# soypat/gsdf

Hardware: AMD Instinct MI355X
Metric: sdf_evals_per_s (higher is better)
Workload: dtype f32

## Files before the change

### gsdf_amd/csrc/abi_host.h

```cpp
#pragma once
#include <hip/hip_runtime.h>

#include <atomic>
#include <cmath>
#include <cstdint>
#include <cstdlib>
#include <string>

#pragma GCC visibility push(default)
#include "../../include/gsdf_hip.h"
#pragma GCC visibility pop

int fail(int code, const std::string& msg);
#define HIP_TRY(expr)                                                                                   \
  do {                                                                                                  \
    hipError_t _e = (expr);                                                                             \
    if (_e != hipSuccess) return fail(GSDF_ERR_HIP, std::string(#expr) + ": " + hipGetErrorString(_e)); \
  } while (0)
#define HIP_TRYM(expr)                                                                                        \
  do {                                                                                                        \
    hipError_t _e = (expr);                                                                                   \
    if (_e != hipSuccess) return bail(fail(GSDF_ERR_HIP, std::string(#expr) + ": " + hipGetErrorString(_e))); \
  } while (0)

inline int env_int(const char* name, int dflt) { const char* e = getenv(name); return e ? atoi(e) : dflt; }
inline uint64_t env_u64(const char* name, uint64_t dflt) { const char* e = getenv(name); return e ? (uint64_t)strtoull(e, nullptr, 10) : dflt; }
inline bool env_flag(const char* name) { const char* e = getenv(name); return e && atoi(e) != 0; }
inline bool env_flag_on(const char* name) { const char* e = getenv(name); return !e || atoi(e) != 0; }
inline bool env_set(const char* name) { return getenv(name) != nullptr; }

inline bool finite_all(const float* v, int n) {
  for (int i = 0; i < n; i++) if (!std::isfinite(v[i])) return false;
  return true;
}

struct gsdf_mesh {
  int device = 0;
  float* d_tris = nullptr;
  uint64_t cap = 0;
  gsdf_mesh_stats st{};
  hipStream_t stream = nullptr;
  hipStream_t rstream = nullptr;
  bool host_out = false;
  void* h_tris = nullptr;
  size_t h_tris_cap = 0;
  void* h_stl = nullptr;
  size_t h_stl_cap = 0;
  int payload = 0;
  uint8_t* d_recs = nullptr;
  uint64_t recs_cap36 = 0;
  uint64_t n_recs = 0;
  bool weldable = false;
  uint8_t* d_wrecs = nullptr;
  uint64_t wrecs_cap36 = 0;
  uint64_t n_wrecs = 0;
  int num_cu = 256;
  int n_stages = 0;
  double stage_ms[8] = {0, 0, 0, 0, 0, 0, 0, 0};
  const char* stage_name[8] = {nullptr, nullptr, nullptr, nullptr, nullptr, nullptr, nullptr, nullptr};
  std::atomic<int> refs{1};
  std::atomic<int> inflight{0};
};
void mesh_inflight_done(gsdf_mesh* m);

struct gsdf_dense_part { uint64_t off, n_recs, tri0; };
constexpr int kDenseMaxParts = 64;
inline uint64_t dense_bytes(uint64_t n_recs) { return n_recs * 40ull + ((((n_recs + 255ull) / 256ull) * 4ull + 7ull) & ~7ull); }
size_t dense_parts_bytes();
void* dense_parts_at(float* d_tris, uint64_t n_tris);
int mesh_march_dense(const uint8_t* d_buf, const gsdf_dense_part* parts, int nparts, void* d_parts, float ox, float oy, float oz, float res,
                     float* d_tris, int num_cu, hipStream_t s);

int indexed_from_cube_slots(int device, int num_cu, hipStream_t s, float* d_slot_cube, uint64_t slot_cap36, uint64_t S, uint64_t cube_cap, const float* d_fv,
                            const void* d_cubes, const hipEvent_t key_ev[4], gsdf_indexed** out);
int launch_block_scan(const unsigned* d_cnt, unsigned n, unsigned* d_base, unsigned long long* d_total, hipStream_t s);

float* pool_take(int device, uint64_t need, uint64_t* cap_out);
void pool_give(int device, float* p, uint64_t cap);
void pool_exporter_opened();
void pool_exporter_closed();
void pool_note_exported(void* base);
void* hpool_take(size_t need, size_t* cap_out);
void hpool_give(void* p, size_t cap);
void big_memcpy(void* dst, const void* src, size_t n);
int host_buf(void** buf, size_t* cap, size_t need);
hipStream_t mesh_stream(gsdf_mesh* m);
void release_tris(gsdf_mesh* m);
```

### gsdf_amd/csrc/abi_mesh.hip

```cpp
#include <algorithm>
#include <cmath>
#include <cstdio>
#include <cstdlib>
#include <cstring>
#include <new>
#include <vector>

#include "kernels_common.h"
#include "kernels_octree.h"
#include "kernels_flat.h"
#include "kernels_dc.h"
#include "kernels_dc_indexed.h"
#include "kernels_stl.h"
#include "kernels_minecraft.h"
#include "abi_program.h"
#include "host_math.h"

namespace {
constexpr size_t kCtrBytes = (sizeof(MeshCounters) + 255) & ~(size_t)255;
const bool ctr_from_kernel = env_flag_on("GSDF_HIP_CTR_FROM_KERNEL");

using leaf_eval_kernel_t = decltype(&leaf_eval_kernel<4, 3>);
using leaf_dense_kernel_t = decltype(&leaf_dense_kernel<3, true, false>);
using dc_origin_kernel_t = decltype(&dc_origin_kernel<4, 3>);
using flat_grid_kernel_t = decltype(&flat_grid_kernel<4, 4>);
leaf_dense_kernel_t leaf_dense_aot(int w) {
  if (w == 3) return leaf_dense_kernel<3, true, false>;
  if (w == 2) return leaf_dense_kernel<2, true, false>;
  return nullptr;
}
leaf_eval_kernel_t leaf_eval_aot(const LeafVariant& v) {
  struct Row { int k, w; bool ucube, ntlds, dz; leaf_eval_kernel_t f; };
  static const Row rows[] = {
      {4, 2, true, true, true, leaf_eval_kernel<4, 2, true, true, false, true>},   {4, 3, true, true, true, leaf_eval_kernel<4, 3, true, true, false, true>},
      {4, 2, true, false, true, leaf_eval_kernel<4, 2, true, false, false, true>}, {4, 3, true, false, true, leaf_eval_kernel<4, 3, true, false, false, true>},
      {4, 2, false, true, false, leaf_eval_kernel<4, 2, false, true>}, {4, 2, true, true, false, leaf_eval_kernel<4, 2, true, true>}, {4, 2, true, false, false, leaf_eval_kernel<4, 2, true, false>},
      {4, 3, false, true, false, leaf_eval_kernel<4, 3, false, true>}, {4, 3, true, true, false, leaf_eval_kernel<4, 3, true, true>}, {4, 3, true, false, false, leaf_eval_kernel<4, 3, true, false>},
      {2, 3, false, true, false, leaf_eval_kernel<2, 3, false, true>}, {2, 3, true, true, false, leaf_eval_kernel<2, 3, true, true>}, {2, 3, true, false, false, leaf_eval_kernel<2, 3, true, false>},
      {1, 4, false, true, false, leaf_eval_kernel<1, 4, false, true>}, {1, 4, true, true, false, leaf_eval_kernel<1, 4, true, true>}, {1, 4, true, false, false, leaf_eval_kernel<1, 4, true, false>},
  };
  if (v.both) return nullptr;
  for (const Row& r : rows)
    if (r.k == v.k && r.w == v.w && r.ucube == v.ucube && r.ntlds == v.ntlds && r.dz == v.dz) return r.f;
  return nullptr;
}
dc_origin_kernel_t dc_origin_aot(SweepVariant v) {
  if (v.k == 4 && v.w == 3) return dc_origin_kernel<4, 3>;
  if (v.k == 2 && v.w == 3) return dc_origin_kernel<2, 3>;
  if (v.k == 1 && v.w == 4) return dc_origin_kernel<1, 4>;
  return nullptr;
}
flat_grid_kernel_t flat_grid_aot(SweepVariant v) {
  if (v.k == 4) return v.w == 4 ? flat_grid_kernel<4, 4> : flat_grid_kernel<4, 3>;
  if (v.k == 2) return v.w == 4 ? flat_grid_kernel<2, 4> : flat_grid_kernel<2, 3>;
  return flat_grid_kernel<1, 4>;
}
}

struct gsdf_mesh_job {
  gsdf_program* p = nullptr;
  gsdf_mesh* m = nullptr;
  gsdf_mesh_opts opts{};
  float res = 0, ox = 0, oy = 0, oz = 0;
  hipStream_t s = nullptr;
  int levels = 0, lq = 0, ls = 0, prune_cols = 0, pmask = 0, ptest = 0, lk = 0;
  size_t lds_prune = 0, lds_m = 0;
  bool want_recs = false;
  uint64_t qcap = 0, want = 0, want_rec_n = 0;
  int attempt = 0, slot;
  bool ctr_on_host = false, used_dz = false, used_dense = false;
  int chain_first = 0;
  uint64_t nblk = 0, nblk_q = 0, lbound = 0;
  size_t clear_bytes = 0;
  bool masks_valid = false;
  Cube* q[2] = {nullptr, nullptr};
  uint64_t capq[2] = {0, 0};
  MeshCounters* d_ctr = nullptr;
  MeshCounters* hcp = nullptr;
  hipEvent_t ev_done = nullptr;
  gsdf_program::OctreeWs& w;
  explicit gsdf_mesh_job(gsdf_program* pp, int sl) : p(pp), slot(sl), w(pp->ws[sl]) {}

  int enqueue();
  int prepare_outputs();
  int enqueue_descent();
  int enqueue_leaf();
  int enqueue_handover();
  int finish(bool* again);
  int stats();
};

int gsdf_mesh_job::enqueue() {
  ctr_on_host = false;
  used_dz = false;
  used_dense = false;
  if (int rc = prepare_outputs()) return rc;
  if (int rc = enqueue_descent()) return rc;
  if (int rc = enqueue_leaf()) return rc;
  HIP_TRY(hipEventRecord(w.ev[2], s));
  return enqueue_handover();
}

int gsdf_mesh_job::prepare_outputs() {
  HIP_TRY(w.q0.ensure(qcap * sizeof(Cube)));
  HIP_TRY(w.q1.ensure(qcap * sizeof(Cube)));
  q[0] = (Cube*)w.q0.p; q[1] = (Cube*)w.q1.p;
  capq[0] = w.q0.cap / sizeof(Cube); capq[1] = w.q1.cap / sizeof(Cube);
  if (want_recs && !m->d_recs) {
    const uint64_t nrec = want_rec_n ? want_rec_n : (p->last_recs ? p->last_recs + p->last_recs / 16 + 1024 : (uint64_t)1 << 20);
    const uint64_t units = (dense_bytes(nrec) + 35) / 36;
    m->d_recs = (uint8_t*)pool_take(p->device, units, &m->recs_cap36);
    if (!m->d_recs) { HIP_TRY(hipMalloc((void**)&m->d_recs, units * 36)); m->recs_cap36 = units; }
  }
  if (!want_recs && !m->d_tris) {
    uint64_t need = want ? want : (p->last_tris ? p->last_tris + p->last_tris / 16 + 1024 : (uint64_t)1 << 20);
    if (opts.host_output) {
      void* hb = nullptr;
      size_t hcap = 0;
      if (int rc = host_buf(&hb, &hcap, (size_t)need * 36)) return rc;
      m->d_tris = (float*)hb;
      m->cap = hcap / 36;
      m->host_out = true;
    } else {
      m->d_tris = pool_take(p->device, need, &m->cap);
      if (!m->d_tris) {
        HIP_TRY(hipMalloc((void**)&m->d_tris, need * 36));
        m->cap = need;
      }
    }
  }
  lbound = capq[lq & 1] << (3 * (lq - 1));
  {
    const uint64_t full = (levels - lq) * 3 >= 40 ? UINT64_MAX : ((uint64_t)1 << (3 * (levels - 1)));
    if (lbound > full) lbound = full;
  }
  constexpr uint64_t kRecBlocks0 = (uint64_t)384 << 10;
  nblk_q = (lbound + 63) / 64;
  nblk = p->rec_blocks ? p->rec_blocks : kRecBlocks0;
  if (nblk > nblk_q) nblk = nblk_q;
  const uint64_t ngrp = (nblk + MARCH_GROUP - 1) / MARCH_GROUP;
  const size_t hdr_bytes = nblk * sizeof(uint32_t), rec_bytes = nblk * (size_t)REC_BLOCK * sizeof(uint32_t);
  if (w.hdr.ensure(hdr_bytes) != hipSuccess || w.rec.ensure(rec_bytes) != hipSuccess) {
    (void)hipGetLastError();
    w.hdr.release(); w.rec.release();
    return fail(GSDF_ERR_CAPACITY, "no device memory for the cut-leaf record arena (" + std::to_string(nblk) + " blocks: " + std::to_string(hdr_bytes) + " + " +
                                       std::to_string(rec_bytes) + " bytes)");
  }
  if (want_recs && w.grp.ensure(ngrp * sizeof(unsigned long long)) != hipSuccess) {
    (void)hipGetLastError();
    return (fail(GSDF_ERR_CAPACITY, "no device memory for the cut-leaf record arena (payload = records needs it)"));
  }
  clear_bytes = kCtrBytes + ngrp * sizeof(unsigned long long);
  HIP_TRY(w.ctr.ensure(clear_bytes));
  d_ctr = (MeshCounters*)w.ctr.p;
  masks_valid = lq == 3 && ptest == 1 && p->prog.n_skip_ids > 0 && (pmask == 1 || (pmask > 1 && ((pmask >> lq) & 1)));
  return GSDF_OK;
}

int gsdf_mesh_job::enqueue_descent() {
  static const bool use_spec = env_flag_on("GSDF_HIP_PRUNE_SPEC");
  if (!use_spec) HIP_TRY(hipMemsetAsync(d_ctr, 0, clear_bytes, s));
  HIP_TRY(hipEventRecord(w.ev[0], s));
  static const int prune_bpc = env_int("GSDF_HIP_PRUNE_BPC", 2);
  int first_level = levels;
  chain_first = levels;
  unsigned* spec_part = nullptr;
  unsigned spec_rows = 0, spec_mask = 0;
  int spec_top_S = 0;
  const unsigned test_mask = pmask == 1 ? 0xffffffffu : (unsigned)pmask;
  if (use_spec) {
    const int S = levels - lq + 1 < 7 ? levels - lq + 1 : 7;
    const int last_spec = levels - (S - 1);
    unsigned n_spec = 0;
    for (int j = 0; j < S; j++) n_spec += 1u << (3 * j);
    const unsigned rrows = (n_spec + SPEC_STAGE - 1) / SPEC_STAGE;
    const size_t part_off = ((size_t)n_spec + 63) & ~(size_t)63;
    const unsigned n_last = 1u << (3 * (S - 1));
    const size_t mask_off_b = (part_off + (size_t)rrows * 16 * sizeof(unsigned) + 63) & ~(size_t)63;
    const bool spec_masks = masks_valid && last_spec == lq;
    HIP_TRY(w.spec_pass.ensure(mask_off_b + (spec_masks ? (size_t)n_last * sizeof(uint16_t) : 0)));
    uint16_t* d_mask16 = spec_masks ? (uint16_t*)((char*)w.spec_pass.p + mask_off_b) : nullptr;
    const bool chain_follows = last_spec - 1 >= lq;
    spec_part = chain_follows ? (unsigned*)((char*)w.spec_pass.p + part_off) : nullptr;
    spec_rows = rrows;
    spec_top_S = levels | (S << 8);
    spec_mask = test_mask;
    const int shard_level = opts.shard_count > 1 ? ls : -1;
    HIP_TRY(launch_kernel(prune_spec_kernel, p->spec.f_prune_spec, grid_for(n_spec, p->num_cu, 8), BLOCK, lds_prune, s, p->d_code.p, levels, n_spec, prune_cols, p->prog.nslots, ox, oy,
                          oz, res, test_mask, ptest, shard_level, opts.shard_rank, opts.shard_count, w.spec_pass.p, (unsigned*)d_ctr, clear_bytes / 4, d_mask16, n_spec - n_last));
    hipLaunchKernelGGL(prune_resolve_kernel, dim3((n_spec + SPEC_STAGE - 1) / SPEC_STAGE), dim3(BLOCK), 0, s, (const uint8_t*)w.spec_pass.p, levels, S,
                       n_spec, test_mask, q[last_spec & 1], (unsigned long long)capq[last_spec & 1], d_ctr, spec_part,
                       (const uint16_t*)d_mask16);
    HIP_TRY(hipGetLastError());
    first_level = last_spec - 1;
    chain_first = first_level;
  }
  for (int level = first_level; level >= lq; level--) {
    const int expand = level != levels;
    const int do_test = (level >= 3 && (pmask == 1 || (pmask > 1 && ((pmask >> level) & 1)))) ? ptest : 0;
    uint64_t bound = (levels - level) * 3 >= 40 ? UINT64_MAX : ((uint64_t)1 << (3 * (levels - level)));
    if (bound > capq[(level + 1) & 1] * 8) bound = capq[(level + 1) & 1] * 8;
    HIP_TRY(launch_kernel(prune_kernel, p->spec.f_prune, grid_for(bound, p->num_cu, prune_bpc), BLOCK, lds_prune, s, p->d_code.p, q[(level + 1) & 1], capq[(level + 1) & 1], expand, level,
                          prune_cols, p->prog.nslots, ox, oy, oz, res, do_test, q[level & 1], capq[level & 1], (opts.shard_count > 1 && level == ls) ? 1 : 0, opts.shard_rank,
                          opts.shard_count, d_ctr, level == first_level ? spec_part : nullptr, spec_rows, spec_top_S, spec_mask));
  }
  HIP_TRY(hipEventRecord(w.ev[1], s));
  return GSDF_OK;
}

int gsdf_mesh_job::enqueue_leaf() {
  const uint64_t bound = lbound;
  const unsigned long long tcap = opts.max_tris ? opts.max_tris : m->cap;
  static const int leaf_bpc = env_int("GSDF_HIP_LEAF_BPC", 32);
  const unsigned grid = grid_for(bound, p->num_cu, leaf_bpc);
  const Cube* cubes = q[lq & 1];
  const uint64_t ncubes = capq[lq & 1];
  uint32_t* d_hdr = (uint32_t*)w.hdr.p;
  uint32_t* d_rec = (uint32_t*)w.rec.p;
  unsigned long long* d_psum = (unsigned long long*)((char*)w.ctr.p + kCtrBytes);
  const unsigned use_masks = masks_valid ? 1u : 0u;
  used_dense = opts.share_corners == 1 && lq == 3 && lk == 4;
  const bool want_dz = opts.share_corners == 2 && lq == 3 && lk == 4;
  if (used_dense) {
    spec_ensure(p, SPEC_DENSE);
    const size_t lds_d = p->lds_dense();
    HIP_TRY(launch_kernel(leaf_dense_aot(3 * lds_d <= gsdf_program::kLdsPerCu ? 3 : 2), p->spec.f_leaf_dense, grid, BLOCK, lds_d, s, p->d_code.p, cubes, ncubes, p->prog.nslots, ox, oy, oz, res,
                          d_hdr, d_rec, d_psum, nblk, d_ctr, use_masks));
  } else {
    if (want_dz) spec_ensure(p, SPEC_ROWS);
    const LeafPick pick = p->leaf_pick(lq, want_dz);
    used_dz = pick.v.dz;
    HIP_TRY(launch_kernel(leaf_eval_aot(pick.v), pick.f, grid, BLOCK, lq != 3 ? lds_m + 256 : lds_m, s, p->d_code.p, cubes, ncubes, lq, p->prog.nslots, ox, oy, oz, res, d_hdr, d_rec,
                          d_psum, nblk, d_ctr, use_masks));
  }
  HIP_TRY(hipEventRecord(w.ev[3], s));
  if (want_recs) {
    uint64_t rec_cap = m->recs_cap36 * 36 / 41;
    if (rec_cap > 2) rec_cap -= 2;
    hipLaunchKernelGGL(scan_groups_kernel, dim3(1), dim3(1024), 0, s, (const unsigned long long*)d_psum, (unsigned long long)nblk, lq, d_ctr,
                       (unsigned long long*)w.grp.p, m->d_recs, (unsigned long long)rec_cap,
                       ctr_from_kernel ? hcp : (MeshCounters*)nullptr);
    HIP_TRY(hipGetLastError());
    const uint64_t ngrp_q = (nblk_q + MARCH_GROUP - 1) / MARCH_GROUP;
    const uint64_t gmax = (uint64_t)p->num_cu * 8;
    hipLaunchKernelGGL(pack_records_kernel, dim3((unsigned)(ngrp_q < gmax ? (ngrp_q ? ngrp_q : 1) : gmax)), dim3(BLOCK), 0, s, (const uint32_t*)d_hdr,
                       (const uint32_t*)d_rec, (const unsigned long long*)w.grp.p, (unsigned long long)nblk, lq, (const MeshCounters*)d_ctr,
                       m->d_recs, (unsigned long long)rec_cap);
  } else {
    static const int march_bpc = env_int("GSDF_HIP_MARCH_BPC", 4);
    const size_t lds_march = MARCH_LDS_BYTES;
    hipLaunchKernelGGL(march_records_kernel, dim3(grid_for(nblk_q, p->num_cu, march_bpc)), dim3(BLOCK), lds_march, s, d_hdr, d_rec,
                       d_psum, (unsigned long long)nblk, lq, ox, oy, oz, res, m->d_tris, (uint64_t)tcap, d_ctr,
                       ctr_from_kernel ? hcp : (MeshCounters*)nullptr);
  }
  ctr_on_host = ctr_from_kernel;
  HIP_TRY(hipGetLastError());
  return GSDF_OK;
}

int gsdf_mesh_job::enqueue_handover() {
  if (!ctr_on_host) {
    HIP_TRY(hipMemcpyAsync(hcp, d_ctr, sizeof(MeshCounters), hipMemcpyDeviceToHost, s));
    HIP_TRY(hipEventRecord(w.ev[4], s));
  }
  ev_done = ctr_on_host ? w.ev[2] : w.ev[4];
  return GSDF_OK;
}

int gsdf_mesh_job::finish(bool* again) {
    MeshCounters& hc = *hcp;
    HIP_TRY(hipEventSynchronize(ev_done));
    if (hc.q_overflow) {
      if (attempt >= 8) return (fail(GSDF_ERR_CAPACITY, "octree queue capacity exceeded"));
      qcap *= 4;
      *again = true;
      return GSDF_OK;
    }
    const uint64_t need = ((hc.n_level[lq] << (3 * (lq - 1))) + 63) / 64;
    if (need > nblk) {
      if (attempt >= 8) return (fail(GSDF_ERR_CAPACITY, "cut-leaf record arena capacity exceeded"));
      p->rec_blocks = need + need / 8 + 1024;
      *again = true;
      return GSDF_OK;
    }
    if (hc.overflow && want_recs) {
      if (attempt >= 8) return (fail(GSDF_ERR_CAPACITY, "device record buffer capacity exceeded"));
      pool_give(p->device, (float*)m->d_recs, m->recs_cap36);
      m->d_recs = nullptr; m->recs_cap36 = 0;
      want_rec_n = hc.n_cut + hc.n_cut / 16 + 1024;
      *again = true;
      return GSDF_OK;
    }
    if (hc.overflow) {
      if (opts.max_tris) return (fail(GSDF_ERR_CAPACITY, "device triangle buffer capacity exceeded"));
      if (attempt >= 8) return (fail(GSDF_ERR_CAPACITY, "device triangle buffer capacity exceeded"));
      release_tris(m);
      want = hc.n_tris + hc.n_tris / 16 + 1024;
      *again = true;
      return GSDF_OK;
    }
    *again = false;
    return GSDF_OK;
}

int gsdf_mesh_job::stats() {
  MeshCounters& hc = *hcp;
  float ms01 = 0, ms12 = 0, ms13 = 0;
  HIP_TRY(hipEventElapsedTime(&ms01, w.ev[0], w.ev[1]));
  HIP_TRY(hipEventElapsedTime(&ms12, w.ev[1], w.ev[2]));
  HIP_TRY(hipEventElapsedTime(&ms13, w.ev[1], w.ev[3]));
  uint64_t evals_prune = 0, pruned = 0;
  for (int level = levels; level >= lq; level--) {
    evals_prune += hc.n_items[level];
    const bool dealt_here = opts.shard_count > 1 && level == ls;
    const uint64_t passed = (level <= chain_first && !dealt_here) ? hc.n_level[level] : hc.n_pass[level];
    if (hc.n_items[level]) pruned += (hc.n_items[level] - passed) << (3 * (level - 1));
  }
  const uint64_t n_leaves = hc.n_level[lq] << (3 * (lq - 1));
  const uint64_t evals_leaf = used_dz || used_dense ? hc.n_points
                                                    : n_leaves * (uint64_t)lk + (uint64_t)(8 - lk) * (lq == 3 ? n_leaves : hc.n_cont);
  m->st.n_tris = hc.n_tris;
  m->st.evals = evals_prune + evals_leaf;
  m->st.evals_prune = evals_prune;
  m->st.evals_leaf = evals_leaf;
  m->st.pruned_leaves = pruned;
  m->st.leaf_cubes = n_leaves;
  m->st.active_leaves = hc.n_active;
  m->st.ms_prune = ms01;
  m->st.ms_leaf = ms12;
  m->st.ms_march = ms13;
  m->st.ms_emit = ms12 - ms13;
  m->st.cut_leaves = hc.n_cut;
  m->st.ms_total = (double)ms01 + (double)ms12;
  p->evals += m->st.evals;
  p->last_tris = hc.n_tris;
  if (want_recs) { m->payload = GSDF_PAYLOAD_RECORDS; m->n_recs = hc.n_cut; p->last_recs = hc.n_cut; m->weldable = opts.shard_count == 1; }
  return GSDF_OK;
}

static void job_release(gsdf_mesh_job* j, bool failed = true) {
  if (!j) return;
  if (failed && j->s) { (void)hipStreamSynchronize(j->s); (void)hipGetLastError(); }
  if (j->p) j->w.job_busy = false;
  if (j->m) gsdf_hip_mesh_destroy(j->m);
  delete j;
}

static constexpr size_t lds_prune_of(int cols) { return (size_t)(cols > 0 ? cols : 1) * 2 * BLOCK * sizeof(float) + PRUNE_STAGE * sizeof(Cube) + 64; }
static constexpr size_t kPruneSpecStatic = SPEC_STAGE * sizeof(Cube) + 256;
static_assert(lds_prune_of(GSDF_HIP_MAX_COLS_OCTREE) + kPruneSpecStatic <= gsdf_program::kLdsPerCu && lds_prune_of(GSDF_HIP_MAX_COLS_OCTREE + 1) + kPruneSpecStatic > gsdf_program::kLdsPerCu,
              "gsdf_hip.h: GSDF_HIP_MAX_COLS_OCTREE is the largest slots + interval stack the centre tests fit into a CU's LDS");
static constexpr size_t lds_dc_edges_of(int slots) { return (size_t)(slots > 0 ? slots : 1) * 3 * BLOCK * sizeof(float) + DC_EDGE_PASSES * BLOCK * sizeof(uint16_t) + 64; }
static_assert(lds_dc_edges_of(GSDF_HIP_MAX_SLOTS_DC) <= gsdf_program::kLdsPerCu && lds_dc_edges_of(GSDF_HIP_MAX_SLOTS_DC + 1) > gsdf_program::kLdsPerCu,
              "gsdf_hip.h: GSDF_HIP_MAX_SLOTS_DC is the largest slot count the edge pass fits into a CU's LDS");
static_assert(GSDF_HIP_MAX_SLOTS_ALL + 16 == GSDF_HIP_MAX_COLS_OCTREE && GSDF_HIP_MAX_SLOTS_ALL <= GSDF_HIP_MAX_SLOTS_DC, "gsdf_hip.h: GSDF_HIP_MAX_SLOTS_ALL");

extern "C" int gsdf_hip_mesh_octree_start(gsdf_program* p, float res, const gsdf_mesh_opts* opts_in, gsdf_mesh_job** out) {
  if (!p || !out) return fail(GSDF_ERR_BAD_ARGUMENT, "null argument");
  *out = nullptr;
  spec_adopt(p);
  if (p->prog.is2d) return fail(GSDF_ERR_DIMENSION, "program is 2D");
  if (!(res > 0) || std::isnan(res) || std::isinf(res)) return fail(GSDF_ERR_RESOLUTION, "invalid renderer cube resolution");
  gsdf_mesh_opts opts{};
  opts.prune = 1; opts.shard_rank = 0; opts.shard_count = 1; opts.share_corners = 0;
  if (opts_in) opts = *opts_in;
  if (opts.shard_count < 1 || opts.shard_rank < 0 || opts.shard_rank >= opts.shard_count) return fail(GSDF_ERR_BAD_ARGUMENT, "bad shard rank/count");
  if (opts.payload != GSDF_PAYLOAD_TRIANGLES && opts.payload != GSDF_PAYLOAD_RECORDS) return fail(GSDF_ERR_BAD_ARGUMENT, "bad payload kind");
  const bool want_recs = opts.payload == GSDF_PAYLOAD_RECORDS;
  if (opts.share_corners < 0 || opts.share_corners > 3) return fail(GSDF_ERR_BAD_ARGUMENT, "share_corners is 0 (every corner of every leaf, as the reference), 1 (distinct lattice points of a brick), 2 (distinct z rows of a brick) or 3 (1 or 2, whichever suits the tree)");
  if (opts.share_corners == 3) opts.share_corners = gsdf_dev::spec_xy_shared_weight(p->prog) < 3 ? 1 : 2;
  if (want_recs && (opts.host_output || opts.max_tris))
    return fail(GSDF_ERR_BAD_ARGUMENT, "payload = records goes with the two-kernel leaf phase only (no host_output, max_tris)");
  {
    const size_t need_prune = lds_prune_of(p->prog.nslots + p->prog.lip_depth) + kPruneSpecStatic, need_leaf = p->leaf_config().lds + 256 + 1024;
    if (int rc = p->lds_refused("gsdf_hip_mesh_octree", need_prune > need_leaf ? need_prune : need_leaf, "slots + interval stack <= " + std::to_string(GSDF_HIP_MAX_COLS_OCTREE))) return rc;
  }
  HIP_TRY(hipSetDevice(p->device));

  float mn[3], mx[3];
  scale_centered(p->prog.bb, 1.01f, mn, mx);
  const float longAxis = fmaxf(mx[0] - mn[0], fmaxf(mx[1] - mn[1], mx[2] - mn[2]));
  const float l2 = gsdf::log2f32(longAxis / res);
  const int levels = (int)std::ceil(l2) + 1;
  if (levels <= 1) return fail(GSDF_ERR_RESOLUTION, "resolution not fine enough for marching cubes");
  if (levels > 17) return fail(GSDF_ERR_RESOLUTION, "resolution too fine: more than 17 octree levels");
// ... 61 lines not shown
    j->attempt++;
    if (int rc = j->enqueue()) { job_release(j); return rc; }
  }
  if (int rc = j->stats()) { job_release(j); return rc; }
  *out = j->m;
  j->m = nullptr;
  job_release(j, false);
  return GSDF_OK;
}

extern "C" int gsdf_hip_mesh_octree(gsdf_program* p, float res, const gsdf_mesh_opts* opts_in, gsdf_mesh** out) {
  if (!out) return fail(GSDF_ERR_BAD_ARGUMENT, "null argument");
  *out = nullptr;
  gsdf_mesh_job* j = nullptr;
  if (int rc = gsdf_hip_mesh_octree_start(p, res, opts_in, &j)) return rc;
  return gsdf_hip_mesh_octree_wait(j, out);
}

static_assert(sizeof(gsdf_dense_part) == sizeof(DensePart) && kDenseMaxParts == DENSE_MAX_PARTS, "abi_host.h mirrors kernels_octree.h");
size_t dense_parts_bytes() { return sizeof(DenseParts) + 8; }
void* dense_parts_at(float* d_tris, uint64_t n_tris) {
  return (void*)(((uintptr_t)(d_tris + n_tris * 9) + 7) & ~(uintptr_t)7);
}
int mesh_march_dense(const uint8_t* d_buf, const gsdf_dense_part* parts, int nparts, void* d_parts, float ox, float oy, float oz, float res,
                     float* d_tris, int num_cu, hipStream_t s) {
  if (nparts < 1 || nparts > DENSE_MAX_PARTS) return fail(GSDF_ERR_BAD_ARGUMENT, "march over packed records: 1 to 64 parts");
  DenseParts h{};
  h.n = nparts;
  uint64_t chunks = 0;
  for (int i = 0; i < nparts; i++) {
    h.p[i].off = parts[i].off; h.p[i].n_recs = parts[i].n_recs; h.p[i].tri0 = parts[i].tri0;
    chunks += (parts[i].n_recs + DENSE_CHUNK - 1) / DENSE_CHUNK;
    if (dense_bytes(parts[i].n_recs) != dense_payload_bytes(parts[i].n_recs)) return fail(GSDF_ERR_BAD_ARGUMENT, "internal: payload layouts differ");
  }
  if (chunks == 0) return GSDF_OK;
  HIP_TRY(hipMemcpyAsync(d_parts, &h, sizeof h, hipMemcpyHostToDevice, s));
  static const int march_bpc = env_int("GSDF_HIP_MARCH_BPC", 4);
  const uint64_t gmax = (uint64_t)num_cu * (uint64_t)(march_bpc > 0 ? march_bpc : 4);
  const size_t lds = MARCH_DENSE_LDS_BYTES;
  hipLaunchKernelGGL(march_dense_kernel, dim3((unsigned)(chunks < gmax ? chunks : gmax)), dim3(BLOCK), lds, s, d_buf, (const DenseParts*)d_parts, ox, oy, oz, res, d_tris);
  HIP_TRY(hipGetLastError());
  return GSDF_OK;
}

extern "C" int gsdf_hip_mesh_stage_ms(const gsdf_mesh* m, double* ms, const char** names, int cap, int* n) {
  if (!m || !n) return fail(GSDF_ERR_BAD_ARGUMENT, "null argument");
  *n = m->n_stages;
  for (int k = 0; k < m->n_stages && k < cap; k++) {
    if (ms) ms[k] = m->stage_ms[k];
    if (names) names[k] = m->stage_name[k];
  }
  return GSDF_OK;
}

extern "C" int gsdf_hip_mesh_payload(const gsdf_mesh* m, uint64_t* n_records, uint64_t* payload_bytes) {
  if (!m) return fail(GSDF_ERR_BAD_ARGUMENT, "null argument");
  const bool r = m->payload == GSDF_PAYLOAD_RECORDS;
  if (n_records) *n_records = r ? m->n_recs : 0;
  if (payload_bytes) *payload_bytes = r ? dense_bytes(m->n_recs) : 0;
  return m->payload;
}

extern "C" int gsdf_hip_mesh_read_records(const gsdf_mesh* m, uint32_t* dst, uint64_t dst_records, uint64_t* n_records) {
  if (!m) return fail(GSDF_ERR_BAD_ARGUMENT, "null argument");
  const bool r = m->payload == GSDF_PAYLOAD_RECORDS;
  const uint8_t* d = r ? m->d_recs : m->d_wrecs;
  const uint64_t n = r ? m->n_recs : m->n_wrecs;
  if (!r && !m->weldable) return fail(GSDF_ERR_BAD_ARGUMENT, "the mesh holds no cut-leaf records (payload = GSDF_PAYLOAD_RECORDS keeps them)");
  if (n_records) *n_records = n;
  if (!dst) return GSDF_OK;
  if (dst_records < n) return fail(GSDF_ERR_SHORT_BUFFER, "short buffer");
  if (n == 0) return GSDF_OK;
  HIP_TRY(hipSetDevice(m->device));
  HIP_TRY(hipMemcpy(dst, d, n * 40ull, hipMemcpyDeviceToHost));
  return GSDF_OK;
}

extern "C" int gsdf_hip_mesh_march(gsdf_mesh* m) {
  if (!m) return fail(GSDF_ERR_BAD_ARGUMENT, "null argument");
  if (m->payload != GSDF_PAYLOAD_RECORDS) return GSDF_OK;
  if (m->inflight.load() > 0) return fail(GSDF_ERR_BAD_ARGUMENT, "the mesh is being gathered: wait for the gather first");
  HIP_TRY(hipSetDevice(m->device));
  const uint64_t n = m->st.n_tris;
  if (n) {
    const uint64_t units = n + (dense_parts_bytes() + 35) / 36;
    m->d_tris = pool_take(m->device, units, &m->cap);
    if (!m->d_tris) {
      if (hipMalloc((void**)&m->d_tris, units * 36) != hipSuccess) { (void)hipGetLastError(); return fail(GSDF_ERR_HIP, "hipMalloc of the triangle buffer failed"); }
      m->cap = units;
    }
    const gsdf_dense_part part{0, m->n_recs, 0};
    hipStream_t rs = mesh_stream(m);
    const int rc = mesh_march_dense(m->d_recs, &part, 1, dense_parts_at(m->d_tris, n), m->st.origin[0], m->st.origin[1], m->st.origin[2], m->st.res, m->d_tris,
                                    m->num_cu, rs);
    if (rc) { release_tris(m); return rc; }
    hipError_t e = hipStreamSynchronize(rs);
    if (e != hipSuccess) { release_tris(m); return fail(GSDF_ERR_HIP, std::string("march over the records: ") + hipGetErrorString(e)); }
  }
  if (m->weldable) { m->d_wrecs = m->d_recs; m->wrecs_cap36 = m->recs_cap36; m->n_wrecs = m->n_recs; }
  else pool_give(m->device, (float*)m->d_recs, m->recs_cap36);
  m->d_recs = nullptr; m->recs_cap36 = 0; m->n_recs = 0;
  m->payload = GSDF_PAYLOAD_TRIANGLES;
  return GSDF_OK;
}

namespace {
// ... 610 lines not shown
```

### gsdf_amd/csrc/abi_program.h

```cpp
#pragma once
#include <condition_variable>
#include <mutex>
#include <thread>
#include <vector>

#include "abi_host.h"
#include "compile.h"
#include "launch_args.h"
#include "specialize.h"

struct NoCopy {
  NoCopy() = default;
  NoCopy(const NoCopy&) = delete;
  NoCopy& operator=(const NoCopy&) = delete;
};
struct Arena : NoCopy {
  void* p = nullptr;
  size_t cap = 0;
  ~Arena() { release(); }
  hipError_t ensure(size_t bytes) {
    if (bytes <= cap) return hipSuccess;
    release();
    size_t want = bytes + bytes / 4 + 4096;
    hipError_t e = hipMalloc(&p, want);
// ... 31 lines not shown
  int k, w;
  std::string spec_name(const char* base, int dim = 0) const { return std::string(base) + "<" + (dim ? std::to_string(dim) + ", " : "") + std::to_string(k) + ", " + std::to_string(w) + ">"; }
  std::string short_name(const char* base, int dim = 0) const { return std::string(base) + "<" + (dim ? std::to_string(dim) + "," : "") + std::to_string(k) + "," + std::to_string(w) + ">"; }
};
struct LeafVariant {
  int k, w;
  bool ucube, ntlds, both, dz;
  std::string spec_name() const {
    auto b = [](bool x) { return x ? ", true" : ", false"; };
    return "leaf_eval_kernel<" + std::to_string(k) + ", " + std::to_string(w) + b(ucube) + b(ntlds) + b(both) + b(dz) + ">";
  }
  std::string short_name() const {
    return "leaf_eval_kernel<" + std::to_string(k) + "," + std::to_string(w) + (both ? ",both" : "") + (dz ? ",rows" : "") + ">";
  }
};
struct LeafPick { LeafVariant v; hipFunction_t f; };

enum SpecGroup { SPEC_AUX, SPEC_ROWS, SPEC_EVAL_K1, SPEC_DENSE, SPEC_VIEW, SPEC_PROJECT, SPEC_PICTURE, SPEC_RAY, SPEC_GROUPS };
struct SpecBuilt {
  std::vector<hipModule_t> mods;
  int eval_k = 0, eval_w = 0, leaf_k = 0, leaf_w = 0, rows_w = 0, dense_w = 0;
  bool leaf_both = false, rows_both = false;
  std::string compiler, key;
  double compile_s = 0;
};
struct SpecFns {
  hipFunction_t f_eval = nullptr, f_eval_k1 = nullptr, f_prune = nullptr, f_prune_spec = nullptr, f_leaf = nullptr, f_leaf_dz = nullptr, f_leaf_dense = nullptr;
  hipFunction_t f_dc_block_test = nullptr, f_dc_origin = nullptr, f_dc_edges = nullptr, f_dc_normals = nullptr, f_normals = nullptr, f_image = nullptr, f_flat_grid = nullptr;
  hipFunction_t f_view = nullptr, f_view_plain = nullptr, f_project = nullptr, f_imgc[4] = {nullptr, nullptr, nullptr, nullptr};
  hipFunction_t f_ray = nullptr, f_ray_thick = nullptr;
};
struct SpecKernels : SpecBuilt, SpecFns, NoCopy {
  std::atomic<unsigned> todo{0};
  ~SpecKernels() { for (hipModule_t m : mods) (void)hipModuleUnload(m); }
  bool specialised() const { return !mods.empty(); }
  void take(SpecKernels& from) {
    std::swap(static_cast<SpecBuilt&>(*this), static_cast<SpecBuilt&>(from));
    compile_s += from.compile_s;
    std::atomic_thread_fence(std::memory_order_release);
    static_cast<SpecFns&>(*this) = from;
    todo.store(from.todo.load(), std::memory_order_release);
  }
};

struct gsdf_program {
  gsdf_dev::Program prog;
  int device = 0;
  Stream stream;
  struct OctreeWs {
    Stream own;
    Arena q0, q1;
    Arena ctr;
    Arena spec_pass;
    Arena rec, hdr;
    Arena grp;
    EventSet<5> ev;
    bool job_busy = false;
    hipStream_t job_stream = nullptr;
  };
  static constexpr int kJobs = 3;
  OctreeWs ws[kJobs];
  bool mesh_in_flight() const { for (const OctreeWs& w : ws) if (w.job_busy) return true; return false; }
  DevPtr<uint32_t> d_code;
  std::atomic<uint64_t> evals{0};
  DevPtr<void> d_pos;
  DevPtr<float> d_dist;
  size_t cap_pos_bytes = 0, cap_dist = 0;
  struct Slot : NoCopy {
    Stream s;
    PinnedPtr<void> h_pos;
    PinnedPtr<float> h_dist;
    bool busy = false, waiting = false;
    unsigned gen = 0;
    float* user_dist = nullptr;
    size_t n = 0;
    bool zero_copy = false;
    PinnedPtr<unsigned> h_flag;
    unsigned* d_flag = nullptr;
    unsigned flag_val = 0;
    bool flagged = false;
  };
  static constexpr int kSlots = 4;
  Slot slot[kSlots];
  std::mutex slot_mu;
  std::condition_variable slot_cv;
  std::atomic<uint64_t> evals_host{0};
  int num_cu = 256;
  Arena dc_tile, dc_grid, dc_dist, dc_fv, dc_nrm, dc_edge, dc_erun, dc_flag;
  Arena dc_ix, dc_ix_sort;
  EventSet<4> dc_ev;
  Arena flat_grid;
  Arena flat_bits;
  Arena flat_list;
  PinnedPtr<void> h_ctr;
  uint64_t last_tris = 0;
  uint64_t last_recs = 0;
  uint64_t rec_blocks = 0;
  uint64_t last_dc_cubes = 0;
  SpecKernels spec;
  size_t lds_dense() const { return (size_t)(prog.nslots * 4 > 8 ? prog.nslots * 4 : 8) * BLOCK * sizeof(float) + 256 + 4 * 512 * sizeof(float) + 4 * 24 * sizeof(float) + 16; }
  struct CountedLaunch { DevPtr<void> ctr; EventSet<2> ev; };
  CountedLaunch proj, ray;
  std::atomic<int> spec_async{0};
  std::thread spec_thread;
  gsdf_program* spec_shadow = nullptr;
  std::mutex spec_async_mu;
// ... 108 lines not shown
```

### gsdf_amd/csrc/compile.cpp

```cpp
#include "compile.h"

#include <algorithm>
#include <cmath>
#include <cstdlib>
#include <cstring>
#include <stdexcept>
#include <string>
#include <utility>

#include "host_math.h"
#include "dev_ops.h"
#include "gsdf_seams.h"

namespace gsdf_dev {

float recip_for(float d) {
  const float a = std::fabs(d);
  if (!(a >= 9.313225746154785e-10f && a <= 1073741824.0f)) return 0.f;
  float best = (float)(1.0 / (double)d);
  long double berr = fabsl(1.0L - (long double)d * (long double)best);
  const float cand[2] = {std::nextafterf(best, INFINITY), std::nextafterf(best, -INFINITY)};
  for (float c : cand) {
    long double err = fabsl(1.0L - (long double)d * (long double)c);
    if (err < berr) { berr = err; best = c; }
  }
  return best;
}

namespace {

constexpr float SQRT3 = 1.7320508075688772935274463415058723669428052538103806280558069794f;

struct Ctx {
  const gsdf_tree* t;
  std::vector<uint32_t> code;
  int slots = 0;
  int max_slots = 0;
  int lip_depth = 0, max_lip_depth = 0;
  int n_recip = 0, n_recip_declined = 0, n_poly_recip = 0, n_poly_plain = 0;
  float node_recip(float d) { const float r = recip_for(d); (r != 0.f ? n_recip : n_recip_declined)++; return r; }
  int lip_push() { const int d = lip_depth++; if (lip_depth > max_lip_depth) max_lip_depth = lip_depth; op(D_LIP_PUSH, d); return d; }
  void lip_pop(int d) { op(D_LIP_POP, d); lip_depth--; }
  int discont = 0;
  bool numbering = false;
  std::vector<double> cand_cost;
  std::vector<int> cand_id;
  std::vector<uint64_t> cand_key;
  size_t cand_next = 0;
  bool cand_mismatch = false;
  int candidate(double cost, uint32_t node, uint32_t child_slot) {
    const size_t i = cand_next++;
    const uint64_t key = ((uint64_t)node << 32) | child_slot;
    if (!numbering) { cand_cost.push_back(cost); cand_key.push_back(key); return -1; }
    if (i >= cand_id.size() || cand_key[i] != key) { cand_mismatch = true; return -1; }
    return cand_id[i];
  }
  size_t max_code;
  std::vector<int8_t> clob;
  struct Table { size_t patch; float angle; int n; };
  std::vector<Table> tables;
  uint32_t xyver = 1, next_ver = 2, hxyver = 0;
  std::vector<uint32_t> slotver = std::vector<uint32_t>(1 << 16, 0);
  void bump() { xyver = next_ver++; }
  uint32_t pver = 1;
  std::vector<uint32_t> slotpver = std::vector<uint32_t>(1 << 16, 0);
  uint8_t dep[3] = {1, 2, 4};
  std::vector<uint32_t> slotdep = std::vector<uint32_t>(1 << 16, 0x070707u);
  uint32_t shxy_flag() const { return ((dep[0] | dep[1]) & 4) ? 0u : D_FLAG_SHXY; }
  uint32_t shz_flag() const { return (dep[2] & 3) ? 0u : D_FLAG_SHZ; }
  void dep_after(uint32_t base) {
    switch (base) {
      case D_TRANSLATE: case D_SCALE_PRE: case D_SYMMETRY: case D_ELONGATE_PRE: case D_ELONGATE2D_PRE: case D_EXTRUDE_PRE:
        break;
      case D_ROT2D: case D_CIRC_PRE: dep[0] = dep[1] = (uint8_t)(dep[0] | dep[1]); break;
      case D_TWIST: dep[0] = dep[1] = (uint8_t)(dep[0] | dep[1] | dep[2]); break;
      default: dep[0] = dep[1] = dep[2] = 7; break;
    }
  }
  struct Outer { bool valid = false; int slot = 0; float ok = 0.f; } outer;
  struct Saved { int slot; bool is2d; };
  std::vector<Saved> live;
  int find_saved(bool is2d) const {
    for (size_t k = live.size(); k-- > 0;) {
      const Saved& s = live[k];
      if (is2d ? (slotver[(size_t)s.slot] == xyver) : (!s.is2d && slotpver[(size_t)s.slot] == pver)) return s.slot;
    }
    return -1;
  }
  void mark_saved(int slot, bool is2d) {
    slotver[(size_t)slot] = xyver;
    slotpver[(size_t)slot] = pver;
    slotdep[(size_t)slot] = dep[0] | (dep[1] << 8) | (dep[2] << 16);
    live.push_back({slot, is2d});
  }
  void load_saved(int slot, bool is2d) {
    op(is2d ? D_LOADP2 : D_LOADP3, slot);
// ... 618 lines not shown

void gen(Ctx& c, uint32_t i, int depth) {
  if (depth > 256) throw std::runtime_error("tree too deep (cycle?)");
  const gsdf_node& n = c.node(i);
  if (n.op != GSDF_DIFF && n.op != GSDF_SMOOTH_DIFF && n.op != GSDF_DIFF2D) c.outer.valid = false;
  const float* P = n.p;
  auto need_children = [&](uint32_t k) { if (n.nchild != k) throw std::runtime_error("bad child count for op " + std::to_string(n.op)); };
  auto child_dim = [&](bool want2d) {
    for (uint32_t k = 0; k < n.nchild; k++)
      if ((bool)gsdf_op_is2d(c.node(c.child(n, k)).op) != want2d) throw std::runtime_error("child dimension mismatch for op " + std::to_string(n.op));
  };
  switch (n.op) {
    case GSDF_SPHERE: c.op(D_SPHERE); c.f(P[0]); break;
    case GSDF_BOX: c.op(D_BOX); c.f(0.5f * P[0]); c.f(0.5f * P[1]); c.f(0.5f * P[2]); c.f(P[3]); break;
    case GSDF_BOXFRAME: {
      float e = P[3];
      c.op(D_BOXFRAME); c.f(e);
      c.f(0.5f * P[0] + (-2 * e)); c.f(0.5f * P[1] + (-2 * e)); c.f(0.5f * P[2] + (-2 * e));
      break;
    }
    case GSDF_TORUS: c.op(D_TORUS | c.hxy_flag() | c.shxy_flag()); c.f(P[0]); c.f(P[1]); break;
    case GSDF_CYLINDER: {
      float r = P[0], h = (P[1] - 2 * P[2]) / 2, round = P[2];
      if (round == 0) { c.op(D_CYL0 | c.hxy_flag() | c.shxy_flag()); c.f(r); c.f(h); }
      else { c.op(D_CYLR | c.hxy_flag() | c.shxy_flag()); c.f(r); c.f(h); c.f(round); }
      break;
    }
    case GSDF_HEX: c.op(D_HEX); c.f(P[0]); c.f(P[1]); c.f(0.57735f * P[0]); break;
    case GSDF_UNION: if (n.nchild < 2) throw std::runtime_error("OpUnion must have at least 2 elements"); child_dim(false); gen_combine(c, n, D_COMBINE_MIN, false, depth); break;
    case GSDF_INTERSECT: need_children(2); child_dim(false); gen_combine(c, n, D_COMBINE_MAX, false, depth); break;
    case GSDF_DIFF: need_children(2); child_dim(false); gen_combine(c, n, D_COMBINE_DIFF, false, depth); break;
    case GSDF_XOR: need_children(2); child_dim(false); gen_combine(c, n, D_COMBINE_XOR, false, depth); break;
    case GSDF_SMOOTH_UNION: need_children(2); child_dim(false); gen_combine(c, n, D_COMBINE_SUNION, true, depth); break;
    case GSDF_SMOOTH_DIFF: need_children(2); child_dim(false); gen_combine(c, n, D_COMBINE_SDIFF, true, depth); break;
    case GSDF_SMOOTH_INTERSECT: need_children(2); child_dim(false); gen_combine(c, n, D_COMBINE_SINTER, true, depth); break;
    case GSDF_SCALE: need_children(1); child_dim(false);
      { const int ld = c.lip_push(); c.op(D_SCALE_PRE); c.f(1.f / P[0]); c.bump(); gen(c, c.child(n, 0), depth + 1); c.op(D_MULR); c.f(P[0]); c.lip_pop(ld); } break;
    case GSDF_SYMMETRY: need_children(1); child_dim(false);
      c.op(D_SYMMETRY); c.u((uint32_t)(int)P[0]); if ((int)P[0] & 3) c.bump(); gen(c, c.child(n, 0), depth + 1); break;
    case GSDF_ARRAY: {
      need_children(1); child_dim(false);
      int slotP = c.alloc(3), slotD = c.alloc(1);
      const unsigned seams = array_seams(c, i);
      const int lipd = seams ? c.lip_push() : -1;
      c.op(D_SAVEP3, slotP);
      c.op(D_SETSLOT, slotD); c.f(1e20f);
      for (int k = 0; k < 2; k++) for (int j = 0; j < 2; j++) for (int ii = 0; ii < 2; ii++) {
        c.op(D_ARRAY_PRE, slotP);
        c.bump();
        c.f((float)ii); c.f((float)j); c.f((float)k);
        c.f(P[0]); c.f(P[1]); c.f(P[2]);
        c.f(P[3] + -1); c.f(P[4] + -1); c.f(P[5] + -1);
        if (seams && k == 0 && j == 0 && ii == 0) { c.op(D_LIP_SEAM); c.u(seams); }
        c.discont++; gen(c, c.child(n, 0), depth + 1); c.discont--;
        c.op(D_COMBINE_MIN, slotD);
        if (!(k == 1 && j == 1 && ii == 1)) c.op(D_SAVER, slotD);
      }
      if (lipd >= 0) c.lip_pop(lipd);
      c.release(4);
      break;
    }
    case GSDF_ELONGATE: {
      need_children(1); child_dim(false);
      int s = c.alloc(1);
      c.op(D_ELONGATE_PRE, s); c.f(0.5f * P[0]); c.f(0.5f * P[1]); c.f(0.5f * P[2]);
      c.bump();
      gen(c, c.child(n, 0), depth + 1);
      c.op(D_ADDR_SLOT, s);
      c.release(1);
      break;
    }
    case GSDF_SHELL: need_children(1); child_dim(false);
      { const int ld = c.lip_push(); c.op(D_SCALE_PRE); c.f(1 / P[0]); c.bump(); gen(c, c.child(n, 0), depth + 1); c.op(D_SHELL_POST); c.f(P[0]); c.lip_pop(ld); } break;
    case GSDF_OFFSET: need_children(1); child_dim(false);
      gen(c, c.child(n, 0), depth + 1); c.op(D_ADDR); c.f(P[0]); break;
    case GSDF_TRANSLATE: need_children(1); child_dim(false);
      c.op(D_TRANSLATE); c.f(P[0]); c.f(P[1]); c.f(P[2]);
      if (!(P[0] == 0.f && P[1] == 0.f)) c.bump();
      gen(c, c.child(n, 0), depth + 1); break;
    case GSDF_TRANSFORM: {
      need_children(1); child_dim(false);
      if (n.aux_len < 16) throw std::runtime_error("transform needs 16 aux floats");
      int lipd = -1;
      {
        float f = lip_norm3(&c.t->aux[n.aux_off]);
        if (f > kLipRigidTol) { lipd = c.lip_push(); c.op(D_LIP_MUL); c.f(f * kLipRoundUp); }
      }
      c.op(D_TRANSFORM);
      for (int k = 0; k < 12; k++) c.f(c.t->aux[n.aux_off + k]);
      c.bump();
      gen(c, c.child(n, 0), depth + 1);
      if (lipd >= 0) c.lip_pop(lipd);
      break;
    }
    case GSDF_CIRCARRAY: case GSDF_CIRCARRAY2D: {
      need_children(1);
      bool is2d = n.op == GSDF_CIRCARRAY2D;
      child_dim(is2d);
      int slotP = c.alloc(is2d ? 2 : 3), slotD = c.alloc(1);
      const bool seams = circ_seams(c, i);
      const int lipd = seams ? c.lip_push() : -1;
      if (!is2d) c.op(D_SAVEP3, slotP);
      c.op(D_CIRC_PRE | c.shxy_flag(), slotP);
      c.bump();
      c.slotver[(size_t)slotP] = c.xyver;
      c.slotpver[(size_t)slotP] = c.next_ver++;
      c.slotdep[(size_t)slotP] = c.dep[0] | (c.dep[1] << 8) | (c.dep[2] << 16);
      c.live.push_back({slotP, is2d});
      c.bump();
      c.f((float)(2 * gsdf::kPi) / P[1]); c.f(P[1]); c.f((float)((int)P[0] - 1));
      c.tables.push_back({c.code.size(), (float)(2 * gsdf::kPi) / P[1], (int)P[1]});
      c.u(0);
      Region cg;
      const bool sector_off = [] { const char* e = getenv("GSDF_HIP_NO_SECTOR_GATE"); return e && atoi(e) != 0; }();
      constexpr double kSectorGateMinCost = 150.0;
      const bool sector_gate = !sector_off && !is2d && subtree_cost(c, c.child(n, 0)) >= kSectorGateMinCost && lower_region(c, c.child(n, 0), cg) &&
                               (cg.kind == Region::BOX || cg.kind == Region::OBOX);
      if (sector_gate && cg.kind == Region::BOX) {
        Region o;
        o.kind = Region::OBOX;
        o.b[0] = 0.5f * (cg.b[0] + cg.b[3]); o.b[1] = 0.5f * (cg.b[1] + cg.b[4]); o.b[2] = 1.f; o.b[3] = 0.f;
        o.b[4] = 0.5f * (cg.b[3] - cg.b[0]) * 1.000001f; o.b[5] = 0.5f * (cg.b[4] - cg.b[1]) * 1.000001f; o.b[6] = cg.b[2]; o.b[7] = cg.b[5];
        cg = o;
      }
      if (sector_gate) { c.op(D_CIRC_ORDER, slotP); for (int j = 0; j < 6; j++) c.f(cg.b[j]); }
      if (seams) { c.op(D_LIP_SEAM, slotP); c.u(8u); }
      c.discont++;
      gen(c, c.child(n, 0), depth + 1);
      c.op(D_SAVER, slotD);
      c.load_saved(slotP, is2d);
      if (is2d) c.slotpver[(size_t)slotP] = c.pver;
      long skip_at = -1, gate_pc = -1;
      const uint32_t hxy_before = c.hxyver;
      if (sector_gate) {
        gate_pc = (long)c.code.size();
        c.op(D_GATEOB, slotD);
        for (int j = 0; j < 8; j++) c.f(cg.b[j]);
        c.f(1.0f); c.f(0.0f); c.u(0xffffu); c.f(0.0f); c.f(0.0f);
        skip_at = (long)c.code.size();
        c.u(0);
      }
      gen(c, c.child(n, 0), depth + 1);
      c.discont--;
      if (skip_at >= 0) {
        if (c.hxyver != hxy_before) c.hxyver = 0;
        c.code[(size_t)skip_at] = (uint32_t)((long)c.code.size() - gate_pc);
      }
      c.op(D_COMBINE_MIN, slotD);
      if (lipd >= 0) c.lip_pop(lipd);
      c.live.pop_back();
      c.release(is2d ? 3 : 4);
      break;
    }
    case GSDF_TWIST: {
      need_children(1); child_dim(false);
      const int lipd = c.lip_push();
      c.op(D_TWIST | c.shz_flag()); c.f(P[0]); c.bump(); gen(c, c.child(n, 0), depth + 1);
      c.lip_pop(lipd);
      break;
    }
    case GSDF_EXTRUSION: {
      need_children(1); child_dim(true);
      int s = c.alloc(1);
      c.op(D_EXTRUDE_PRE, s); c.f(P[0] / 2);
      gen(c, c.child(n, 0), depth + 1);
      c.op(D_EXTRUDE_POST, s);
      c.release(1);
      break;
    }
    case GSDF_REVOLUTION: need_children(1); child_dim(true);
      c.op(D_REVOLVE_PRE); c.f(P[0]); c.bump(); gen(c, c.child(n, 0), depth + 1); break;
    case GSDF_SCREW: {
      need_children(1); child_dim(true);
      int s = c.alloc(1);
      const int lipd = c.lip_push();
      c.op(D_SCREW_PRE | c.hxy_flag() | c.shxy_flag(), s);
      c.bump();
      c.f(P[0]); c.f(P[1]); c.f(P[2]); c.f(gsdf::tanf32(P[3])); c.f(P[0] / 2); c.f(c.node_recip(P[0]));
      c.op(D_LIP_WRAP); c.f(P[0] / 2); c.f(lip_screw_seam(*c.t, c.child(n, 0), P[0]));
      c.discont++; gen(c, c.child(n, 0), depth + 1); c.discont--;
      c.lip_pop(lipd);
      c.op(D_MAXR_SLOT, s);
      c.release(1);
      break;
    }
    case GSDF_LINE2D: {
      float bax = P[2] - P[0], bay = P[3] - P[1];
      c.op(D_LINE2D); c.f(P[0]); c.f(P[1]); c.f(bax); c.f(bay); c.f(bax * bax + bay * bay); c.f(P[4] / 2);
      break;
    }
    case GSDF_ARC2D: {
      float s, cs;
      gsdf::sincosf32(P[1] / 2, s, cs);
      c.op(D_ARC2D); c.f(P[0]); c.f(P[2] / 2); c.f(s); c.f(cs); c.f(P[0] * s); c.f(P[0] * cs);
      break;
    }
    case GSDF_QUADBEZIER2D: {
      float Ax = P[0], Ay = P[1], Bx = P[2], By = P[3], Cx = P[4], Cy = P[5];
      float ax = Bx - Ax, ay = By - Ay;
      float a2 = ax * ax + ay * ay;
      float bx = Ax + (Cx - 2 * Bx), by = Ay + (Cy - 2 * By);
      float cx = 2 * ax, cy = 2 * ay;
      float kk = 1.f / (bx * bx + by * by);
      float kx = kk * (ax * bx + ay * by);
      float kx2 = kx * kx;
      c.op(D_QUADBEZIER2D);
      c.f(Ax); c.f(Ay); c.f(ax); c.f(ay); c.f(a2); c.f(bx); c.f(by); c.f(cx); c.f(cy); c.f(kk); c.f(kx); c.f(kx2); c.f(P[6] / 2);
      break;
    }
    case GSDF_CIRCLE2D: c.op(D_CIRCLE2D | c.hxy_flag() | c.shxy_flag()); c.f(P[0]); break;
    case GSDF_EQTRI2D: { float r = P[0] / SQRT3; c.op(D_EQTRI2D); c.f(r); c.f(r / SQRT3); break; }
    case GSDF_RECT2D: c.op(D_RECT2D); c.f(0.5f * P[0]); c.f(0.5f * P[1]); break;
    case GSDF_DIAMOND2D: {
      float bx = 0.5f * P[0], by = 0.5f * P[1];
      c.op(D_DIAMOND2D); c.f(bx); c.f(by); c.f(bx * bx + by * by); c.f(0.5f * bx); c.f(0.5f * by); c.f(bx * by);
      break;
    }
    case GSDF_X2D: c.op(D_X2D); c.f(P[0]); c.f(P[1]); break;
    case GSDF_HEX2D: c.op(D_HEX2D); c.f(P[0]); c.f(0.577350269f * P[0]); break;
    case GSDF_OCT2D: c.op(D_OCT2D); c.f(P[0]); c.f(0.4142135623f * P[0]); break;
    case GSDF_ELLIPSE2D: c.op(D_ELLIPSE2D); c.f(P[0]); c.f(P[1]); break;
    case GSDF_POLY2D: {
      uint32_t nv = n.aux_len / 2;
      if (nv < 3) throw std::runtime_error("polygon needs at least 3 vertices");
      const float* v = &c.t->aux[n.aux_off];
      bool all_recip = true;
      {
        uint32_t jv0 = nv - 1;
        for (uint32_t iv = 0; iv < nv; iv++) {
          float ex = v[2 * jv0] - v[2 * iv], ey = v[2 * jv0 + 1] - v[2 * iv + 1];
          if (recip_for(ex * ex + ey * ey) == 0.f) all_recip = false;
          jv0 = iv;
        }
      }
      (all_recip ? c.n_poly_recip : c.n_poly_plain)++;
      c.op(D_POLY2D); c.u(nv | (all_recip ? 0x80000000u : 0u)); c.f(v[0]); c.f(v[1]);
      while (c.code.size() % 8 != 0) c.u(0);
      uint32_t jv = nv - 1;
      for (uint32_t iv = 0; iv < nv; iv++) {
        float v1x = v[2 * iv], v1y = v[2 * iv + 1], v2x = v[2 * jv], v2y = v[2 * jv + 1];
        float ex = v2x - v1x, ey = v2y - v1y;
        const float n2e = ex * ex + ey * ey;
        c.f(v1x); c.f(v1y); c.f(ex); c.f(ey); c.f(n2e); c.f(v2y); c.f(recip_for(n2e)); c.u(0);
        jv = iv;
      }
      break;
    }
    case GSDF_LINES2D: {
      uint32_t ns = n.aux_len / 4;
      const float* sg = &c.t->aux[n.aux_off];
      c.op(D_LINES2D); c.u(ns); c.f(P[0] / 2);
      for (uint32_t k = 0; k < ns; k++) {
        float ax = sg[4 * k], ay = sg[4 * k + 1], bax = sg[4 * k + 2] - ax, bay = sg[4 * k + 3] - ay;
        c.f(ax); c.f(ay); c.f(bax); c.f(bay); c.f(bax * bax + bay * bay);
      }
      break;
    }
    case GSDF_UNION2D: if (n.nchild < 2) throw std::runtime_error("OpUnion2D must have at least 2 elements"); child_dim(true); gen_combine(c, n, D_COMBINE_MIN, false, depth); break;
    case GSDF_INTERSECT2D: need_children(2); child_dim(true); gen_combine(c, n, D_COMBINE_MAX, false, depth); break;
    case GSDF_DIFF2D: need_children(2); child_dim(true); gen_combine(c, n, D_COMBINE_DIFF, false, depth); break;
    case GSDF_XOR2D: need_children(2); child_dim(true); gen_combine(c, n, D_COMBINE_XOR, false, depth); break;
    case GSDF_ARRAY2D: {
      need_children(1); child_dim(true);
      int slotP = c.alloc(2), slotD = c.alloc(1);
      const unsigned seams = array_seams(c, i);
      const int lipd = seams ? c.lip_push() : -1;
      c.op(D_SAVEP2, slotP);
      c.op(D_SETSLOT, slotD); c.f(1e20f);
      for (int j = 0; j < 2; j++) for (int ii = 0; ii < 2; ii++) {
        c.op(D_ARRAY2D_PRE, slotP);
        c.bump();
        c.f((float)ii); c.f((float)j); c.f(P[0]); c.f(P[1]); c.f(P[2] + -1); c.f(P[3] + -1);
        if (seams && j == 0 && ii == 0) { c.op(D_LIP_SEAM); c.u(seams); }
        c.discont++; gen(c, c.child(n, 0), depth + 1); c.discont--;
        c.op(D_COMBINE_MIN, slotD);
        if (!(j == 1 && ii == 1)) c.op(D_SAVER, slotD);
      }
      if (lipd >= 0) c.lip_pop(lipd);
      c.release(3);
      break;
    }
    case GSDF_OFFSET2D: need_children(1); child_dim(true); gen(c, c.child(n, 0), depth + 1); c.op(D_ADDR); c.f(P[0]); break;
    case GSDF_TRANSLATE2D: need_children(1); child_dim(true);
      c.op(D_TRANSLATE); c.f(P[0]); c.f(P[1]); c.f(0.f); if (!(P[0] == 0.f && P[1] == 0.f)) c.bump(); gen(c, c.child(n, 0), depth + 1); break;
    case GSDF_SYMMETRY2D: need_children(1); child_dim(true);
      c.op(D_SYMMETRY); c.u((uint32_t)(int)P[0] & 3u); if ((int)P[0] & 3) c.bump(); gen(c, c.child(n, 0), depth + 1); break;
    case GSDF_ANNULUS2D: need_children(1); child_dim(true); gen(c, c.child(n, 0), depth + 1); c.op(D_ANNULUS); c.f(P[0]); break;
    case GSDF_TRANSLATEMULTI2D: {
      need_children(1); child_dim(true);
      uint32_t nd = n.aux_len / 2;
      const float* d = &c.t->aux[n.aux_off];
      int slotP = c.alloc(2), slotD = c.alloc(1);
      c.op(D_SAVEP2, slotP);
      c.op(D_SETSLOT, slotD); c.f(3.40282346638528859811704183484516925440e+38f);
      if (nd == 0) { c.op(D_SETR); c.f(3.40282346638528859811704183484516925440e+38f); }
      for (uint32_t k = 0; k < nd; k++) {
        c.op(D_LOADP2_SUB, slotP); c.f(d[2 * k]); c.f(d[2 * k + 1]);
        c.bump();
        gen(c, c.child(n, 0), depth + 1);
        c.op(D_COMBINE_MIN, slotD);
        if (k + 1 < nd) c.op(D_SAVER, slotD);
      }
      c.release(3);
      break;
    }
    case GSDF_ROTATION2D: {
      need_children(1); child_dim(true);
      int lipd = -1;
      {
        float f = lip_norm2(P[0], P[1], P[2], P[3]);
        if (f > kLipRigidTol) { lipd = c.lip_push(); c.op(D_LIP_MUL); c.f(f * kLipRoundUp); }
      }
      c.op(D_ROT2D); c.f(P[0]); c.f(P[1]); c.f(P[2]); c.f(P[3]); c.bump(); gen(c, c.child(n, 0), depth + 1);
      if (lipd >= 0) c.lip_pop(lipd);
      break;
    }
    case GSDF_SCALE2D: need_children(1); child_dim(true);
      { const int ld = c.lip_push(); c.op(D_SCALE_PRE); c.f(1.f / P[0]); c.bump(); gen(c, c.child(n, 0), depth + 1); c.op(D_MULR); c.f(P[0]); c.lip_pop(ld); } break;
    case GSDF_ELONGATE2D: {
      need_children(1); child_dim(true);
      int s = c.alloc(1);
      c.op(D_ELONGATE2D_PRE, s); c.f(0.5f * P[0]); c.f(0.5f * P[1]);
      c.bump();
      gen(c, c.child(n, 0), depth + 1);
      c.op(D_ADDR_SLOT, s);
      c.release(1);
      break;
// ... 63 lines not shown
    const bool masks_off = [] { const char* e = getenv("GSDF_HIP_NO_BRICK_MASKS"); return e && atoi(e) != 0; }();
    cand_id.assign(c0.cand_cost.size(), -1);
    cand_key = c0.cand_key;
    if (!masks_off) {
      std::vector<size_t> idx(c0.cand_cost.size());
      for (size_t i = 0; i < idx.size(); i++) idx[i] = i;
      std::stable_sort(idx.begin(), idx.end(), [&](size_t x, size_t y) { return c0.cand_cost[x] > c0.cand_cost[y]; });
      std::vector<char> take(idx.size(), 0);
      for (size_t i = 0; i < idx.size() && i < 16; i++) take[idx[i]] = 1;
      int next = 0;
      for (size_t i = 0; i < take.size(); i++) if (take[i]) cand_id[i] = next++;
    }
  }
  Ctx c;
  c.t = &t;
  c.max_code = max_code_words;
  c.clob.assign(t.n_nodes, -1);
  c.numbering = true;
  c.cand_id = cand_id;
  c.cand_key = cand_key;
  gen(c, t.root, 0);
  if (c.cand_mismatch || c.cand_next != cand_id.size()) {
    bool any = false;
    for (int v : cand_id) any = any || v >= 0;
    if (any) {
      Ctx c2;
      c2.t = &t;
      c2.max_code = max_code_words;
      c2.clob.assign(t.n_nodes, -1);
      c2.numbering = true;
      c2.cand_id.assign(cand_id.size(), -1);
      c2.cand_key = cand_key;
      gen(c2, t.root, 0);
      if (c2.cand_mismatch || c2.cand_next != cand_id.size()) throw std::runtime_error("lowering is not repeatable: candidate subtrees differ between runs");
      c = std::move(c2);
      std::fill(cand_id.begin(), cand_id.end(), -1);
    }
  }
  c.op(D_END);
  for (const Ctx::Table& tb : c.tables) {
    if (tb.n < 1 || tb.n > 4096) continue;
    c.code[tb.patch] = (uint32_t)c.code.size();
    for (int i = 0; i < tb.n; i++) {
      float sn, cs;
      gsdf::sincosf32(tb.angle * (float)i, sn, cs);
      c.f(sn); c.f(cs);
    }
  }
  Program p;
  p.code = std::move(c.code);
  p.nslots = c.max_slots;
  p.lip_depth = c.max_lip_depth;
  p.n_recip = c.n_recip; p.n_recip_declined = c.n_recip_declined; p.n_poly_recip = c.n_poly_recip; p.n_poly_plain = c.n_poly_plain;
  p.n_skip_ids = 0;
  for (int v : cand_id) if (v >= 0) p.n_skip_ids++;
  p.is2d = gsdf_op_is2d(t.nodes[t.root].op);
  p.has_exact_bb = exact_box(c, t.root, p.exact_bb);
  std::memcpy(p.bb, t.bb, sizeof(p.bb));
  return p;
}

}
```

### gsdf_amd/csrc/compile.h

```cpp
#pragma once
#include <cstddef>
#include <cstdint>
#include <vector>

#include "../../include/gsdf_program.h"

namespace gsdf_dev {

struct Program {
  std::vector<uint32_t> code;
  int nslots = 0;
  int lip_depth = 0;
  int n_skip_ids = 0;
  bool is2d = false;
  float bb[6] = {0};
  bool has_exact_bb = false;
  float exact_bb[6] = {0};
  int n_recip = 0, n_recip_declined = 0, n_poly_recip = 0, n_poly_plain = 0;
};

float recip_for(float d);

int region_of(const gsdf_tree& t, uint32_t node, float params[8]);

Program compile(const gsdf_tree& t, size_t max_code_words = (1u << 22));

}
```

### gsdf_amd/csrc/dev_ops.h

```cpp
#pragma once
#ifndef __HIPCC_RTC__
#include <stdint.h>
#endif

#define D_OP_MASK 0x0fffu
#define D_FLAG_SHZ 0x1000u
#define D_FLAG_SHXY 0x2000u
#define D_FLAG_HXY 0x4000u
#define D_FLAG_SWAP 0x8000u

enum DevOp : uint32_t {
  D_END = 0,
  D_SPHERE,
  D_BOX,
  D_BOXFRAME,
  D_TORUS,
  D_CYL0,
  D_CYLR,
  D_HEX,
  D_LINE2D,
  D_ARC2D,
  D_QUADBEZIER2D,
  D_CIRCLE2D,
  D_EQTRI2D,
// ... 18 lines not shown
  D_ELONGATE2D_PRE,
  D_ARRAY_PRE,
  D_ARRAY2D_PRE,
  D_CIRC_PRE,
  D_LOADP2_SUB,
  D_MULR,
  D_SHELL_POST,
  D_ADDR,
  D_ANNULUS,
  D_EXTRUDE_POST,
  D_MAXR_SLOT,
  D_ADDR_SLOT,
  D_SAVEP3, D_LOADP3, D_SAVEP2, D_LOADP2, D_SAVER,
  D_SETSLOT,
  D_SETR,
  D_COMBINE_MIN, D_COMBINE_MAX, D_COMBINE_DIFF, D_COMBINE_XOR,
  D_COMBINE_SUNION, D_COMBINE_SDIFF, D_COMBINE_SINTER,
  D_GATE2D,
  D_GATE3D,
  D_GATEZC,
  D_UBOUND2D,
  D_UBOUND3D,
  D_GATEOB,
  D_CIRC_ORDER,
  D_LIP_PUSH,
  D_LIP_POP,
  D_LIP_MUL,
  D_LIP_WRAP,
  D_SKIP,
  D_LIP_DOM,
  D_LIP_SEAM,
  D_OP_COUNT
};

static const uint8_t kDevOpParams[D_OP_COUNT] = {
     0,
     1,  4,  4,  2,  2,  3,  3,
     6,  6,  13,  1,  2,  2,  6,  2,
     2,  2,  2,  3,  2,
     3,  1,  1,  12,  1,  4,
     1,  1,  6,  3,  2,
     9,  6,  4,  2,
     1,  1,  1,  1,  0,  0,  0,
     0,  0,  0,  0,  0,  1,  1,
     0,  0,  0,  0,  2,  2,  2,
     10,  12,  13,  1,  1,  14,  6,
     0,  0,  1,  2,
     3,  5,  1,
};
#define GSDF_GATE_SKIP(w) ((w) & 0x00ffffffu)
#define GSDF_GATE_ID1(w) ((w) >> 24)
#define GSDF_BRICK_MASK_VALID 0x80000000u
#define GSDF_SKIP_BIG 1.0e30f
```

### gsdf_amd/csrc/interp.h

```cpp
#pragma once
#ifndef __HIPCC_RTC__
#include <hip/hip_runtime.h>
#endif

#include "dev_math.h"
#include "dev_ops.h"

namespace gsdf_dev {

typedef const uint32_t __attribute__((address_space(4))) * code_ptr;
typedef float v4f __attribute__((ext_vector_type(4)));
typedef const v4f __attribute__((address_space(4))) * f4ptr;

struct P3 { float x, y, z; };

__device__ __forceinline__ uint32_t lane_id() { return __builtin_amdgcn_mbcnt_hi(~0u, __builtin_amdgcn_mbcnt_lo(~0u, 0u)); }

#define LDSF(slot) lds[((slot) * K + kp) * nthreads]
#define KLOOP _Pragma("unroll") for (int kp = 0; kp < K; ++kp)

template <bool ON>
__device__ __forceinline__ float in_vgpr(float s) {
  if (!ON) return s;
  float v;
// ... 80 lines not shown
__device__ __forceinline__ float wave_minmax(float v) {
  if (MAX) {
#define GSDF_DPP_CHAIN(op)                                                                                                   \
  asm volatile("s_nop 1\n\t" op "_dpp %0, %0, %0 row_shr:1 row_mask:0xf bank_mask:0xf\n\t"                                  \
               "s_nop 1\n\t" op "_dpp %0, %0, %0 row_shr:2 row_mask:0xf bank_mask:0xf\n\t"                                  \
               "s_nop 1\n\t" op "_dpp %0, %0, %0 row_shr:4 row_mask:0xf bank_mask:0xf\n\t"                                  \
               "s_nop 1\n\t" op "_dpp %0, %0, %0 row_shr:8 row_mask:0xf bank_mask:0xf\n\t"                                  \
               "s_nop 1\n\t" op "_dpp %0, %0, %0 row_bcast:15 row_mask:0xa bank_mask:0xf\n\t"                               \
               "s_nop 1\n\t" op "_dpp %0, %0, %0 row_bcast:31 row_mask:0xc bank_mask:0xf\n\t"                               \
               "s_nop 1"                                                                                                     \
               : "+v"(v))
    GSDF_DPP_CHAIN("v_max_f32");
  } else {
    GSDF_DPP_CHAIN("v_min_f32");
  }
#undef GSDF_DPP_CHAIN
  return __uint_as_float((uint32_t)__builtin_amdgcn_readlane((int)__float_as_uint(v), 63));
}

template <int K>
__device__ __forceinline__ void poly_cull(code_ptr code, uint32_t q0, uint32_t nv, const P3 (&pv)[K], uint64_t& keepd,
                                          uint64_t& keeps, const bool recip = false) {
  using namespace dm;
  float x0 = pv[0].x, x1 = pv[0].x, y0 = pv[0].y, y1 = pv[0].y;
  KLOOP {
    x0 = minf(x0, pv[kp].x); x1 = maxf(x1, pv[kp].x);
    y0 = minf(y0, pv[kp].y); y1 = maxf(y1, pv[kp].y);
  }
  wave_box(x0, x1, y0, y1);
  const uint32_t lane = lane_id();
  const bool valid = lane < nv;
  const v4f* rec = (const v4f*)((const float*)(uintptr_t)code + q0 + 8u * (valid ? lane : 0u));
  const v4f r0 = rec[0], r1 = rec[1];
  const float v1x = r0.x, v1y = r0.y, ex = r0.z, ey = r0.w, n2e = r1.x, v2y = r1.y;
  const float cx = 0.5f * (x0 + x1), cy = 0.5f * (y0 + y1), hx = 0.5f * (x1 - x0), hy = 0.5f * (y1 - y0);
#ifdef GSDF_NO_CULL_APPROX
  const bool approx = false;
#else
  const bool approx = recip;
#endif
  const float rb2 = hx * hx + hy * hy;
  const float rb = approx ? __builtin_amdgcn_sqrtf(rb2) : sqrtf_(rb2);
  const float wx = cx - v1x, wy = cy - v1y;
  const float num = wx * ex + wy * ey;
  const float t = __builtin_amdgcn_fmed3f(approx ? num * r1.z : num / n2e, 0.f, 1.f);
  const float bx = wx - t * ex, by = wy - t * ey;
  const float dc2 = bx * bx + by * by;
  const float dc = approx ? __builtin_amdgcn_sqrtf(dc2) : sqrtf_(dc2);
  const float m = 1.0e-5f * (absf(wx) + absf(wy) + absf(ex) + absf(ey) + rb + absf(cx) + absf(cy));
  const float U = wave_minmax<false>(valid ? (dc + rb) + m : __builtin_inff());
  const uint64_t vm = nv >= 64u ? ~0ull : (1ull << nv) - 1ull;
  keepd = vm & ~wave_mask((dc - rb) - m > U);
  keeps = vm & ~((wave_mask(y0 >= v1y) & wave_mask(y0 >= v2y)) | (wave_mask(y1 < v1y) & wave_mask(y1 < v2y)));
}

template <int K, typename F>
__device__ __forceinline__ void xy_shared(const P3 (&pv)[K], float (&out)[K], bool shared, bool brick, F f, bool column = false) {
  if (shared && column) {
    const float v = f(pv[0].x, pv[0].y);
    KLOOP out[kp] = v;
    return;
  }
  if (K == 4 && shared && brick) {
    const uint32_t lane = lane_id();
    const bool odd = ((lane >> 4) & 1u) != 0u;
    const float sx = odd ? pv[K > 2 ? 2 : 0].x : pv[0].x, sy = odd ? pv[K > 2 ? 2 : 0].y : pv[0].y;
    const float v = f(sx, sy);
    const float v0 = __shfl(v, (int)(lane & 15u), 64), v1 = __shfl(v, (int)((lane & 15u) + 16u), 64);
    out[0] = v0; out[K > 1 ? 1 : 0] = v0;
    out[K > 2 ? 2 : 0] = v1; out[K > 3 ? 3 : 0] = v1;
    return;
  }
  KLOOP if (!(kp & 1)) out[kp] = f(pv[kp].x, pv[kp].y);
  if (shared) { KLOOP if (kp & 1) out[kp] = out[kp ? kp - 1 : 0]; }
  else { KLOOP if (kp & 1) out[kp] = f(pv[kp].x, pv[kp].y); }
}
struct XYCache {
  float th = 0.0f;
  uint32_t pc = 0xffffffffu;
};

template <int K>
__device__ __forceinline__ void atan2_shared(const P3 (&pv)[K], float (&out)[K], bool shared, bool brick, bool column) {
#if defined(GSDF_SPECIALIZED) && !defined(GSDF_NO_ATAN2_FAST)
  if (!(shared && column)) {
    dm::wave_ok ok;
    xy_shared<K>(pv, out, shared, brick, [&ok](float x, float y) { return dm::atan2_fast(y, x, ok); }, column);
    if (ok.all()) return;
  }
#endif
  xy_shared<K>(pv, out, shared, brick, [](float x, float y) { return dm::atan2_ref(y, x); }, column);
}

__device__ __forceinline__ void cossin_voted(float x, float& c, float& s) {
#if defined(GSDF_SPECIALIZED) && !defined(GSDF_NO_COSSIN_FAST)
  dm::wave_ok ok;
  dm::cossin_fast(x, c, s, ok);
  if (ok.all()) return;
#endif
  dm::cossinf_(x, c, s);
}

#define ENSURE_HXY() \
  if (!use_hxy) xy_shared<K>(pv, hxy, sh_xy, brick, [](float x, float y) { return dm::hypotf_(x, y); }, sh_col)

template <int K, int DIM>
// ... 161 lines not shown
            switch (kind) {                                                                                                            \
              case 0u: sb = blo > ahi + GSDF_DOM_M(blo, ahi); sa = alo > bhi + GSDF_DOM_M(alo, bhi); break;                            \
              case 1u: sb = bhi < alo - GSDF_DOM_M(bhi, alo); sa = ahi < blo - GSDF_DOM_M(ahi, blo); break;                            \
              case 2u: sb = blo > -alo + GSDF_DOM_M(blo, alo); sa = ahi < -bhi - GSDF_DOM_M(ahi, bhi); break;                          \
              case 3u: sb = blo - ahi > GSDF_DOM_M(blo, ahi); sa = alo - bhi > GSDF_DOM_M(alo, bhi); break;                            \
              case 4u: sb = blo + alo > GSDF_DOM_M(blo, alo); sa = bhi + ahi < -GSDF_DOM_M(bhi, ahi); break;                           \
              case 5u: sb = alo - bhi > GSDF_DOM_M(alo, bhi); sa = blo - ahi > GSDF_DOM_M(blo, ahi); break;                            \
              default: break;                                                                                                          \
            }                                                                                                                          \
            if (sa && ida < 32u) *lip_fired |= 1u << ida;                                                                              \
            if (sb && idb < 32u) *lip_fired |= 1u << idb;                                                                              \
          }                                                                                                                            \
        }                                                                                                                              \

#define GSDF_LIP_SEAM_BODY \
        if (LIP) {                                                                                                                     \
          const uint32_t seams = PU(0);                                                                                                \
          bool reach = false;                                                                                                          \
          if ((seams & 1u) != 0u) reach = reach || !(absf(pv[0].x) > lipR);                                                            \
          if ((seams & 2u) != 0u) reach = reach || !(absf(pv[0].y) > lipR);                                                            \
          if ((seams & 4u) != 0u) reach = reach || !(absf(pv[0].z) > lipR);                                                            \
          if ((seams & 8u) != 0u) {                  \
            const float x0 = lds[((slot) * K + LIP_LO) * nthreads], y0 = lds[((slot + 1u) * K + LIP_LO) * nthreads];                   \
            reach = !(lip_ray_dist(pv[0].x, pv[0].y) > lipR) || !(lip_ray_dist(x0, y0) > lipR);                                        \
          }                                                                                                                            \
          if (reach) lipR = GSDF_LIP_BIG;                                                                                              \
        }                                                                                                                              \

static_assert(GSDF_BRICK_MASK_VALID == 1u << 31, "GSDF_GATE_TEST reads the brick mask's valid flag as bit 31");
#define GSDF_GATE_TEST(REGION, DIM, I0)                                                                                      \
  float L[K];                                                                                                               \
  bool far_ = false;                                                                                                        \
  {                                                                                                                         \
    const uint32_t gid1 = GSDF_GATE_ID1(PU((I0) + 5));                                                                      \
     \
    const bool untested = !LIP && gid1 != 0u && ((bmask >> 31u) & 1u) != 0u;  \
    if (!untested) {                                                                                                        \
      float a[K], cc[K];                                                                                                    \
      const uint32_t oslot = PU((I0) + 2);                                                                                  \
      const bool has_outer = oslot != 0xffffu;                                                            \
      KLOOP { a[kp] = LDSF(slot); cc[kp] = has_outer ? LDSF(oslot) : 0.0f; }                                                \
      REGION;                                                                                                               \
      if (LIP) KLOOP L[kp] = L[kp] - lipR;  \
      bool lane_good = false;                                                                                               \
      far_ = gate_far<K, DIM, LIP>(pv, a, L, PF(I0), PF((I0) + 1), cc, has_outer, PF((I0) + 3), PF((I0) + 4), &lane_good);  \
      if (LIP && gid1 != 0u && lip_fired != nullptr && lane_good) *lip_fired |= 1u << (gid1 - 1u);                          \
    }                                                                                                                       \
  }
#define GSDF_GATE_TAKEN                                                       \
  {                                                                           \
    if (LIP) { Rv[LIP_LO] = L[LIP_LO]; Rv[LIP_HI] = GSDF_SKIP_BIG; }          \
    else { KLOOP Rv[kp] = L[kp]; }                                            \
  }
#ifndef GSDF_SPECIALIZED
template <int K, int SHARE = 0, bool LIP = false>
__device__ __forceinline__ void sdf_eval(code_ptr code, P3 (&pv)[K], float (&Rv)[K],
                                         float* __restrict__ lds , const uint32_t nthreads,
                                         const bool brick = false ,
                                         const float lip_h = 0.0f, const uint32_t lip_base = 0u,
                                         const uint32_t bmask_w = 0u ,
                                         uint32_t* lip_fired = nullptr ,
                                         XYCache* xyc = nullptr ) {
  using namespace dm;
  static_assert(!LIP || (K == 2 && SHARE == 0), "interval mode: two points per lane, lower and upper bound");
  [[maybe_unused]] float lipR = lip_h;
  const dm::uniform_word bmask{bmask_w};
  KLOOP Rv[kp] = 0.0f;
  float hxy[K];
  KLOOP hxy[kp] = 0.0f;
  uint32_t pc = 0;
#define PF(k) __uint_as_float(code[pc + 1 + (k)])
#define PU(k) (code[pc + 1 + (k)])
  for (;;) {
    pc = __builtin_amdgcn_readfirstlane(pc);
    const uint32_t w = code[pc];
    const uint32_t op = w & D_OP_MASK;
    const uint32_t slot = w >> 16;
    const bool use_hxy = (w & D_FLAG_HXY) != 0u;
    const bool swap_ab = (w & D_FLAG_SWAP) != 0u;
    const bool sh_xy = SHARE != 0 && K >= 2 && (w & D_FLAG_SHXY) != 0u;
    const bool sh_z = SHARE == 1 && K >= 4 && (w & D_FLAG_SHZ) != 0u;
    const bool sh_col = SHARE == 2;
    const bool sh_zu = SHARE == 2 && brick && (w & D_FLAG_SHZ) != 0u;
    switch (op) {
      case D_END:
        return;
      case D_SPHERE: {
        KLOOP {
          [[maybe_unused]] P3& p = pv[kp];
          [[maybe_unused]] float& R = Rv[kp];
          R = norm3(p.x, p.y, p.z) - PF(0);
        }
        pc += 2;
        break;
      }
      case D_BOX: {
        {
          const float r = PF(3);
          float u[K], v[K], w[K];
          KLOOP {
            const P3& p = pv[kp];
            u[kp] = (absf(p.x) - PF(0)) + r; v[kp] = (absf(p.y) - PF(1)) + r; w[kp] = (absf(p.z) - PF(2)) + r;
          }
          if (face3_op<K>(u, v, w)) {
            KLOOP Rv[kp] = face_val(maxf(u[kp], maxf(v[kp], w[kp]))) - r;
          } else {
            float mx[K], my[K], mz[K], in[K], hyz[K], n3[K];
            KLOOP {
              const float qx = u[kp], qy = v[kp], qz = w[kp];
              mx[kp] = maxf(qx, 0.f); my[kp] = maxf(qy, 0.f); mz[kp] = maxf(qz, 0.f);
              in[kp] = minf(maxf(qx, maxf(qy, qz)), 0.0f);
            }
            hypot_k<K>(my, mz, hyz);
            hypot_k<K>(mx, hyz, n3);
            KLOOP Rv[kp] = n3[kp] + in[kp] - r;
          }
// ... 297 lines not shown
          [[maybe_unused]] P3& p = pv[kp];
          [[maybe_unused]] float& R = Rv[kp];
          float a = PF(0), b = PF(1);
          float px = absf(p.x), py = absf(p.y);
          if (px > py) { float t = px; px = py; py = t; t = a; a = b; b = t; }
          float l = b * b - a * a;
          float m = a * px / l;
          float m2 = m * m;
          float nn = b * py / l;
          float n2 = nn * nn;
          float c = (m2 + n2 - 1.f) / 3.f;
          float c3 = c * c * c;
          float q = c3 + 2.f * m2 * n2;
          float d = c3 + m2 * n2;
          float g = m + m * n2;
          float co;
          if (d < 0.f) {
            float h = acosf_(q / c3) / 3.f;
            float sh, ch;
            sincosf_(h, sh, ch);
            float t = 1.7320508075688772f * sh;
            float rx = sqrtf_(-c * (ch + t + 2.f) + m2);
            float ry = sqrtf_(-c * (ch - t + 2.f) + m2);
            co = (ry + signf(l) * rx + absf(g) / (rx * ry) - m) / 2.f;
          } else {
            float h = 2.f * m * nn * sqrtf_(d);
            float sv = signf(q + h) * cbrtf_(absf(q + h));
            float u = signf(q - h) * cbrtf_(absf(q - h));
            float rx = -sv - u - 4.f * c + 2.f * m2;
            float ry = 1.7320508075688772f * (sv - u);
            float rm = hypotf_(rx, ry);
            co = (ry / sqrtf_(rm - rx) + 2.f * g / rm - m) / 2.f;
          }
          float rx2 = a * co, ry2 = b * sqrtf_(1.f - co * co);
          R = norm2(rx2 - px, ry2 - py) * signf(py - ry2);
        }
        pc += 3;
        break;
      }
      case D_POLY2D: {
        const uint32_t hdr = PU(0);
        const uint32_t nv = hdr & 0x7fffffffu;
        const float v0x = PF(1), v0y = PF(2);
        const uint32_t q0 = (pc + 4u + 7u) & ~7u;
        if (LIP) {
          const P3 p1[1] = {pv[0]};
          float d1[1];
          bool neg1[1];
          bool done1 = false;
          if (hdr >> 31) done1 = poly_edges<1, true>(code, q0, nv, v0x, v0y, p1, d1, neg1);
          if (!done1) poly_edges<1, false>(code, q0, nv, v0x, v0y, p1, d1, neg1);
          const float sd = sqrtf_(d1[0]);
          KLOOP Rv[kp] = neg1[0] ? -sd : sd;
        } else {
          float d[K];
          bool neg[K];
          bool done = false;
          uint64_t keepd = ~0ull, keeps = ~0ull;
          if (brick && nv >= 6u && nv <= 64u) poly_cull<K>(code, q0, nv, pv, keepd, keeps, (hdr >> 31) != 0u);
          if (hdr >> 31) done = poly_edges<K, true>(code, q0, nv, v0x, v0y, pv, d, neg, keepd, keeps);
          if (!done) poly_edges<K, false>(code, q0, nv, v0x, v0y, pv, d, neg, keepd, keeps);
          float sd[K];
          sqrt_k<K>(d, sd);
          KLOOP Rv[kp] = neg[kp] ? -sd[kp] : sd[kp];
        }
        pc = q0 + 8u * nv;
        break;
      }
      case D_LINES2D: {
        const uint32_t ns = PU(0);
        const float w2 = PF(1);
        float d[K];
        KLOOP d[kp] = 1e23f;
        uint32_t q = pc + 3;
        for (uint32_t sg = 0; sg < ns; sg++, q += 5) {
          const float ax = __uint_as_float(code[q]), ay = __uint_as_float(code[q + 1]), bax = __uint_as_float(code[q + 2]),
                      bay = __uint_as_float(code[q + 3]), dotba = __uint_as_float(code[q + 4]);
          KLOOP {
            float pax = pv[kp].x - ax, pay = pv[kp].y - ay;
            float h = clampf((pax * bax + pay * bay) / dotba, 0.f, 1.f);
            float rx = pax - h * bax, ry = pay - h * bay;
            d[kp] = minf(d[kp], rx * rx + ry * ry);
          }
        }
        float sd[K];
        sqrt_k<K>(d, sd);
        KLOOP Rv[kp] = sd[kp] - w2;
        pc = q;
        break;
      }
      case D_TRANSLATE: {
        KLOOP {
          [[maybe_unused]] P3& p = pv[kp];
          [[maybe_unused]] float& R = Rv[kp];
          p.x = p.x - PF(0); p.y = p.y - PF(1); p.z = p.z - PF(2);
        }
        pc += 4;
        break;
      }
      case D_SCALE_PRE: {
        KLOOP {
          [[maybe_unused]] P3& p = pv[kp];
          [[maybe_unused]] float& R = Rv[kp];
          const float f = PF(0);
          p.x = f * p.x; p.y = f * p.y; p.z = f * p.z;
        }
        if (LIP) lipR = lipR * absf(PF(0));
        pc += 2;
        break;
      }
      case D_SYMMETRY: {
        KLOOP {
// ... 61 lines not shown
        break;
      }
      case D_EXTRUDE_PRE: {
        KLOOP {
          [[maybe_unused]] P3& p = pv[kp];
          [[maybe_unused]] float& R = Rv[kp];
          LDSF(slot) = absf(p.z) - PF(0);
        }
        if (LIP) LIP_WIDEN(lds[((slot) * K + LIP_LO) * nthreads], lds[((slot) * K + LIP_HI) * nthreads]);
        pc += 2;
        break;
      }
      case D_REVOLVE_PRE: {
        KLOOP {
          [[maybe_unused]] P3& p = pv[kp];
          [[maybe_unused]] float& R = Rv[kp];
          float x = hypotf_(p.x, p.z) - PF(0);
          p.x = x;
        }
        pc += 2;
        break;
      }
      case D_SCREW_PRE: {
        float th[K];
#ifdef GSDF_NO_XYCACHE
        xyc = nullptr;
#endif
        if (!LIP && xyc != nullptr && sh_xy && sh_col && xyc->pc == pc) {
          KLOOP th[kp] = xyc->th;
        } else {
          atan2_shared<K>(pv, th, sh_xy, brick, sh_col);
          if (!LIP && xyc != nullptr && sh_xy && sh_col) { xyc->th = th[0]; xyc->pc = pc; }
        }
        ENSURE_HXY();
        {
          const float pitch = PF(0), lead = PF(1), L = PF(2), tanTaper = PF(3), halfp = PF(4), rpitch = PF(5);
          const float twopi = 6.2831853071795862f, rtwopi = 0.15915493667125702f;
          float n1[K], q1[K], xs[K], t[K];
          KLOOP n1[kp] = lead * th[kp];
          div_uniform_k<K>(n1, twopi, rtwopi, q1);
          KLOOP xs[kp] = (pv[kp].z + q1[kp]) + halfp;
          div_uniform_k<K>(xs, pitch, rpitch, t);
          KLOOP {
            [[maybe_unused]] P3& p = pv[kp];
            float y0 = hxy[kp];
            y0 += p.z * tanTaper;
            float x0 = pitch * (t[kp] - floorf_(t[kp])) - halfp;
            LDSF(slot) = absf(p.z) - L;
            p.x = x0; p.y = y0;
          }
          if (LIP) {
            LIP_WIDEN(lds[((slot) * K + LIP_LO) * nthreads], lds[((slot) * K + LIP_HI) * nthreads]);
            lipR = minf(lipR * lip_screw(hxy[0], lipR, absf(lead), tanTaper), GSDF_LIP_BIG);
          }
        }
        pc += 7;
        break;
      }
      case D_ELONGATE_PRE: {
        KLOOP {
          [[maybe_unused]] P3& p = pv[kp];
          [[maybe_unused]] float& R = Rv[kp];
          float qx = absf(p.x) - PF(0), qy = absf(p.y) - PF(1), qz = absf(p.z) - PF(2);
          LDSF(slot) = minf(maxf(qx, maxf(qy, qz)), 0.f);
          p.x = maxf(qx, 0.f); p.y = maxf(qy, 0.f); p.z = maxf(qz, 0.f);
        }
        if (LIP) LIP_WIDEN(lds[((slot) * K + LIP_LO) * nthreads], lds[((slot) * K + LIP_HI) * nthreads]);
        pc += 4;
        break;
      }
      case D_ELONGATE2D_PRE: {
        KLOOP {
          [[maybe_unused]] P3& p = pv[kp];
          [[maybe_unused]] float& R = Rv[kp];
          float qx = absf(p.x) - PF(0), qy = absf(p.y) - PF(1);
          LDSF(slot) = minf(maxf(qx, qy), 0.f);
          p.x = maxf(qx, 0.f); p.y = maxf(qy, 0.f);
        }
        if (LIP) LIP_WIDEN(lds[((slot) * K + LIP_LO) * nthreads], lds[((slot) * K + LIP_HI) * nthreads]);
        pc += 3;
        break;
      }
      case D_ARRAY_PRE: {
        KLOOP {
          [[maybe_unused]] P3& p = pv[kp];
          [[maybe_unused]] float& R = Rv[kp];
          float ox = LDSF(slot), oy = LDSF(slot + 1), oz = LDSF(slot + 2);
          const float sx = PF(3), sy = PF(4), sz = PF(5);
          float idx = roundf_(ox / sx), idy = roundf_(oy / sy), idz = roundf_(oz / sz);
          float o_x = signf(ox - sx * idx), o_y = signf(oy - sy * idy), o_z = signf(oz - sz * idz);
          float rx = clampf(idx + PF(0) * o_x, 0.f, PF(6));
          float ry = clampf(idy + PF(1) * o_y, 0.f, PF(7));
          float rz = clampf(idz + PF(2) * o_z, 0.f, PF(8));
          p.x = ox - sx * rx; p.y = oy - sy * ry; p.z = oz - sz * rz;
        }
        pc += 10;
        break;
      }
      case D_ARRAY2D_PRE: {
        KLOOP {
          [[maybe_unused]] P3& p = pv[kp];
          [[maybe_unused]] float& R = Rv[kp];
          float ox = LDSF(slot), oy = LDSF(slot + 1);
          const float sx = PF(2), sy = PF(3);
          float idx = roundf_(ox / sx), idy = roundf_(oy / sy);
          float o_x = signf(ox - sx * idx), o_y = signf(oy - sy * idy);
// ... 239 lines not shown
                        dz = maxf(absf(pv[kp].z - z0), absf(pv[kp].z - z1));
            m2[kp] = minf(m2[kp], dx * dx + dy * dy + dz * dz);
          }
        }
        if (LIP) {
          const float u = 1.002f * (sqrtf_(m2[0]) + lipR) + 2e-6f * (absf(pv[0].x) + absf(pv[0].y) + absf(pv[0].z)) + 1e-30f;
          KLOOP LDSF(slot) = u;
        } else {
          KLOOP LDSF(slot) = 1.001f * sqrtf_(m2[kp]) + 1e-30f;
        }
        pc = q;
        break;
      }
      case D_GATE2D: {
        GSDF_GATE_TEST((region_lb_box<K, 2>(pv, PF(0), PF(1), 0.f, PF(2), PF(3), 0.f, L)), 2, 4)
        if (far_) { GSDF_GATE_TAKEN pc += GSDF_GATE_SKIP(PU(9)); } else { pc += 11; }
        break;
      }
      case D_GATE3D: {
        GSDF_GATE_TEST((region_lb_box<K, 3>(pv, PF(0), PF(1), PF(2), PF(3), PF(4), PF(5), L)), 3, 6)
        if (far_) { GSDF_GATE_TAKEN pc += GSDF_GATE_SKIP(PU(11)); } else { pc += 13; }
        break;
      }
      case D_GATEZC: {
        GSDF_GATE_TEST((region_lb_zcyl<K>(pv, hxy, use_hxy, PF(0), PF(1), PF(2), PF(3), PF(4), PF(5), PF(6), L)), 3, 7)
        if (far_) { GSDF_GATE_TAKEN pc += GSDF_GATE_SKIP(PU(12)); } else { pc += 14; }
        break;
      }
      case D_GATEOB: {
        GSDF_GATE_TEST((region_lb_obox<K, 3>(pv, PF(0), PF(1), PF(2), PF(3), PF(4), PF(5), PF(6), PF(7), L)), 3, 8)
        if (far_) { GSDF_GATE_TAKEN pc += GSDF_GATE_SKIP(PU(13)); } else { pc += 15; }
        break;
      }
      case D_CIRC_ORDER: {
        if (!LIP) {
          const float d1 = pv[0].x * PF(0) + pv[0].y * PF(1);
          const float d0 = lds[((slot) * K) * nthreads] * PF(0) + lds[((slot + 1) * K) * nthreads] * PF(1);
          const uint64_t v0 = __builtin_amdgcn_ballot_w64(d0 > d1), v1 = __builtin_amdgcn_ballot_w64(d1 > d0);
          if (__builtin_popcountll(v0) > __builtin_popcountll(v1)) {
            KLOOP {
              const float tx = LDSF(slot), ty = LDSF(slot + 1);
              LDSF(slot) = pv[kp].x; LDSF(slot + 1) = pv[kp].y;
              pv[kp].x = tx; pv[kp].y = ty;
            }
          }
        }
        pc += 7;
        break;
      }
      case D_LIP_PUSH: {
        if (LIP) {
          lds[((lip_base + slot) * K) * nthreads] = lipR;
          lds[((lip_base + slot) * K + LIP_HI) * nthreads] = absf(pv[0].x) + absf(pv[0].y) + absf(pv[0].z);
        }
        pc += 1;
        break;
      }
      case D_LIP_POP: { if (LIP) lipR = lds[((lip_base + slot) * K) * nthreads]; pc += 1; break; }
      case D_LIP_MUL: { if (LIP) lipR = minf(lipR * PF(0), GSDF_LIP_BIG); pc += 2; break; }
      case D_LIP_WRAP: { if (LIP) { if (absf(pv[0].x) + lipR >= PF(0)) lipR = lipR + PF(1); } pc += 3; break; }
      default:
        if (op == D_SKIP) {
        const uint32_t sw = PU(2);
        if (!LIP && ((bmask >> (PU(0) & 31u)) & 1u) != 0u) {
          if (use_hxy) xy_shared<K>(pv, hxy, sh_xy, brick, [](float x, float y) { return dm::hypotf_(x, y); }, sh_col);
          KLOOP Rv[kp] = PF(1);
          pc += GSDF_GATE_SKIP(sw);
        } else {
          pc += 4;
        }
          break;
        }
        if (op == D_LIP_DOM) {
          GSDF_LIP_DOM_BODY
          pc += 6;
          break;
        }
        if (op == D_LIP_SEAM) {
          GSDF_LIP_SEAM_BODY
          pc += 2;
          break;
        }
        KLOOP Rv[kp] = __builtin_nanf("");
        return;
    }
    if (LIP && op >= D_SPHERE && op <= D_LINES2D) LIP_WIDEN(Rv[LIP_LO], Rv[LIP_HI]);
  }
#undef PF
#undef PU
}
#else
}
#include "gsdf_spec_gen.h"
namespace gsdf_dev {
#endif

#undef ENSURE_HXY
#undef LDSF
#undef KLOOP
#undef LIP_WIDEN
#undef LIP_LO
#undef LIP_HI
#undef GSDF_GATE_TEST
#undef GSDF_GATE_TAKEN
#undef GSDF_LIP_DOM_BODY
#undef GSDF_LIP_SEAM_BODY

}
```

### gsdf_amd/csrc/kernels_octree.h

```cpp
#pragma once
#include "kernels_common.h"

#define PRUNE_STAGE 1024
__global__ void __launch_bounds__(BLOCK) prune_kernel(const uint32_t* __restrict__ code_g, const Cube* __restrict__ in,
                                                      unsigned long long in_cap, int expand, int level, int ncols, int lip_base, float ox,
                                                      float oy, float oz, float res,
                                                      int do_test, Cube* __restrict__ out, unsigned long long out_cap,
                                                      int shard_here, unsigned shard_rank, unsigned shard_count,
                                                      MeshCounters* __restrict__ ctr, const unsigned* __restrict__ spec_part,
                                                      unsigned spec_rows, int spec_top_S, unsigned spec_mask) {
  code_ptr code = as_code(code_g);
  float* lds = g_smem + threadIdx.x;
  if (spec_part != nullptr && blockIdx.x == 0) {
    __shared__ unsigned s_sum[16];
    if (threadIdx.x < 16u) s_sum[threadIdx.x] = 0u;
    __syncthreads();
    unsigned acc = 0;
    for (unsigned r = threadIdx.x >> 4; r < spec_rows; r += BLOCK / 16) acc += spec_part[r * 16u + (threadIdx.x & 15u)];
    if (acc) atomicAdd(&s_sum[threadIdx.x & 15u], acc);
    __syncthreads();
    if (threadIdx.x < 16u) {
      const int j = (int)(threadIdx.x >> 1), top = spec_top_S & 0xff, S = spec_top_S >> 8, lv = top - j;
      if (j < S) {
        if (threadIdx.x & 1u) ctr->n_pass[lv] = (unsigned long long)s_sum[threadIdx.x];
        else if (lv >= 3 && ((spec_mask >> lv) & 1u) != 0u) ctr->n_items[lv] = (unsigned long long)s_sum[threadIdx.x];
      }
    }
  }
  Cube* s_q = (Cube*)(g_smem + (size_t)(ncols > 0 ? ncols : 1) * 2 * BLOCK);
  unsigned* s_w = (unsigned*)(s_q + PRUNE_STAGE);
  unsigned long long* s_base = (unsigned long long*)(s_w + 8);
  unsigned long long n_in = expand ? uniform_u64(ctr->n_level[level + 1]) : 0ull;
  if (n_in > in_cap) n_in = in_cap;
  const unsigned long long n_items = expand ? n_in * 8ull : 1ull;
  if (blockIdx.x == 0 && threadIdx.x == 0) ctr->n_items[level] = do_test ? n_items : 0ull;
  const float size = (float)(1 << (level - 1)) * res;
  const float maxDist = size * (1.73205080757f / 2);
  const uint64_t step = (uint64_t)gridDim.x * BLOCK;
  const unsigned lane = threadIdx.x & 63, wave = threadIdx.x >> 6;
  unsigned long long my_pass = 0;
  unsigned cur = 0;
  auto flush = [&]() {
    if (threadIdx.x == 0) *s_base = atomicAdd(&ctr->n_level[level], (unsigned long long)cur);
    __syncthreads();
    const unsigned long long fb = *s_base;
    if (fb + cur <= out_cap) {
      for (unsigned k = threadIdx.x; k < cur; k += BLOCK) out[fb + k] = s_q[k];
    } else if (threadIdx.x == 0) {
      ctr->q_overflow = 1ull;
    }
    __syncthreads();
    cur = 0;
  };
  for (uint64_t base = (uint64_t)blockIdx.x * BLOCK; base < n_items; base += step) {
    const uint64_t i = base + threadIdx.x;
    const bool valid = i < n_items;
    Cube c = {0, 0, 0, 0};
    if (valid && expand) {
      const Cube pc = in[i >> 3];
      const unsigned k = (unsigned)(i & 7);
      c.x = (uint16_t)(pc.x * 2 + ((k ^ (k >> 1)) & 1));
      c.y = (uint16_t)(pc.y * 2 + ((k >> 1) & 1));
      c.z = (uint16_t)(pc.z * 2 + ((k >> 2) & 1));
    }
    const dm::lane_pred pvalid = dm::pred(valid);
    dm::lane_pred pkeep = pvalid;
    if (do_test) {
      const float cx0 = ox + size * (float)c.x, cy0 = oy + size * (float)c.y, cz0 = oz + size * (float)c.z;
      P3 p;
      p.x = 0.5f * (cx0 + (cx0 + size));
      p.y = 0.5f * (cy0 + (cy0 + size));
      p.z = 0.5f * (cz0 + (cz0 + size));
      P3 pv[2] = {p, p};
      float dv[2];
      if (do_test == 2) {
        gsdf_dev::sdf_eval<2>(code, pv, dv, lds, BLOCK);
        pkeep = pvalid & ~nb::abs_ge_p(dv[0], maxDist);
      } else {
        uint32_t fired = 0u;
        gsdf_dev::sdf_eval<2, 0, true>(code, pv, dv, lds, BLOCK, false, maxDist, (uint32_t)lip_base, 0u, &fired);
        pkeep = pvalid & ~(dm::pred(nb::ge0(dv[0])) | dm::pred(nb::le0(dv[1])));
        c.w = (uint16_t)fired;
      }
    }
    const unsigned long long pm = pkeep.wave;
    if (lane == 0) my_pass += (unsigned long long)__builtin_popcountll(pm);
    if (shard_here) pkeep = pkeep & dm::pred(brick_owner(c.x, c.y, c.z, shard_count) == shard_rank);
    const bool keep = pkeep.lane;
    const unsigned long long km = pkeep.wave;
    const unsigned lane_prefix = __builtin_amdgcn_mbcnt_hi((unsigned)(km >> 32), __builtin_amdgcn_mbcnt_lo((unsigned)km, 0u));
    if (lane == 0) s_w[wave] = (unsigned)__builtin_popcountll(km);
    __syncthreads();
    const unsigned w0 = s_w[0], w1 = s_w[1], w2 = s_w[2], w3 = s_w[3];
    const unsigned total = w0 + w1 + w2 + w3;
    const unsigned wpre = (wave > 0 ? w0 : 0u) + (wave > 1 ? w1 : 0u) + (wave > 2 ? w2 : 0u);
    if (cur + total > PRUNE_STAGE) flush();
    if (keep) s_q[cur + wpre + lane_prefix] = c;
    cur += total;
    __syncthreads();
  }
  if (cur) flush();
  if (shard_here) {
    if (lane == 0) s_w[4 + wave] = (unsigned)my_pass;
    __syncthreads();
    if (threadIdx.x == 0) {
      const unsigned long long t = (unsigned long long)s_w[4] + s_w[5] + s_w[6] + s_w[7];
      if (t) atomicAdd(&ctr->n_pass[level], t);
    }
  }
}

__device__ __forceinline__ unsigned spec_level_of(unsigned i, unsigned& k) {
  unsigned j = 0, off = 0, n = 1;
  while (i >= off + n) { off += n; n <<= 3; j++; }
  k = i - off;
  return j;
}
__device__ __forceinline__ Cube spec_cube(unsigned j, unsigned k) {
  unsigned x = 0, y = 0, z = 0;
  for (unsigned d = 0; d < j; d++) {
    const unsigned c = (k >> (3u * (j - 1u - d))) & 7u;
    x = 2u * x + ((c ^ (c >> 1)) & 1u);
    y = 2u * y + ((c >> 1) & 1u);
    z = 2u * z + ((c >> 2) & 1u);
  }
  Cube c = {(uint16_t)x, (uint16_t)y, (uint16_t)z, 0};
  return c;
}
__global__ void __launch_bounds__(BLOCK) prune_spec_kernel(const uint32_t* __restrict__ code_g, int top, unsigned n_spec, int ncols,
                                                           int lip_base, float ox, float oy, float oz, float res, unsigned test_mask,
                                                           int ptest, int shard_level, unsigned shard_rank, unsigned shard_count,
                                                           uint8_t* __restrict__ pass, unsigned* __restrict__ clear_p, unsigned clear_words,
                                                           uint16_t* __restrict__ mask16 ,
                                                           unsigned mask_off ) {
  code_ptr code = as_code(code_g);
  float* lds = g_smem + threadIdx.x;
  (void)ncols;
  const unsigned step = gridDim.x * BLOCK;
  for (unsigned k = blockIdx.x * BLOCK + threadIdx.x; k < clear_words; k += step) clear_p[k] = 0u;
  for (unsigned base = blockIdx.x * BLOCK; base < n_spec; base += step) {
    const unsigned i = base + threadIdx.x;
    const bool valid = i < n_spec;
    unsigned k = 0;
    const unsigned j = spec_level_of(valid ? i : 0u, k);
    const int level = top - (int)j;
    const Cube c = spec_cube(j, k);
    const bool tested = level >= 3 && ((test_mask >> level) & 1u) != 0u;
    const float size = (float)(1 << (level - 1)) * res;
    const float maxDist = size * (1.73205080757f / 2);
    const float cx0 = ox + size * (float)c.x, cy0 = oy + size * (float)c.y, cz0 = oz + size * (float)c.z;
    P3 p;
    p.x = 0.5f * (cx0 + (cx0 + size));
    p.y = 0.5f * (cy0 + (cy0 + size));
    p.z = 0.5f * (cz0 + (cz0 + size));
    P3 pv[2] = {p, p};
    float dv[2];
    bool keep;
    if (ptest == 2) {
      gsdf_dev::sdf_eval<2>(code, pv, dv, lds, BLOCK);
      keep = !nb::abs_ge(dv[0], maxDist);
    } else {
      uint32_t fired = 0u;
      gsdf_dev::sdf_eval<2, 0, true>(code, pv, dv, lds, BLOCK, false, maxDist, (uint32_t)lip_base, 0u, &fired);
      keep = !(nb::ge0(dv[0]) || nb::le0(dv[1]));
      if (mask16 != nullptr && valid && tested && i >= mask_off) mask16[i - mask_off] = (uint16_t)fired;
    }
    if (!tested) keep = true;
    const bool own = level != shard_level || brick_owner(c.x, c.y, c.z, shard_count) == shard_rank;
    if (valid) pass[i] = (uint8_t)((keep ? 1u : 0u) | (own ? 2u : 0u));
  }
}

#define SPEC_STAGE 2048
__global__ void __launch_bounds__(BLOCK) prune_resolve_kernel(const uint8_t* __restrict__ pass, int top, int S, unsigned n_spec,
                                                              unsigned test_mask, Cube* __restrict__ out, unsigned long long out_cap,
                                                              MeshCounters* __restrict__ ctr, unsigned* __restrict__ part,
                                                              const uint16_t* __restrict__ mask16 ) {
  __shared__ Cube s_q[SPEC_STAGE];
  __shared__ unsigned s_n, s_items[8], s_pass[8];
  __shared__ unsigned long long s_base;
  if (threadIdx.x == 0) s_n = 0;
  if (threadIdx.x < 8) { s_items[threadIdx.x] = 0; s_pass[threadIdx.x] = 0; }
  __syncthreads();
  const unsigned per = (n_spec + gridDim.x - 1) / gridDim.x;
  const unsigned i0 = blockIdx.x * per, i1 = i0 + per < n_spec ? i0 + per : n_spec;
  for (unsigned base = i0; base < i1; base += BLOCK) {
    const unsigned i = base + threadIdx.x;
    if (i >= i1) continue;
    unsigned k = 0;
    const unsigned j = spec_level_of(i, k);
    unsigned anc = 1u;
    unsigned kk = k, off = i - k;
    for (unsigned a = j; a > 0; a--) {
      kk >>= 3;
      off = (off - 1u) >> 3;
      anc &= pass[off + kk] == 3u ? 1u : 0u;
    }
    const unsigned me = pass[i];
    if (anc) {
      atomicAdd(&s_items[j], 1u);
      if (me & 1u) atomicAdd(&s_pass[j], 1u);
      if (me == 3u && (int)j == S - 1) {
        const unsigned slot = atomicAdd(&s_n, 1u);
        if (slot < SPEC_STAGE) {
          Cube c = spec_cube(j, k);
          if (mask16 != nullptr) c.w = mask16[k];
          s_q[slot] = c;
        }
      }
    }
  }
  __syncthreads();
  const unsigned n = s_n;
  if (threadIdx.x == 0) {
    s_base = n ? atomicAdd(&ctr->n_level[top - (S - 1)], (unsigned long long)n) : 0ull;
    if (part != nullptr) {
      for (int j = 0; j < 8; j++) { part[blockIdx.x * 16u + 2u * j] = s_items[j]; part[blockIdx.x * 16u + 2u * j + 1u] = s_pass[j]; }
    } else {
      for (int j = 0; j < S && j < 8; j++) {
        const int level = top - j;
        const bool tested = level >= 3 && ((test_mask >> level) & 1u) != 0u;
        if (s_items[j] && tested) atomicAdd(&ctr->n_items[level], (unsigned long long)s_items[j]);
        if (s_pass[j]) atomicAdd(&ctr->n_pass[level], (unsigned long long)s_pass[j]);
      }
    }
    if (n > SPEC_STAGE) ctr->q_overflow = 1ull;
  }
  __syncthreads();
  const unsigned long long fb = s_base;
  if (fb + n <= out_cap) {
    for (unsigned q = threadIdx.x; q < n && q < SPEC_STAGE; q += BLOCK) out[fb + q] = s_q[q];
  } else if (threadIdx.x == 0) {
    ctr->q_overflow = 1ull;
  }
}

__device__ __forceinline__ void mc_interp(float ax, float ay, float az, float bx, float by, float bz, float v1, float v2,
                                          float& rx, float& ry, float& rz) {
  const float eps = 1e-12f;
  const bool c1 = dm::absf(0.f - v1) < eps, c2 = dm::absf(0.f - v2) < eps;
  float t = 0.5f;
  if (!c1 || !c2) t = (0.f - v1) / (v2 - v1);
  float x = ax + t * (bx - ax), y = ay + t * (by - ay), z = az + t * (bz - az);
  if (c1 && !c2) { x = ax; y = ay; z = az; }
  if (c2 && !c1) { x = bx; y = by; z = bz; }
  rx = x; ry = y; rz = z;
}

#define REC_BLOCK (64 * REC_WORDS)
#define MARCH_GROUP 64
#define PSUM_PACK(r, t, a, z) ((unsigned long long)(r) | ((unsigned long long)(t) << 20) | ((unsigned long long)(a) << 36) | ((unsigned long long)(z) << 50))
#define PSUM_REC(v) ((unsigned)((v) & 0xfffffull))
#define PSUM_TRI(v) ((unsigned)(((v) >> 20) & 0xffffull))
#define PSUM_ACT(v) ((unsigned)(((v) >> 36) & 0x3fffull))
#define PSUM_ROWS(v) ((unsigned)((v) >> 50))

template <bool NTLDS, bool ROWS>
__device__ __forceinline__ void leaf_block_tail(const float (&dc)[8], unsigned index, dm::lane_pred pass , unsigned nact, unsigned zrows, uint32_t lxy,
                                                uint32_t lz, uint64_t blk, unsigned long long n_blocks_cap, const uint8_t* s_nt,
                                                uint32_t* __restrict__ hdr, uint32_t* __restrict__ rec, unsigned long long* __restrict__ psum) {
  const dm::lane_pred pcut = pass & dm::pred(index != 0u) & dm::pred(index != 255u);
  const bool cut = pcut.lane;
  const unsigned long long cm = pcut.wave;
  const unsigned rank = __builtin_amdgcn_mbcnt_hi((unsigned)(cm >> 32), __builtin_amdgcn_mbcnt_lo((unsigned)cm, 0u));
  if (blk < n_blocks_cap) {
    unsigned ntri = 0;
#ifndef GSDF_EXP_NO_NTRI
    if (cm != 0ull) {
      unsigned nt = 0u;
      if (NTLDS) { if (cut) nt = (unsigned)s_nt[index]; }
      else { if (cut) nt = (unsigned)GSDF_MC_NTRI[index]; }
      ntri = (unsigned)__builtin_popcountll(__ballot((nt & 1u) != 0u)) + 2u * (unsigned)__builtin_popcountll(__ballot((nt & 2u) != 0u)) +
             4u * (unsigned)__builtin_popcountll(__ballot((nt & 4u) != 0u));
    }
#endif
    if ((threadIdx.x & 63u) == 0u) {
      const uint32_t nrec = (uint32_t)__builtin_popcountll(cm);
      hdr[blk] = nrec | (ntri << 8);
#ifndef GSDF_EXP_NO_PSUM
      if (ROWS) atomicAdd(&psum[blk / MARCH_GROUP], PSUM_PACK(nrec, ntri, nact, zrows));
      else if (nact) atomicAdd(&psum[blk / MARCH_GROUP], PSUM_PACK(nrec, ntri, nact, 0u));
#endif
    }
    if (cut) {
      uint2* w = (uint2*)(rec + blk * REC_BLOCK + rank * REC_WORDS);
      w[0] = make_uint2(__float_as_uint(dc[0]), __float_as_uint(dc[1]));
      w[1] = make_uint2(__float_as_uint(dc[2]), __float_as_uint(dc[3]));
      w[2] = make_uint2(__float_as_uint(dc[4]), __float_as_uint(dc[5]));
      w[3] = make_uint2(__float_as_uint(dc[6]), __float_as_uint(dc[7]));
      w[4] = make_uint2(lxy, lz | (index << 16));
    }
  }
}

template <int K, int WAVES, bool UCUBE = true, bool NTLDS = true, bool BOTH = false, bool DZ = false>
__global__ void __launch_bounds__(BLOCK, WAVES) leaf_eval_kernel(const uint32_t* __restrict__ code_g, const Cube* __restrict__ cubes,
                                                          unsigned long long cube_cap, int lq, int nslots, float ox, float oy, float oz,
                                                          float res, uint32_t* __restrict__ hdr, uint32_t* __restrict__ rec,
                                                          unsigned long long* __restrict__ psum, unsigned long long n_blocks_cap,
                                                          MeshCounters* __restrict__ ctr,
                                                          unsigned mask_valid ) {
  code_ptr code = as_code(code_g);
  float* lds = g_smem + threadIdx.x;
  uint8_t* s_nt = (uint8_t*)(g_smem + (size_t)(nslots * K > 8 ? nslots * K : 8) * BLOCK);
  const int sh = UCUBE ? 2 : lq - 1;
  const unsigned lane = threadIdx.x & 63u;
  const unsigned wave_off = __builtin_amdgcn_readfirstlane(threadIdx.x & ~63u);
  const uint8_t nt0 = NTLDS ? GSDF_MC_NTRI[threadIdx.x] : (uint8_t)0;
  unsigned long long cw_first = 0ull;
  if (UCUBE) {
    uint64_t ci = ((uint64_t)blockIdx.x * BLOCK + wave_off) >> (3 * sh);
    if (ci >= cube_cap) ci = cube_cap - 1;
    cw_first = *(const unsigned long long*)(cubes + ci);
  }
  unsigned long long n_cubes = ctr->n_level[lq];
  cw_first = uniform_u64(cw_first);
  n_cubes = uniform_u64(n_cubes);
  if (NTLDS) {
    s_nt[threadIdx.x] = nt0;
    __syncthreads();
  }
  const float cubeDiag = 2 * 1.73205080757f * res;
  if (n_cubes > cube_cap) n_cubes = cube_cap;
  const uint64_t n_leaves = uniform_u64(n_cubes << (3 * sh));
  unsigned my_cont = 0;
  const uint64_t step = (uint64_t)gridDim.x * BLOCK;
  auto cube_word = [&](uint64_t b) -> unsigned long long {
    if (b >= n_leaves) return 0ull;
    return *(const unsigned long long*)(cubes + (b >> (3 * sh)));
  };
  unsigned long long cw_next = cw_first;
  for (uint64_t base = (uint64_t)blockIdx.x * BLOCK + (UCUBE ? wave_off : 0u); base < n_leaves; base += step) {
    const uint64_t i = base + (UCUBE ? lane : threadIdx.x);
    const bool valid = UCUBE ? true : i < n_leaves;
    Cube lf = {0, 0, 0, 0};
    uint32_t lxy = 0u, lz = 0u;
    unsigned nact = 0;
    unsigned zrows = 8u;
    const unsigned long long cw = cw_next;
    if (UCUBE) cw_next = cube_word(base + step);
    if (!UCUBE && valid) {
      const Cube pc = cubes[i >> (3 * sh)];
      const unsigned l = (unsigned)(i & ((1u << (3 * sh)) - 1u));
      const unsigned m = (1u << sh) - 1u;
      lf.x = (uint16_t)((pc.x << sh) + (l & m));
      lf.y = (uint16_t)((pc.y << sh) + ((l >> sh) & m));
      lf.z = (uint16_t)((pc.z << sh) + ((l >> (2 * sh)) & m));
      lxy = (uint32_t)lf.x | ((uint32_t)lf.y << 16);
      lz = (uint32_t)lf.z;
    }
    unsigned index = 0;
    dm::lane_pred pass = {false, 0ull};
    float dc[8];
    if (UCUBE) {
      const unsigned bx = ((unsigned)(cw & 0xffffu)) << 2, by = ((unsigned)((cw >> 16) & 0xffffu)) << 2, bz = ((unsigned)((cw >> 32) & 0xffffu)) << 2;
      const float xa = ox + res * (float)(uint16_t)(bx + ((lane & 7u) >> 1)), ya = oy + res * (float)(uint16_t)(by + (lane >> 4));
      const float px = (lane & 1u) ? xa + res : xa, py = (lane & 8u) ? ya + res : ya;
      const uint32_t bmask = mask_valid ? (__builtin_amdgcn_readfirstlane((uint32_t)(cw >> 48)) | GSDF_BRICK_MASK_VALID) : 0u;
      float dall[8];
#pragma unroll
      for (int j = 0; j < 8; j++) dall[j] = 0.f;
      gsdf_dev::XYCache xyc;
#define GSDF_COLUMN_PASS                                                     \
  {                                                                          \
    P3 pk[K];                                                                \
    float dk[K];                                                             \
    _Pragma("unroll") for (int kp = 0; kp < K; kp++) {                       \
      const unsigned r = c0 + kp;                          \
      const float za = oz + res * (float)(uint16_t)(bz + (r >> 1));          \
      pk[kp].x = px;                                                         \
      pk[kp].y = py;                                                         \
      pk[kp].z = (r & 1u) ? za + res : za;                                   \
    }                                                                        \
    gsdf_dev::sdf_eval<K, 2>(code, pk, dk, lds, BLOCK, true, 0.0f, 0u, bmask, nullptr, &xyc); \
    _Pragma("unroll") for (int j = 0; j < 8 - K; j++) dall[j] = dall[j + K]; \
    _Pragma("unroll") for (int kp = 0; kp < K; kp++) dall[8 - K + kp] = dk[kp]; \
  }
      unsigned rowmask = 0xffu, nrows = 8u;
      if (DZ && K == 4) {
        unsigned mism = 0u;
#pragma unroll
        for (unsigned k = 1; k < 4; k++) {
          const float far = (oz + res * (float)(uint16_t)(bz + k - 1u)) + res, near = oz + res * (float)(uint16_t)(bz + k);
          mism |= (__float_as_uint(far) != __float_as_uint(near) ? 1u : 0u) << (k - 1u);
        }
        mism = __builtin_amdgcn_readfirstlane(mism);
#ifdef GSDF_EXP_DZ_FORCE
        mism = GSDF_EXP_DZ_FORCE;
#endif
        rowmask = 0xabu | ((mism & 1u) << 2) | ((mism & 2u) << 3) | ((mism & 4u) << 4);
        nrows = (unsigned)__builtin_popcount(rowmask);
        zrows = nrows;
        unsigned rowsw = 0u, mr = rowmask;
#pragma unroll
        for (unsigned sl = 0; sl < 8; sl++) {
          const unsigned r = mr ? (unsigned)__builtin_ctz(mr) : 7u;
          mr &= mr - 1u;
          rowsw |= r << (4u * sl);
        }
#define GSDF_ROWS_PASS(KK, NIB0, D0)                                                        \
  {                                                                                          \
    P3 pk[KK];                                                                               \
    float dk[KK];                                                                            \
    _Pragma("unroll") for (int kp = 0; kp < KK; kp++) {                                      \
      const unsigned r = (rowsw >> (4u * ((NIB0) + (unsigned)kp))) & 7u;   \
      const float za = oz + res * (float)(uint16_t)(bz + (r >> 1));                          \
      pk[kp].x = px;                                                                         \
      pk[kp].y = py;                                                                         \
      pk[kp].z = (r & 1u) ? za + res : za;                                                   \
    }                                                                                        \
    gsdf_dev::sdf_eval<KK, 2>(code, pk, dk, lds, BLOCK, true, 0.0f, 0u, bmask, nullptr, &xyc); \
    _Pragma("unroll") for (int kp = 0; kp < KK; kp++) dall[(D0) + kp] = dk[kp];              \
  }
        if (BOTH) {
          GSDF_ROWS_PASS(4, 0u, 0)
          if (nrows <= 5u) GSDF_ROWS_PASS(1, 4u, 4)
          else if (nrows == 6u) GSDF_ROWS_PASS(2, 4u, 4)
          else GSDF_ROWS_PASS(4, 4u, 4)
        } else {
          const unsigned np4 = nrows > 6u ? 2u : 1u;
#pragma unroll 1
          for (unsigned pz = 0; pz < np4; pz++) {
#pragma unroll
            for (int j = 0; j < 4; j++) dall[j] = dall[j + 4];
            GSDF_ROWS_PASS(4, 4u * pz, 4)
          }
          if (np4 == 1u) {
#pragma unroll
            for (int j = 0; j < 4; j++) dall[j] = dall[j + 4];
            GSDF_ROWS_PASS(2, 4u, 4)
          }
        }
#undef GSDF_ROWS_PASS
      } else if (BOTH) {
#ifdef GSDF_EXP_ROWS
#pragma unroll
        for (unsigned c0 = 0; c0 < GSDF_EXP_ROWS; c0 += K) GSDF_COLUMN_PASS
#else
#pragma unroll
        for (unsigned c0 = 0; c0 < 8; c0 += K) GSDF_COLUMN_PASS
#endif
      } else {
#pragma unroll 1
        for (unsigned c0 = 0; c0 < 8; c0 += K) GSDF_COLUMN_PASS
      }
#undef GSDF_COLUMN_PASS
      float* D = g_smem + wave_off;
      const unsigned wcol = lane ^ ((lane >> 3) & 1u);
#pragma unroll
      for (int r = 0; r < 8; r++) D[r * BLOCK + wcol] = dall[r];
      __builtin_amdgcn_wave_barrier();
      const unsigned li = lane & 3u, lj = (lane >> 2) & 3u, lk = lane >> 4;
      const unsigned rcol = 16u * lj + 2u * li;
#pragma unroll
      for (int c = 0; c < 8; c++) {
        const unsigned cy = (c >> 1) & 1u, cz = (c >> 2) & 1u;
        unsigned row = 2u * lk + cz;
        if (DZ && K == 4) row = (unsigned)__builtin_popcount(rowmask & ((2u << row) - 1u)) - 1u;
        dc[c] = D[row * BLOCK + rcol + cy * 8u + (c & 1u)];
        index |= (nb::lt0(dc[c]) ? 1u : 0u) << c;
      }
      lxy = ((bx & 0xffffu) | ((by & 0xffffu) << 16)) | (li | (lj << 16));
      lz = (bz & 0xffffu) | lk;
      pass = nb::abs_le_p(dc[0], cubeDiag);
      nact = (unsigned)__builtin_popcountll(pass.wave);
    } else {
      const float x0 = ox + res * (float)lf.x, y0 = oy + res * (float)lf.y, z0 = oz + res * (float)lf.z;
      const float x1 = x0 + res, y1 = y0 + res, z1 = z0 + res;
      float dall[8];
#pragma unroll
      for (int j = 0; j < 8; j++) dall[j] = 0.f;
#pragma unroll 1
      for (unsigned c0 = 0; c0 < 8; c0 += K) {
        P3 pk[K];
        float dk[K];
#pragma unroll
        for (int kp = 0; kp < K; kp++) {
          const unsigned c = (0x62735140u >> (4u * (c0 + kp))) & 7u;
          pk[kp].x = ((c ^ (c >> 1)) & 1u) ? x1 : x0;
          pk[kp].y = ((c >> 1) & 1u) ? y1 : y0;
          pk[kp].z = ((c >> 2) & 1u) ? z1 : z0;
        }
        gsdf_dev::sdf_eval<K, true>(code, pk, dk, lds, BLOCK, false);
#pragma unroll
        for (int j = 0; j < 8 - K; j++) dall[j] = dall[j + K];
#pragma unroll
        for (int kp = 0; kp < K; kp++) {
          const unsigned c = (0x62735140u >> (4u * (c0 + kp))) & 7u;
          dall[8 - K + kp] = dk[kp];
          index |= (nb::lt0(dk[kp]) ? 1u : 0u) << c;
        }
        if (c0 == 0) {
          const dm::lane_pred pvalid = dm::pred(valid);
          pass = pvalid & nb::abs_le_p(dk[0], cubeDiag);
          if (pass.wave == 0ull) break;
          nact = (unsigned)__builtin_popcountll(pass.wave);
          my_cont += (unsigned)__builtin_popcountll(pvalid.wave);
        }
      }
      dc[0] = dall[0]; dc[1] = dall[2]; dc[2] = dall[6]; dc[3] = dall[4]; dc[4] = dall[1]; dc[5] = dall[3]; dc[6] = dall[7]; dc[7] = dall[5];
    }
    const uint64_t blk = UCUBE ? base >> 6 : uniform_u64((base + (uint64_t)(threadIdx.x & ~63u)) >> 6);
    leaf_block_tail<NTLDS, DZ && UCUBE && K == 4>(dc, index, pass, nact, zrows, lxy, lz, blk, n_blocks_cap, s_nt, hdr, rec, psum);
  }
  if (!UCUBE) {
    unsigned* s_stat = (unsigned*)g_smem;
    __syncthreads();
    if ((threadIdx.x & 63u) == 0u) s_stat[threadIdx.x >> 6] = my_cont;
    __syncthreads();
    if (threadIdx.x == 0) {
      const unsigned long long c = (unsigned long long)s_stat[0] + s_stat[1] + s_stat[2] + s_stat[3];
      if (c) atomicAdd(&ctr->n_cont, c);
    }
  }
}

template <int WAVES, bool NTLDS, bool TAILS>
__global__ void __launch_bounds__(BLOCK, WAVES) leaf_dense_kernel(const uint32_t* __restrict__ code_g, const Cube* __restrict__ cubes,
                                                                  unsigned long long cube_cap, int nslots, float ox, float oy, float oz, float res,
                                                                  uint32_t* __restrict__ hdr, uint32_t* __restrict__ rec,
                                                                  unsigned long long* __restrict__ psum, unsigned long long n_blocks_cap,
                                                                  MeshCounters* __restrict__ ctr, unsigned mask_valid ) {
  code_ptr code = as_code(code_g);
  float* lds = g_smem + threadIdx.x;
  const size_t cols = (size_t)(nslots * 4 > 8 ? nslots * 4 : 8) * BLOCK;
  uint8_t* s_nt = (uint8_t*)(g_smem + cols);
  float* s_D = g_smem + cols + (NTLDS ? 64 : 0);
  float* s_val = s_D + 4 * 512;
  unsigned* s_pts = (unsigned*)(s_val + 4 * 24);
  const unsigned lane = threadIdx.x & 63u, wave = threadIdx.x >> 6;
  float* D = s_D + wave * 512;
  float* val = s_val + wave * 24;
  if (NTLDS) s_nt[threadIdx.x] = GSDF_MC_NTRI[threadIdx.x];
  unsigned long long n_cubes = uniform_u64(ctr->n_level[3]);
  if (NTLDS) __syncthreads();
  if (n_cubes > cube_cap) n_cubes = cube_cap;
  const float cubeDiag = 2 * 1.73205080757f * res;
  const float org[3] = {ox, oy, oz};
  unsigned my_points = 0;
  const uint64_t step = (uint64_t)gridDim.x * 4;
  for (uint64_t brick = (uint64_t)blockIdx.x * 4 + wave; brick < n_cubes; brick += step) {
    const unsigned long long cw = uniform_u64(*(const unsigned long long*)(cubes + brick));
    const unsigned pidx[3] = {(unsigned)(cw & 0xffffu), (unsigned)((cw >> 16) & 0xffffu), (unsigned)((cw >> 32) & 0xffffu)};
    const uint32_t bmask = mask_valid ? ((uint32_t)(cw >> 48) | GSDF_BRICK_MASK_VALID) : 0u;
    unsigned mb[3], nax[3];
#pragma unroll
    for (int ax = 0; ax < 3; ax++) {
      const unsigned i0 = pidx[ax] * 4u;
      unsigned m = 0;
#pragma unroll
      for (unsigned k = 1; k < 4; k++) {
        const float far = (org[ax] + res * (float)(uint16_t)(i0 + k - 1u)) + res, near = org[ax] + res * (float)(uint16_t)(i0 + k);
        m |= (__float_as_uint(far) != __float_as_uint(near) ? 1u : 0u) << (k - 1u);
      }
      mb[ax] = __builtin_amdgcn_readfirstlane(m);
      nax[ax] = 5u + (unsigned)__builtin_popcount(mb[ax]);
// ... 604 lines not shown
```

### gsdf_amd/csrc/specialize.cpp

```cpp
#include "specialize.h"

#include <hip/hiprtc.h>

#include <fcntl.h>
#include <spawn.h>
#include <sys/stat.h>
#include <sys/wait.h>
#include <unistd.h>

extern char** environ;

#include <cstdio>
#include <cstdlib>
#include <cstring>

#include "dev_ops.h"
#include "embedded_src.inc"

namespace gsdf_dev {

namespace {

struct Ins { uint32_t pc, w, op; };

std::vector<Ins> decode(const Program& p) {
  std::vector<Ins> out;
  uint32_t pc = 0;
  const size_t n = p.code.size();
  while (pc < n) {
    const uint32_t w = p.code[pc], op = w & D_OP_MASK;
    if (op >= D_OP_COUNT) break;
    if (op == D_END) break;
    out.push_back({pc, w, op});
    if (op == D_POLY2D) {
      const uint32_t nv = p.code[pc + 1] & 0x7fffffffu;
      pc = ((pc + 4u + 7u) & ~7u) + 8u * nv;
    } else if (op == D_LINES2D) {
      pc += 3u + 5u * p.code[pc + 1];
    } else if (op == D_UBOUND2D || op == D_UBOUND3D) {
      pc += 2u + (op == D_UBOUND2D ? 4u : 6u) * p.code[pc + 1];
    } else {
      pc += 1u + kDevOpParams[op];
    }
  }
  return out;
}

}

int spec_instruction_count(const Program& p) { return (int)decode(p).size(); }

int spec_xy_shared_weight(const Program& p) {
  int w = 0;
  for (const Ins& in : decode(p))
    if ((in.w & D_FLAG_SHXY) && in.op != D_SKIP) w += (in.op == D_SCREW_PRE || in.op == D_CIRC_PRE) ? 4 : 1;
  return w;
}

std::string spec_source(const Program& p) {
  std::string s;
  s.reserve(1 << 16);
  char buf[256];
  s += "// generated by specialize.cpp for one lowered program -- sdf_eval<K, SHARE> without fetch/decode\n#pragma once\n";
  s += "namespace gsdf_dev {\n";
  snprintf(buf, sizeof buf, "static constexpr uint32_t kSpecCode[%zu] = {", p.code.size() ? p.code.size() : (size_t)1);
  s += buf;
  for (size_t i = 0; i < p.code.size(); i++) {
    snprintf(buf, sizeof buf, "%s0x%xu", i ? "," : "", p.code[i]);
    s += buf;
    if ((i & 15) == 15) s += "\n";
  }
  if (p.code.empty()) s += "0u";
  s += "};\n";
  s += "template <int K, int SHARE = 0, bool LIP = false>\n"
       "__device__ __forceinline__ void sdf_eval(code_ptr code, P3 (&pv)[K], float (&Rv)[K], float* __restrict__ lds,\n"
       "                                         const uint32_t nthreads, const bool brick = false,\n"
       "                                         const float lip_h = 0.0f, const uint32_t lip_base = 0u,\n"
       "                                         const uint32_t bmask_w = 0u, uint32_t* lip_fired = nullptr, XYCache* xyc = nullptr) {\n"
       "  using namespace dm;\n"
       "  static_assert(!LIP || (K == 2 && SHARE == 0), \"interval mode: two points per lane\");\n"
       "  (void)code; (void)lds; (void)nthreads; (void)brick; (void)lip_base; (void)bmask_w; (void)lip_fired; (void)xyc;\n"
       "  [[maybe_unused]] float lipR = lip_h;\n"
       "  [[maybe_unused]] const dm::uniform_word bmask{bmask_w};  // (its bit tests stay scalar: dev_math.h)\n"
       "  KLOOP Rv[kp] = 0.0f;\n"
       "  float hxy[K];\n"
       "  KLOOP hxy[kp] = 0.0f;\n"
       "#define PU(k) (kSpecCode[pc + 1 + (k)])\n"
       "#define PF(k) __uint_as_float(PU(k))\n";
  std::vector<uint32_t> close_at;
  for (const Ins& in : decode(p)) {
    while (!close_at.empty() && close_at.back() == in.pc) { s += "  }}  // end of gated child\n"; close_at.pop_back(); }
    if (in.op == D_GATE2D || in.op == D_GATE3D || in.op == D_GATEZC || in.op == D_GATEOB) {
      const uint32_t np = kDevOpParams[in.op];
      const uint32_t skip = GSDF_GATE_SKIP(p.code[in.pc + np]);
      snprintf(buf, sizeof buf, "  {  // %u %s -> %u\n    constexpr uint32_t pc = %uu, w = 0x%xu, slot = w >> 16; (void)pc;\n", in.pc, kOpName[in.op],
               in.pc + skip, in.pc, in.w);
      s += buf;
      s += "    constexpr bool use_hxy = (w & D_FLAG_HXY) != 0u; (void)use_hxy;\n";
      if (in.op == D_GATE2D) s += "    GSDF_GATE_TEST((region_lb_box<K, 2>(pv, PF(0), PF(1), 0.f, PF(2), PF(3), 0.f, L)), 2, 4)\n";
      else if (in.op == D_GATE3D) s += "    GSDF_GATE_TEST((region_lb_box<K, 3>(pv, PF(0), PF(1), PF(2), PF(3), PF(4), PF(5), L)), 3, 6)\n";
      else if (in.op == D_GATEOB) s += "    GSDF_GATE_TEST((region_lb_obox<K, 3>(pv, PF(0), PF(1), PF(2), PF(3), PF(4), PF(5), PF(6), PF(7), L)), 3, 8)\n";
      else s += "    GSDF_GATE_TEST((region_lb_zcyl<K>(pv, hxy, use_hxy, PF(0), PF(1), PF(2), PF(3), PF(4), PF(5), PF(6), L)), 3, 7)\n";
      s += "    if (far_) GSDF_GATE_TAKEN else {\n";
      close_at.push_back(in.pc + skip);
      continue;
    }
    if (in.op == D_SKIP) {
      const uint32_t skip = GSDF_GATE_SKIP(p.code[in.pc + 3]);
      snprintf(buf, sizeof buf, "  {  // %u D_SKIP %u -> %u\n    constexpr uint32_t pc = %uu, w = 0x%xu; (void)pc;\n", in.pc, p.code[in.pc + 1], in.pc + skip, in.pc, in.w);
      s += buf;
      s += "    constexpr bool use_hxy = (w & D_FLAG_HXY) != 0u, sh_xy = SHARE != 0 && K >= 2 && (w & D_FLAG_SHXY) != 0u, sh_col = SHARE == 2;\n"
           "    (void)use_hxy; (void)sh_xy; (void)sh_col;\n"
           "    if (!LIP && ((bmask >> (PU(0) & 31u)) & 1u) != 0u) {\n"
           "      if (use_hxy) xy_shared<K>(pv, hxy, sh_xy, brick, [](float x, float y) { return dm::hypotf_(x, y); }, sh_col);\n"
           "      KLOOP Rv[kp] = PF(1);\n"
           "    } else {\n";
      close_at.push_back(in.pc + skip);
      continue;
    }
    if (in.op == D_LIP_DOM) {
      snprintf(buf, sizeof buf, "  {  // %u D_LIP_DOM\n    constexpr uint32_t pc = %uu, w = 0x%xu, slot = w >> 16; (void)pc; (void)slot;\n", in.pc, in.pc, in.w);
      s += buf;
      s += "    constexpr bool swap_ab = (w & D_FLAG_SWAP) != 0u; (void)swap_ab;\n    GSDF_LIP_DOM_BODY\n  }\n";
      continue;
    }
    if (in.op == D_LIP_SEAM) {
      snprintf(buf, sizeof buf, "  {  // %u D_LIP_SEAM\n    constexpr uint32_t pc = %uu, w = 0x%xu, slot = w >> 16; (void)pc; (void)slot;\n", in.pc, in.pc, in.w);
      s += buf;
      s += "    GSDF_LIP_SEAM_BODY\n  }\n";
      continue;
    }
    const char* body = kOpBody[in.op];
    if (!body) continue;
    snprintf(buf, sizeof buf, "  {  // %u %s\n    constexpr uint32_t pc = %uu, w = 0x%xu;\n", in.pc, kOpName[in.op], in.pc, in.w);
// ... 419 lines not shown
```

### gsdf_amd/hip.py

```python
import ctypes as C
import os
import numpy as np

from ._ctypes_common import GsdfTree

_HERE = os.path.dirname(os.path.abspath(__file__))
LIB_PATH = os.path.join(_HERE, "csrc", "libgsdfhip.so")
_LIB = None

ErrEmptyBuffers = "empty buffers"
ErrMismatchBufferLength = "position and distance buffer length mismatch"

SYMBOLS = ["gsdf_hip_last_error", "gsdf_hip_init", "gsdf_hip_program_create", "gsdf_hip_program_destroy",
           "gsdf_hip_program_bounds", "gsdf_hip_program_is2d", "gsdf_hip_program_info", "gsdf_hip_evaluations", "gsdf_hip_lower", "gsdf_hip_lower_region", "gsdf_hip_eval3_submit", "gsdf_hip_eval_wait", "gsdf_hip_host_alloc", "gsdf_hip_host_register", "gsdf_hip_host_release", "gsdf_hip_comm_unique_id", "gsdf_hip_comm_create", "gsdf_hip_comm_rank", "gsdf_hip_comm_world", "gsdf_hip_comm_allreduce_sum_u64", "gsdf_hip_mesh_gatherv", "gsdf_hip_mesh_gatherv_start", "gsdf_hip_mesh_gatherv_wait", "gsdf_hip_comm_destroy", "gsdf_hip_selftest_div", "gsdf_hip_selftest_sqrt", "gsdf_hip_selftest_circ", "gsdf_hip_selftest_atan2", "gsdf_hip_selftest_cossin", "gsdf_hip_selftest_math", "gsdf_hip_mesh_minecraft", "gsdf_hip_blockcache_create", "gsdf_hip_blockcache_reset", "gsdf_hip_blockcache_eval3", "gsdf_hip_blockcache_hits", "gsdf_hip_blockcache_evaluations", "gsdf_hip_blockcache_destroy", "gsdf_hip_program_specialize", "gsdf_hip_program_specialize_async", "gsdf_hip_program_specialize_poll", "gsdf_hip_program_is_specialized", "gsdf_hip_program_kernels", "gsdf_hip_specialize_source", "gsdf_hip_specialize_check",
           "gsdf_hip_eval3", "gsdf_hip_eval2", "gsdf_hip_eval3_dev", "gsdf_hip_eval2_dev", "gsdf_hip_normals3", "gsdf_hip_image2", "gsdf_hip_image2_color", "gsdf_hip_picture_size", "gsdf_hip_color_iq", "gsdf_hip_color_gradient", "gsdf_hip_view_orbit", "gsdf_hip_render3",
           "gsdf_hip_mesh_octree", "gsdf_hip_mesh_dualcontour", "gsdf_hip_mesh_flat", "gsdf_hip_mesh_stats_get", "gsdf_hip_mesh_read", "gsdf_hip_mesh_dev_tris",
           "gsdf_hip_mesh_stl", "gsdf_hip_mesh_host_tris", "gsdf_hip_mesh_host_stl", "gsdf_hip_mesh_destroy", "gsdf_hip_brick_owner", "gsdf_hip_slab_range",
           "gsdf_hip_mesh_payload", "gsdf_hip_mesh_march", "gsdf_hip_mesh_stage_ms", "gsdf_hip_mesh_octree_start", "gsdf_hip_mesh_octree_wait", "gsdf_hip_comm_transport", "gsdf_hip_gather_plan",
           "gsdf_hip_mesh_read_records", "gsdf_hip_mesh_weld", "gsdf_hip_indexed_counts", "gsdf_hip_indexed_stats_get", "gsdf_hip_indexed_read",
           "gsdf_hip_indexed_normals", "gsdf_hip_indexed_read_normals", "gsdf_hip_indexed_ply", "gsdf_hip_indexed_host_ply", "gsdf_hip_indexed_destroy",
           "gsdf_hip_indexed_create", "gsdf_hip_indexed_report", "gsdf_hip_indexed_shells", "gsdf_hip_indexed_read_shell_of", "gsdf_hip_indexed_extract",
           "gsdf_hip_indexed_simplify", "gsdf_hip_indexed_simplify_adaptive", "gsdf_hip_indexed_clean", "gsdf_hip_indexed_project", "gsdf_hip_indexed_read_fit", "gsdf_hip_mesh_dualcontour_indexed",
           "gsdf_hip_raycast3", "gsdf_hip_indexed_thickness",
           "gsdf_hip_contour2", "gsdf_hip_slice3", "gsdf_hip_contour_counts", "gsdf_hip_contour_read", "gsdf_hip_contour_stats_get", "gsdf_hip_contour_destroy",
           "gsdf_hip_contour_create", "gsdf_hip_contour_simplify", "gsdf_hip_contour_measures", "gsdf_hip_contour_measures_ms"]


PRUNE_ASSUME_SDF = 1 << 30


GATHER_ALL, GATHER_ROOT, GATHER_NONE = 0, 1, 2
PAYLOAD_TRIANGLES, PAYLOAD_RECORDS = 0, 1
GOP_COPY, GOP_SEND, GOP_RECV = 0, 1, 2


class GatherOp(C.Structure):
    _fields_ = [("kind", C.c_int32), ("peer", C.c_int32), ("src_off", C.c_uint64), ("dst_off", C.c_uint64), ("bytes", C.c_uint64)]


class GatherStats(C.Structure):
    _fields_ = [("ms_counts", C.c_double), ("ms_payload", C.c_double), ("bytes_sent", C.c_uint64), ("bytes_received", C.c_uint64),
                ("ms_march", C.c_double)]


class MeshOpts(C.Structure):
    _fields_ = [("prune", C.c_int), ("shard_rank", C.c_int), ("shard_count", C.c_int), ("max_tris", C.c_uint64),
                ("stream", C.c_void_p), ("share_corners", C.c_int), ("host_output", C.c_int), ("payload", C.c_int), ("reserved", C.c_int)]


class GsdfView(C.Structure):
    _fields_ = [("ro", C.c_float * 3), ("uu", C.c_float * 3), ("vv", C.c_float * 3), ("ww", C.c_float * 3), ("char_dist", C.c_float),
                ("aa", C.c_int32), ("max_steps", C.c_int32), ("reserved", C.c_int32)]


class GsdfColor2(C.Structure):
    _fields_ = [("kind", C.c_int32), ("length", C.c_float), ("c0", C.c_uint8 * 4), ("c1", C.c_uint8 * 4), ("reserved", C.c_int32 * 4)]


COLOR_DEFAULT, COLOR_IQ, COLOR_GRADIENT, COLOR_BW_SMOOTH = 0, 1, 2, 3


class MeshStats(C.Structure):
    _fields_ = [("n_tris", C.c_uint64), ("evals", C.c_uint64), ("pruned_leaves", C.c_uint64), ("leaf_cubes", C.c_uint64),
                ("active_leaves", C.c_uint64), ("levels", C.c_int), ("origin", C.c_float * 3), ("res", C.c_float),
                ("ms_total", C.c_double), ("ms_prune", C.c_double), ("ms_leaf", C.c_double), ("ms_march", C.c_double),
                ("evals_prune", C.c_uint64), ("evals_leaf", C.c_uint64), ("ms_emit", C.c_double), ("cut_leaves", C.c_uint64)]


class IndexedStats(C.Structure):
    _fields_ = [("ms_keys", C.c_double), ("ms_insert", C.c_double), ("ms_number", C.c_double), ("ms_ply", C.c_double),
                ("probes", C.c_uint64), ("table_cells", C.c_uint64), ("attempts", C.c_int32), ("has_normals", C.c_int32)]
# ... 131 lines not shown
    def result_bytes(self):
        return bytes(self)[:self.RESULT_BYTES]


LOOP_MEASURE_DTYPE = np.dtype([("area", "<f8"), ("length", "<f8"), ("bbox", "<f4", (4,)), ("n_verts", "<u4"), ("layer", "<u4")])
LAYER_MEASURE_DTYPE = np.dtype([("area", "<f8"), ("length", "<f8"), ("bbox", "<f4", (4,)), ("n_loops", "<u4"), ("n_verts", "<u4")])


SHELL_DTYPE = np.dtype([("n_verts", "<u8"), ("n_tris", "<u8"), ("nonfinite", "<u8"), ("edges", "<u8"), ("boundary_edges", "<u8"),
                        ("nonmanifold_edges", "<u8"), ("misoriented_edges", "<u8"), ("euler", "<i8"), ("area", "<f8"), ("volume", "<f8"),
                        ("centroid", "<f8", (3,)), ("bbox", "<f4", (6,)), ("label", "<u4"), ("reserved", "<u4")])
SHELL_NONE = 0xffffffff


class HipError(RuntimeError):
    def __init__(self, code, msg):
        super().__init__(f"gsdf_hip error {code}: {msg}")
        self.code = code
        self.msg = msg


def lib():
    global _LIB
    if _LIB is None:
        if not os.path.exists(LIB_PATH):
            raise ImportError(f"{LIB_PATH} is missing: the HIP extension must be built "
                              "(python -c 'import __graft_entry__ as g; g.build()'); there is no CPU fallback")
        L = C.CDLL(LIB_PATH)
        L.gsdf_hip_last_error.restype = C.c_char_p
        L.gsdf_hip_init.argtypes = [C.c_int]
        L.gsdf_hip_program_create.argtypes = [C.POINTER(GsdfTree), C.POINTER(C.c_void_p)]
        L.gsdf_hip_program_destroy.argtypes = [C.c_void_p]
        L.gsdf_hip_program_destroy.restype = None
        L.gsdf_hip_program_bounds.argtypes = [C.c_void_p, C.POINTER(C.c_float)]
        L.gsdf_hip_program_is2d.argtypes = [C.c_void_p]
        L.gsdf_hip_program_info.argtypes = [C.c_void_p, C.POINTER(C.c_uint32), C.POINTER(C.c_uint32)]
        L.gsdf_hip_lower.argtypes = [C.POINTER(GsdfTree), C.c_void_p, C.c_uint32, C.POINTER(C.c_uint32), C.POINTER(C.c_uint32)]
        L.gsdf_hip_lower_region.argtypes = [C.POINTER(GsdfTree), C.c_uint32, C.POINTER(C.c_int), C.POINTER(C.c_float)]
        L.gsdf_hip_comm_unique_id.argtypes = [C.c_void_p]
        L.gsdf_hip_comm_create.argtypes = [C.c_void_p, C.c_int, C.c_int, C.POINTER(C.c_void_p)]
        L.gsdf_hip_comm_rank.argtypes = [C.c_void_p]
        L.gsdf_hip_comm_world.argtypes = [C.c_void_p]
        L.gsdf_hip_comm_allreduce_sum_u64.argtypes = [C.c_void_p, C.POINTER(C.c_uint64), C.c_size_t]
        L.gsdf_hip_mesh_gatherv.argtypes = [C.c_void_p, C.c_void_p, C.POINTER(C.c_void_p), C.POINTER(C.c_uint64)]
        L.gsdf_hip_mesh_gatherv_start.argtypes = [C.c_void_p, C.c_void_p, C.c_int, C.c_int, C.POINTER(C.c_void_p)]
        L.gsdf_hip_mesh_gatherv_wait.argtypes = [C.c_void_p, C.POINTER(C.c_void_p), C.POINTER(C.c_uint64), C.POINTER(GatherStats)]
        L.gsdf_hip_comm_destroy.argtypes = [C.c_void_p]
        L.gsdf_hip_comm_transport.restype = C.c_char_p
        L.gsdf_hip_comm_transport.argtypes = [C.c_void_p]
        L.gsdf_hip_gather_plan.argtypes = [C.POINTER(C.c_uint64), C.c_int, C.c_int, C.c_int, C.c_int, C.POINTER(GatherOp), C.c_size_t,
                                           C.POINTER(C.c_size_t), C.POINTER(C.c_uint64)]
        L.gsdf_hip_mesh_payload.argtypes = [C.c_void_p, C.POINTER(C.c_uint64), C.POINTER(C.c_uint64)]
        L.gsdf_hip_mesh_march.argtypes = [C.c_void_p]
        L.gsdf_hip_mesh_stage_ms.argtypes = [C.c_void_p, C.POINTER(C.c_double), C.POINTER(C.c_char_p), C.c_int, C.POINTER(C.c_int)]
        L.gsdf_hip_eval3_submit.argtypes = [C.c_void_p, C.c_void_p, C.c_size_t, C.c_size_t, C.c_void_p, C.c_size_t, C.POINTER(C.c_int)]
        L.gsdf_hip_eval_wait.argtypes = [C.c_void_p, C.c_int]
        L.gsdf_hip_host_alloc.restype = C.c_void_p
        L.gsdf_hip_host_alloc.argtypes = [C.c_size_t]
        L.gsdf_hip_host_register.argtypes = [C.c_void_p, C.c_size_t]
        L.gsdf_hip_host_release.argtypes = [C.c_void_p]
        L.gsdf_hip_selftest_div.argtypes = [C.c_float, C.POINTER(C.c_uint64), C.POINTER(C.c_uint64), C.POINTER(C.c_float)]
        L.gsdf_hip_selftest_sqrt.argtypes = [C.POINTER(C.c_uint64)]
        L.gsdf_hip_selftest_circ.argtypes = [C.c_float, C.POINTER(C.c_uint64), C.POINTER(C.c_uint64)]
        L.gsdf_hip_selftest_atan2.argtypes = [C.c_int, C.c_int, C.POINTER(C.c_uint64), C.POINTER(C.c_uint64)]
        L.gsdf_hip_selftest_cossin.argtypes = [C.POINTER(C.c_uint64), C.POINTER(C.c_uint64)]
        L.gsdf_hip_selftest_math.argtypes = [C.c_int, C.c_void_p, C.c_void_p, C.c_void_p, C.c_uint64, C.c_float]
        L.gsdf_hip_blockcache_create.argtypes = [C.c_void_p, C.c_float, C.c_float, C.c_float, C.POINTER(C.c_void_p)]
        L.gsdf_hip_blockcache_reset.argtypes = [C.c_void_p, C.c_void_p, C.c_float, C.c_float, C.c_float]
        L.gsdf_hip_blockcache_eval3.argtypes = [C.c_void_p, C.c_void_p, C.c_size_t, C.c_size_t, C.c_void_p, C.c_size_t]
        L.gsdf_hip_blockcache_hits.restype = C.c_uint64
        L.gsdf_hip_blockcache_hits.argtypes = [C.c_void_p]
        L.gsdf_hip_blockcache_evaluations.restype = C.c_uint64
        L.gsdf_hip_blockcache_evaluations.argtypes = [C.c_void_p]
        L.gsdf_hip_blockcache_destroy.restype = None
        L.gsdf_hip_blockcache_destroy.argtypes = [C.c_void_p]
        L.gsdf_hip_program_specialize.argtypes = [C.c_void_p]
        L.gsdf_hip_program_is_specialized.argtypes = [C.c_void_p, C.POINTER(C.c_double)]
        L.gsdf_hip_program_specialize_async.argtypes = [C.c_void_p]
        L.gsdf_hip_program_specialize_poll.argtypes = [C.c_void_p, C.c_int]
        L.gsdf_hip_program_kernels.argtypes = [C.c_void_p, C.c_char_p, C.c_size_t]
        L.gsdf_hip_specialize_source.argtypes = [C.POINTER(GsdfTree), C.c_char_p, C.c_size_t, C.POINTER(C.c_size_t)]
        L.gsdf_hip_specialize_check.argtypes = [C.POINTER(GsdfTree), C.POINTER(C.c_size_t)]
        L.gsdf_hip_evaluations.restype = C.c_uint64
        L.gsdf_hip_evaluations.argtypes = [C.c_void_p]
        for f in (L.gsdf_hip_eval3, L.gsdf_hip_eval2):
            f.argtypes = [C.c_void_p, C.c_void_p, C.c_size_t, C.c_size_t, C.c_void_p, C.c_size_t]
        for f in (L.gsdf_hip_eval3_dev, L.gsdf_hip_eval2_dev):
            f.argtypes = [C.c_void_p, C.c_void_p, C.c_size_t, C.c_void_p, C.c_size_t, C.c_void_p]
        L.gsdf_hip_normals3.argtypes = [C.c_void_p, C.c_void_p, C.c_void_p, C.c_size_t, C.c_float]
        L.gsdf_hip_image2.argtypes = [C.c_void_p, C.c_int, C.c_int, C.c_void_p, C.c_void_p]
        L.gsdf_hip_image2_color.argtypes = [C.c_void_p, C.POINTER(GsdfColor2), C.c_int, C.c_int, C.c_void_p, C.c_void_p]
        L.gsdf_hip_picture_size.argtypes = [C.POINTER(C.c_float), C.c_int, C.POINTER(C.c_int)]
        L.gsdf_hip_color_iq.argtypes = [C.POINTER(C.c_float), C.c_float, C.POINTER(GsdfColor2)]
        L.gsdf_hip_color_gradient.argtypes = [C.c_float, C.POINTER(C.c_uint8), C.POINTER(C.c_uint8), C.POINTER(GsdfColor2)]
        L.gsdf_hip_view_orbit.argtypes = [C.POINTER(C.c_float), C.c_float, C.c_float, C.c_float, C.POINTER(C.c_float), C.POINTER(GsdfView)]
        L.gsdf_hip_render3.argtypes = [C.c_void_p, C.POINTER(GsdfView), C.c_int, C.c_int, C.c_void_p, C.c_void_p, C.c_void_p]
        L.gsdf_hip_mesh_octree.argtypes = [C.c_void_p, C.c_float, C.POINTER(MeshOpts), C.POINTER(C.c_void_p)]
        L.gsdf_hip_mesh_octree_start.argtypes = [C.c_void_p, C.c_float, C.POINTER(MeshOpts), C.POINTER(C.c_void_p)]
        L.gsdf_hip_mesh_octree_wait.argtypes = [C.c_void_p, C.POINTER(C.c_void_p)]
        L.gsdf_hip_mesh_dualcontour.argtypes = [C.c_void_p, C.c_float, C.c_int, C.c_int, C.c_int, C.c_void_p, C.POINTER(C.c_void_p)]
        L.gsdf_hip_mesh_flat.argtypes = [C.c_void_p, C.c_float, C.c_int, C.c_int, C.c_void_p, C.POINTER(C.c_void_p)]
        L.gsdf_hip_mesh_minecraft.argtypes = [C.c_void_p, C.c_float, C.c_void_p, C.POINTER(C.c_void_p)]
        L.gsdf_hip_mesh_stats_get.argtypes = [C.c_void_p, C.POINTER(MeshStats)]
        L.gsdf_hip_mesh_read.argtypes = [C.c_void_p, C.c_uint64, C.c_uint64, C.c_void_p]
        L.gsdf_hip_mesh_dev_tris.restype = C.c_void_p
        L.gsdf_hip_mesh_dev_tris.argtypes = [C.c_void_p]
# ... 317 lines not shown

class OctreeHIP:

    def __init__(self, sdf, res, evalBufferSize=64, prune=True, shard_rank=0, shard_count=1, max_tris=0, stream=None,
                 share_corners=False, host_output=False, assume_sdf=False, payload=PAYLOAD_TRIANGLES):
        if evalBufferSize < 64:
            raise ValueError("bad octree eval buffer size")
        self.sdf = sdf
        self._mesh = None
        self._cursor = 0
        self._opts = MeshOpts(int(prune) | (PRUNE_ASSUME_SDF if assume_sdf else 0), shard_rank, shard_count, max_tris, stream, int(share_corners), int(host_output), int(payload), 0)
        self.Reset(sdf, res)

    def Reset(self, sdf, res):
        self._free()
        self.sdf = sdf
        m = C.c_void_p()
        _check(lib().gsdf_hip_mesh_octree(sdf._h, np.float32(res), C.byref(self._opts), C.byref(m)))
        self._adopt(m)

    def _adopt(self, m):
        self._mesh = m
        self._cursor = 0
        st = MeshStats()
        _check(lib().gsdf_hip_mesh_stats_get(m, C.byref(st)))
        self.stats = st

    @classmethod
    def start(cls, sdf, res, **kw):
        self = cls.__new__(cls)
        self.sdf, self._mesh, self._cursor = sdf, None, 0
        kw.setdefault("prune", True)
        self._opts = MeshOpts(int(kw["prune"]) | (PRUNE_ASSUME_SDF if kw.get("assume_sdf") else 0), kw.get("shard_rank", 0), kw.get("shard_count", 1),
                              kw.get("max_tris", 0), kw.get("stream"), int(kw.get("share_corners", False)), int(kw.get("host_output", False)),
                              int(kw.get("payload", PAYLOAD_TRIANGLES)), 0)
        j = C.c_void_p()
        _check(lib().gsdf_hip_mesh_octree_start(sdf._h, np.float32(res), C.byref(self._opts), C.byref(j)))
        return PendingMesh(self, j)

    def _free(self):
        if getattr(self, "_mesh", None):
            lib().gsdf_hip_mesh_destroy(self._mesh)
            self._mesh = None

    def __del__(self):
        try:
            self._free()
        except Exception:
            pass

    def TotalPruned(self):
        return int(self.stats.pruned_leaves)

    def payload(self):
        n, b = C.c_uint64(), C.c_uint64()
        k = lib().gsdf_hip_mesh_payload(self._mesh, C.byref(n), C.byref(b))
        _check(min(k, 0))
        return k, int(n.value), int(b.value)

    def stage_ms(self):
        ms, names, n = (C.c_double * 8)(), (C.c_char_p * 8)(), C.c_int()
        _check(lib().gsdf_hip_mesh_stage_ms(self._mesh, ms, names, 8, C.byref(n)))
        return {names[k].decode(): float(ms[k]) for k in range(n.value)}

    def march(self):
        _check(lib().gsdf_hip_mesh_march(self._mesh))
        return self

    def records(self):
        n = C.c_uint64()
        _check(lib().gsdf_hip_mesh_read_records(self._mesh, None, 0, C.byref(n)))
        raw = np.zeros((n.value, 10), np.uint32)
        if n.value:
            _check(lib().gsdf_hip_mesh_read_records(self._mesh, raw.ctypes.data, n.value, None))
        leaf = np.stack([raw[:, 8] & 0xffff, raw[:, 8] >> 16, raw[:, 9] & 0xffff], axis=1).astype(np.int64)
        return raw[:, :8].copy().view(np.float32), leaf, (raw[:, 9] >> 16).astype(np.int64)

    def weld(self):
        h = C.c_void_p()
        _check(lib().gsdf_hip_mesh_weld(self._mesh, C.byref(h)))
        return IndexedHIP(h)

    def n_tris(self):
        return int(self.stats.n_tris)

    def dev_ptr(self):
        return lib().gsdf_hip_mesh_dev_tris(self._mesh)

    def ReadTriangles(self, dst, userData=None):
        if dst.shape[0] < 5:
            raise BufferError("short buffer")
        remaining = self.n_tris() - self._cursor
        n = min(remaining, dst.shape[0])
        if n:
            _check(lib().gsdf_hip_mesh_read(self._mesh, self._cursor, n, dst.ctypes.data))
        self._cursor += n
        return n, self._cursor >= self.n_tris()

    def RenderAll(self):
        n = self.n_tris()
        out = np.empty((n, 3, 3), np.float32)
        if n:
            _check(lib().gsdf_hip_mesh_read(self._mesh, 0, n, out.ctypes.data))
        return out

    def WriteBinarySTL(self):
# ... 534 lines not shown
```

### include/gsdf_hip.h

```cpp
#ifndef GSDF_HIP_H
#define GSDF_HIP_H
#include <stddef.h>
#include <stdint.h>

#include "gsdf_program.h"

#ifdef __cplusplus
extern "C" {
#endif

typedef enum gsdf_status {
  GSDF_OK = 0,
  GSDF_ERR_EMPTY_BUFFERS = -1,
  GSDF_ERR_LENGTH_MISMATCH = -2,
  GSDF_ERR_BAD_ARGUMENT = -3,
  GSDF_ERR_BAD_TREE = -4,
  GSDF_ERR_HIP = -5,
  GSDF_ERR_NO_DEVICE = -6,
  GSDF_ERR_DIMENSION = -7,
  GSDF_ERR_RESOLUTION = -8,
  GSDF_ERR_SHORT_BUFFER = -9,
  GSDF_ERR_CAPACITY = -10
} gsdf_status;

// ... 98 lines not shown
  int shard_count;
  uint64_t max_tris;
  void* stream;
  int share_corners;
  int host_output;
  int payload;
  int reserved;
} gsdf_mesh_opts;
#define GSDF_PAYLOAD_TRIANGLES 0
#define GSDF_PAYLOAD_RECORDS 1

typedef struct gsdf_mesh_stats {
  uint64_t n_tris;
  uint64_t evals;
  uint64_t pruned_leaves;
  uint64_t leaf_cubes;
  uint64_t active_leaves;
  int levels;
  float origin[3];
  float res;
  double ms_total;
  double ms_prune;
  double ms_leaf;
  double ms_march;
  uint64_t evals_prune;
  uint64_t evals_leaf;
  double ms_emit;
  uint64_t cut_leaves;
} gsdf_mesh_stats;

GSDF_ABI_ASSERT(sizeof(gsdf_mesh_opts) == 48, "gsdf_mesh_opts is 48 bytes");
GSDF_ABI_ASSERT(offsetof(gsdf_mesh_opts, prune) == 0 && offsetof(gsdf_mesh_opts, shard_rank) == 4 && offsetof(gsdf_mesh_opts, shard_count) == 8, "gsdf_mesh_opts head");
GSDF_ABI_ASSERT(offsetof(gsdf_mesh_opts, max_tris) == 16 && offsetof(gsdf_mesh_opts, stream) == 24, "gsdf_mesh_opts middle");
GSDF_ABI_ASSERT(offsetof(gsdf_mesh_opts, share_corners) == 32 && offsetof(gsdf_mesh_opts, host_output) == 36 && offsetof(gsdf_mesh_opts, payload) == 40, "gsdf_mesh_opts tail");
GSDF_ABI_ASSERT(sizeof(gsdf_mesh_stats) == 128, "gsdf_mesh_stats is 128 bytes");
GSDF_ABI_ASSERT(offsetof(gsdf_mesh_stats, n_tris) == 0 && offsetof(gsdf_mesh_stats, evals) == 8 && offsetof(gsdf_mesh_stats, pruned_leaves) == 16, "gsdf_mesh_stats counters");
GSDF_ABI_ASSERT(offsetof(gsdf_mesh_stats, leaf_cubes) == 24 && offsetof(gsdf_mesh_stats, active_leaves) == 32 && offsetof(gsdf_mesh_stats, levels) == 40, "gsdf_mesh_stats counters 2");
GSDF_ABI_ASSERT(offsetof(gsdf_mesh_stats, origin) == 44 && offsetof(gsdf_mesh_stats, res) == 56 && offsetof(gsdf_mesh_stats, ms_total) == 64, "gsdf_mesh_stats lattice");
GSDF_ABI_ASSERT(offsetof(gsdf_mesh_stats, ms_prune) == 72 && offsetof(gsdf_mesh_stats, ms_leaf) == 80 && offsetof(gsdf_mesh_stats, ms_march) == 88, "gsdf_mesh_stats times");
GSDF_ABI_ASSERT(offsetof(gsdf_mesh_stats, evals_prune) == 96 && offsetof(gsdf_mesh_stats, evals_leaf) == 104 && offsetof(gsdf_mesh_stats, ms_emit) == 112 && offsetof(gsdf_mesh_stats, cut_leaves) == 120, "gsdf_mesh_stats tail");
GSDF_ABI_ASSERT(GSDF_ERR_EMPTY_BUFFERS == -1 && GSDF_ERR_LENGTH_MISMATCH == -2 && GSDF_ERR_SHORT_BUFFER == -9 && GSDF_ERR_CAPACITY == -10, "status codes are part of the ABI");

int gsdf_hip_mesh_octree(gsdf_program* p, float res, const gsdf_mesh_opts* opts, gsdf_mesh** out);
typedef struct gsdf_mesh_job gsdf_mesh_job;
int gsdf_hip_mesh_octree_start(gsdf_program* p, float res, const gsdf_mesh_opts* opts, gsdf_mesh_job** job);
int gsdf_hip_mesh_octree_wait(gsdf_mesh_job* job, gsdf_mesh** out);
int gsdf_hip_mesh_dualcontour(gsdf_program* p, float res, int chiseled, int shard_rank, int shard_count, void* stream,
                              gsdf_mesh** out);
int gsdf_hip_mesh_flat(gsdf_program* p, float res, int shard_rank, int shard_count, void* stream, gsdf_mesh** out);
int gsdf_hip_mesh_minecraft(gsdf_program* p, float res, void* stream, gsdf_mesh** out);
int gsdf_hip_mesh_stats_get(const gsdf_mesh* m, gsdf_mesh_stats* st);
int gsdf_hip_mesh_stage_ms(const gsdf_mesh* m, double* ms, const char** names, int cap, int* n);
int gsdf_hip_mesh_payload(const gsdf_mesh* m, uint64_t* n_records, uint64_t* payload_bytes);
int gsdf_hip_mesh_read_records(const gsdf_mesh* m, uint32_t* dst, uint64_t dst_records, uint64_t* n_records);
int gsdf_hip_mesh_march(gsdf_mesh* m);
int gsdf_hip_mesh_read(const gsdf_mesh* m, uint64_t first, uint64_t count, float* dst);
const float* gsdf_hip_mesh_dev_tris(const gsdf_mesh* m);
int gsdf_hip_mesh_stl(const gsdf_mesh* m, uint8_t* dst, size_t dst_cap);
int gsdf_hip_mesh_host_tris(gsdf_mesh* m, const float** tris);
int gsdf_hip_mesh_host_stl(gsdf_mesh* m, const uint8_t** stl, size_t* len);
void gsdf_hip_mesh_destroy(gsdf_mesh* m);

typedef struct gsdf_indexed gsdf_indexed;
typedef struct gsdf_indexed_stats {
  double ms_keys;
  double ms_insert;
  double ms_number;
  double ms_ply;
  uint64_t probes;
  uint64_t table_cells;
  int32_t attempts;
  int32_t has_normals;
} gsdf_indexed_stats;
GSDF_ABI_ASSERT(sizeof(gsdf_indexed_stats) == 56, "gsdf_indexed_stats is 56 bytes");
int gsdf_hip_mesh_weld(const gsdf_mesh* m, gsdf_indexed** out);
int gsdf_hip_indexed_counts(const gsdf_indexed* ix, uint64_t* n_verts, uint64_t* n_tris, double* ms_device);
int gsdf_hip_indexed_stats_get(const gsdf_indexed* ix, gsdf_indexed_stats* st);
int gsdf_hip_indexed_read(const gsdf_indexed* ix, float* verts, uint32_t* idx, uint64_t* keys);
int gsdf_hip_indexed_normals(gsdf_indexed* ix, gsdf_program* p, float step);
int gsdf_hip_indexed_read_normals(const gsdf_indexed* ix, float* normals);
int gsdf_hip_indexed_ply(gsdf_indexed* ix, uint8_t* dst, size_t cap, size_t* len);
int gsdf_hip_indexed_host_ply(gsdf_indexed* ix, const uint8_t** ply, size_t* len);
void gsdf_hip_indexed_destroy(gsdf_indexed* ix);

typedef struct gsdf_indexed_report {
  uint64_t n_verts, n_tris;
  uint64_t degenerate, nonfinite, used_verts;
  uint64_t edges, boundary_edges, nonmanifold_edges, misoriented_edges;
  uint64_t n_shells;
  int64_t euler;
  double area, volume, centroid[3];
  float bbox[6];
  int32_t closed_oriented;
  int32_t exponent;
  double ms_edges;
  double ms_shells;
  double ms_measure;
  uint64_t probes;
  uint64_t table_cells;
  int32_t attempts;
  int32_t reserved;
} gsdf_indexed_report;
GSDF_ABI_ASSERT(sizeof(gsdf_indexed_report) == 208, "gsdf_indexed_report is 208 bytes");
GSDF_ABI_ASSERT(offsetof(gsdf_indexed_report, degenerate) == 16 && offsetof(gsdf_indexed_report, edges) == 40 && offsetof(gsdf_indexed_report, n_shells) == 72, "gsdf_indexed_report counts");
GSDF_ABI_ASSERT(offsetof(gsdf_indexed_report, euler) == 80 && offsetof(gsdf_indexed_report, area) == 88 && offsetof(gsdf_indexed_report, centroid) == 104, "gsdf_indexed_report measures");
GSDF_ABI_ASSERT(offsetof(gsdf_indexed_report, bbox) == 128 && offsetof(gsdf_indexed_report, closed_oriented) == 152 && offsetof(gsdf_indexed_report, exponent) == 156, "gsdf_indexed_report box");
// ... 291 lines not shown
```

Baseline: 493.3 billion.

## Precompute per-cube polygon edge cull masks during pruning and reuse them in leaf eval

During interval pruning at the leaf-parent level, the compiler-chosen largest top-level 2D polygon has its per-edge keep masks computed once per cube and stored in a new emask buffer. The leaf evaluation kernel reads that word, readfirstlane'd per wave, and skips the per-brick poly_cull when it is valid. This trades extra work and memory in the prune and resolve kernels, plus seam and magnitude padding logic, for less per-leaf polygon culling. It also adds an edge_bricks stat and an opt-out environment variable.

```diff
diff --git a/gsdf_amd/csrc/abi_host.h b/gsdf_amd/csrc/abi_host.h
--- a/gsdf_amd/csrc/abi_host.h
+++ b/gsdf_amd/csrc/abi_host.h
@@ -26,6 +26,7 @@
 inline int env_int(const char* name, int dflt) { const char* e = getenv(name); return e ? atoi(e) : dflt; }
 inline uint64_t env_u64(const char* name, uint64_t dflt) { const char* e = getenv(name); return e ? (uint64_t)strtoull(e, nullptr, 10) : dflt; }
 inline bool env_flag(const char* name) { const char* e = getenv(name); return e && atoi(e) != 0; }
+inline bool env_flag_set(const char* name) { const char* e = getenv(name); return e && atoi(e) != 0; }
 inline bool env_flag_on(const char* name) { const char* e = getenv(name); return !e || atoi(e) != 0; }
 inline bool env_set(const char* name) { return getenv(name) != nullptr; }
 
@@ -51,6 +52,7 @@
   uint64_t recs_cap36 = 0;
   uint64_t n_recs = 0;
   bool weldable = false;
+  uint64_t edge_bricks = 0;
   uint8_t* d_wrecs = nullptr;
   uint64_t wrecs_cap36 = 0;
   uint64_t n_wrecs = 0;
diff --git a/gsdf_amd/csrc/abi_mesh.hip b/gsdf_amd/csrc/abi_mesh.hip
--- a/gsdf_amd/csrc/abi_mesh.hip
+++ b/gsdf_amd/csrc/abi_mesh.hip
@@ -68,11 +68,13 @@
   bool want_recs = false;
   uint64_t qcap = 0, want = 0, want_rec_n = 0;
   int attempt = 0, slot;
-  bool ctr_on_host = false, used_dz = false, used_dense = false;
+  bool ctr_on_host = false, used_dz = false, used_dense = false, used_spec_leaf = false;
   int chain_first = 0;
   uint64_t nblk = 0, nblk_q = 0, lbound = 0;
   size_t clear_bytes = 0;
   bool masks_valid = false;
+  bool edges_valid = false;
+  uint32_t* d_emask = nullptr;
   Cube* q[2] = {nullptr, nullptr};
   uint64_t capq[2] = {0, 0};
   MeshCounters* d_ctr = nullptr;
@@ -94,6 +96,7 @@
   ctr_on_host = false;
   used_dz = false;
   used_dense = false;
+  used_spec_leaf = false;
   if (int rc = prepare_outputs()) return rc;
   if (int rc = enqueue_descent()) return rc;
   if (int rc = enqueue_leaf()) return rc;
@@ -154,6 +157,12 @@
   HIP_TRY(w.ctr.ensure(clear_bytes));
   d_ctr = (MeshCounters*)w.ctr.p;
   masks_valid = lq == 3 && ptest == 1 && p->prog.n_skip_ids > 0 && (pmask == 1 || (pmask > 1 && ((pmask >> lq) & 1)));
+  edges_valid = lq == 3 && ptest == 1 && p->prog.edge_pc != GSDF_EDGE_NONE && (pmask == 1 || (pmask > 1 && ((pmask >> lq) & 1))) && !env_flag_set("GSDF_HIP_NO_EDGE_MASKS");
+  d_emask = nullptr;
+  if (edges_valid) {
+    HIP_TRY(w.emask.ensure(capq[lq & 1] * sizeof(uint32_t)));
+    d_emask = (uint32_t*)w.emask.p;
+  }
   return GSDF_OK;
 }
 
@@ -178,7 +187,10 @@
     const unsigned n_last = 1u << (3 * (S - 1));
     const size_t mask_off_b = (part_off + (size_t)rrows * 16 * sizeof(unsigned) + 63) & ~(size_t)63;
     const bool spec_masks = masks_valid && last_spec == lq;
-    HIP_TRY(w.spec_pass.ensure(mask_off_b + (spec_masks ? (size_t)n_last * sizeof(uint16_t) : 0)));
+    const bool spec_edges = edges_valid && last_spec == lq;
+    const size_t emask_off_b = (mask_off_b + (spec_masks ? (size_t)n_last * sizeof(uint16_t) : 0) + 63) & ~(size_t)63;
+    HIP_TRY(w.spec_pass.ensure(emask_off_b + (spec_edges ? (size_t)n_last * sizeof(uint32_t) : 0)));
+    uint32_t* d_emask32 = spec_edges ? (uint32_t*)((char*)w.spec_pass.p + emask_off_b) : nullptr;
     uint16_t* d_mask16 = spec_masks ? (uint16_t*)((char*)w.spec_pass.p + mask_off_b) : nullptr;
     const bool chain_follows = last_spec - 1 >= lq;
     spec_part = chain_follows ? (unsigned*)((char*)w.spec_pass.p + part_off) : nullptr;
@@ -187,10 +199,10 @@
     spec_mask = test_mask;
     const int shard_level = opts.shard_count > 1 ? ls : -1;
     HIP_TRY(launch_kernel(prune_spec_kernel, p->spec.f_prune_spec, grid_for(n_spec, p->num_cu, 8), BLOCK, lds_prune, s, p->d_code.p, levels, n_spec, prune_cols, p->prog.nslots, ox, oy,
-                          oz, res, test_mask, ptest, shard_level, opts.shard_rank, opts.shard_count, w.spec_pass.p, (unsigned*)d_ctr, clear_bytes / 4, d_mask16, n_spec - n_last));
+                          oz, res, test_mask, ptest, shard_level, opts.shard_rank, opts.shard_count, w.spec_pass.p, (unsigned*)d_ctr, clear_bytes / 4, d_mask16, n_spec - n_last, d_emask32));
     hipLaunchKernelGGL(prune_resolve_kernel, dim3((n_spec + SPEC_STAGE - 1) / SPEC_STAGE), dim3(BLOCK), 0, s, (const uint8_t*)w.spec_pass.p, levels, S,
                        n_spec, test_mask, q[last_spec & 1], (unsigned long long)capq[last_spec & 1], d_ctr, spec_part,
-                       (const uint16_t*)d_mask16);
+                       (const uint16_t*)d_mask16, (const uint32_t*)d_emask32, d_emask32 ? d_emask : (uint32_t*)nullptr);
     HIP_TRY(hipGetLastError());
     first_level = last_spec - 1;
     chain_first = first_level;
@@ -202,7 +214,7 @@
     if (bound > capq[(level + 1) & 1] * 8) bound = capq[(level + 1) & 1] * 8;
     HIP_TRY(launch_kernel(prune_kernel, p->spec.f_prune, grid_for(bound, p->num_cu, prune_bpc), BLOCK, lds_prune, s, p->d_code.p, q[(level + 1) & 1], capq[(level + 1) & 1], expand, level,
                           prune_cols, p->prog.nslots, ox, oy, oz, res, do_test, q[level & 1], capq[level & 1], (opts.shard_count > 1 && level == ls) ? 1 : 0, opts.shard_rank,
-                          opts.shard_count, d_ctr, level == first_level ? spec_part : nullptr, spec_rows, spec_top_S, spec_mask));
+                          opts.shard_count, d_ctr, level == first_level ? spec_part : nullptr, spec_rows, spec_top_S, spec_mask, level == lq ? d_emask : (uint32_t*)nullptr));
   }
   HIP_TRY(hipEventRecord(w.ev[1], s));
   return GSDF_OK;
@@ -231,7 +243,8 @@
     const LeafPick pick = p->leaf_pick(lq, want_dz);
     used_dz = pick.v.dz;
     HIP_TRY(launch_kernel(leaf_eval_aot(pick.v), pick.f, grid, BLOCK, lq != 3 ? lds_m + 256 : lds_m, s, p->d_code.p, cubes, ncubes, lq, p->prog.nslots, ox, oy, oz, res, d_hdr, d_rec,
-                          d_psum, nblk, d_ctr, use_masks));
+                          d_psum, nblk, d_ctr, use_masks, (const uint32_t*)d_emask));
+    used_spec_leaf = pick.f != nullptr;
   }
   HIP_TRY(hipEventRecord(w.ev[3], s));
   if (want_recs) {
@@ -331,6 +344,7 @@
   m->st.ms_march = ms13;
   m->st.ms_emit = ms12 - ms13;
   m->st.cut_leaves = hc.n_cut;
+  m->edge_bricks = (edges_valid && used_spec_leaf && !used_dz && !used_dense) ? hc.n_points / 64 : 0;
   m->st.ms_total = (double)ms01 + (double)ms12;
   p->evals += m->st.evals;
   p->last_tris = hc.n_tris;
@@ -498,6 +512,8 @@
   }
   return GSDF_OK;
 }
+
+extern "C" uint64_t gsdf_hip_mesh_edge_bricks(const gsdf_mesh* m) { return m ? m->edge_bricks : 0; }
 
 extern "C" int gsdf_hip_mesh_payload(const gsdf_mesh* m, uint64_t* n_records, uint64_t* payload_bytes) {
   if (!m) return fail(GSDF_ERR_BAD_ARGUMENT, "null argument");
diff --git a/gsdf_amd/csrc/abi_program.h b/gsdf_amd/csrc/abi_program.h
--- a/gsdf_amd/csrc/abi_program.h
+++ b/gsdf_amd/csrc/abi_program.h
@@ -107,6 +107,7 @@
     Arena q0, q1;
     Arena ctr;
     Arena spec_pass;
+    Arena emask;
     Arena rec, hdr;
     Arena grp;
     EventSet<5> ev;
diff --git a/gsdf_amd/csrc/compile.cpp b/gsdf_amd/csrc/compile.cpp
--- a/gsdf_amd/csrc/compile.cpp
+++ b/gsdf_amd/csrc/compile.cpp
@@ -42,6 +42,8 @@
   int lip_push() { const int d = lip_depth++; if (lip_depth > max_lip_depth) max_lip_depth = lip_depth; op(D_LIP_PUSH, d); return d; }
   void lip_pop(int d) { op(D_LIP_POP, d); lip_depth--; }
   int discont = 0;
+  int cells = 0;
+  uint32_t edge_pc = GSDF_EDGE_NONE, edge_nv = 0;
   bool numbering = false;
   std::vector<double> cand_cost;
   std::vector<int> cand_id;
@@ -766,7 +768,7 @@
         c.f(P[0]); c.f(P[1]); c.f(P[2]);
         c.f(P[3] + -1); c.f(P[4] + -1); c.f(P[5] + -1);
         if (seams && k == 0 && j == 0 && ii == 0) { c.op(D_LIP_SEAM); c.u(seams); }
-        c.discont++; gen(c, c.child(n, 0), depth + 1); c.discont--;
+        c.discont++; c.cells++; gen(c, c.child(n, 0), depth + 1); c.cells--; c.discont--;
         c.op(D_COMBINE_MIN, slotD);
         if (!(k == 1 && j == 1 && ii == 1)) c.op(D_SAVER, slotD);
       }
@@ -839,7 +841,7 @@
       }
       if (sector_gate) { c.op(D_CIRC_ORDER, slotP); for (int j = 0; j < 6; j++) c.f(cg.b[j]); }
       if (seams) { c.op(D_LIP_SEAM, slotP); c.u(8u); }
-      c.discont++;
+      c.discont++; c.cells++;
       gen(c, c.child(n, 0), depth + 1);
       c.op(D_SAVER, slotD);
       c.load_saved(slotP, is2d);
@@ -855,7 +857,7 @@
         c.u(0);
       }
       gen(c, c.child(n, 0), depth + 1);
-      c.discont--;
+      c.discont--; c.cells--;
       if (skip_at >= 0) {
         if (c.hxyver != hxy_before) c.hxyver = 0;
         c.code[(size_t)skip_at] = (uint32_t)((long)c.code.size() - gate_pc);
@@ -892,7 +894,8 @@
       c.bump();
       c.f(P[0]); c.f(P[1]); c.f(P[2]); c.f(gsdf::tanf32(P[3])); c.f(P[0] / 2); c.f(c.node_recip(P[0]));
       c.op(D_LIP_WRAP); c.f(P[0] / 2); c.f(lip_screw_seam(*c.t, c.child(n, 0), P[0]));
-      c.discont++; gen(c, c.child(n, 0), depth + 1); c.discont--;
+      const bool lead_whole = P[0] != 0.f && std::isfinite(P[1] / P[0]) && P[1] == P[0] * std::nearbyint(P[1] / P[0]);
+      c.discont++; c.cells += lead_whole ? 0 : 1; gen(c, c.child(n, 0), depth + 1); c.cells -= lead_whole ? 0 : 1; c.discont--;
       c.lip_pop(lipd);
       c.op(D_MAXR_SLOT, s);
       c.release(1);
@@ -948,6 +951,7 @@
         }
       }
       (all_recip ? c.n_poly_recip : c.n_poly_plain)++;
+      if (c.cells == 0 && nv >= 6 && nv <= 16 && nv > c.edge_nv) { c.edge_pc = (uint32_t)c.code.size(); c.edge_nv = nv; }
       c.op(D_POLY2D); c.u(nv | (all_recip ? 0x80000000u : 0u)); c.f(v[0]); c.f(v[1]);
       while (c.code.size() % 8 != 0) c.u(0);
       uint32_t jv = nv - 1;
@@ -986,7 +990,7 @@
         c.bump();
         c.f((float)ii); c.f((float)j); c.f(P[0]); c.f(P[1]); c.f(P[2] + -1); c.f(P[3] + -1);
         if (seams && j == 0 && ii == 0) { c.op(D_LIP_SEAM); c.u(seams); }
-        c.discont++; gen(c, c.child(n, 0), depth + 1); c.discont--;
+        c.discont++; c.cells++; gen(c, c.child(n, 0), depth + 1); c.cells--; c.discont--;
         c.op(D_COMBINE_MIN, slotD);
         if (!(j == 1 && ii == 1)) c.op(D_SAVER, slotD);
       }
@@ -1156,6 +1160,7 @@
   p.nslots = c.max_slots;
   p.lip_depth = c.max_lip_depth;
   p.n_recip = c.n_recip; p.n_recip_declined = c.n_recip_declined; p.n_poly_recip = c.n_poly_recip; p.n_poly_plain = c.n_poly_plain;
+  p.edge_pc = c.edge_pc;
   p.n_skip_ids = 0;
   for (int v : cand_id) if (v >= 0) p.n_skip_ids++;
   p.is2d = gsdf_op_is2d(t.nodes[t.root].op);
diff --git a/gsdf_amd/csrc/compile.h b/gsdf_amd/csrc/compile.h
--- a/gsdf_amd/csrc/compile.h
+++ b/gsdf_amd/csrc/compile.h
@@ -12,6 +12,7 @@
   int nslots = 0;
   int lip_depth = 0;
   int n_skip_ids = 0;
+  uint32_t edge_pc = 0xffffffffu;
   bool is2d = false;
   float bb[6] = {0};
   bool has_exact_bb = false;
diff --git a/gsdf_amd/csrc/dev_ops.h b/gsdf_amd/csrc/dev_ops.h
--- a/gsdf_amd/csrc/dev_ops.h
+++ b/gsdf_amd/csrc/dev_ops.h
@@ -94,3 +94,5 @@
 #define GSDF_GATE_ID1(w) ((w) >> 24)
 #define GSDF_BRICK_MASK_VALID 0x80000000u
 #define GSDF_SKIP_BIG 1.0e30f
+#define GSDF_EDGE_UNDECIDED 0u
+#define GSDF_EDGE_NONE 0xffffffffu
diff --git a/gsdf_amd/csrc/interp.h b/gsdf_amd/csrc/interp.h
--- a/gsdf_amd/csrc/interp.h
+++ b/gsdf_amd/csrc/interp.h
@@ -156,6 +156,57 @@
   const uint64_t vm = nv >= 64u ? ~0ull : (1ull << nv) - 1ull;
   keepd = vm & ~wave_mask((dc - rb) - m > U);
   keeps = vm & ~((wave_mask(y0 >= v1y) & wave_mask(y0 >= v2y)) | (wave_mask(y1 < v1y) & wave_mask(y1 < v2y)));
+}
+
+struct EdgeBall {
+  float cx, cy;
+  float rb;
+  float pad;
+};
+__device__ __forceinline__ uint32_t poly_edge_word(code_ptr code, uint32_t q0, uint32_t nv, float cx, float cy, float rb, float pad,
+                                                   bool seam, const bool recip) {
+  using namespace dm;
+#ifdef GSDF_NO_CULL_APPROX
+  const bool approx = false;
+#else
+  const bool approx = recip;
+#endif
+  auto nonfinite = [](float v) { return __builtin_amdgcn_classf(v, 0x207); };
+  bool bad = seam || nonfinite(cx) || nonfinite(cy) || nonfinite(rb) || nonfinite(pad) || !(rb < GSDF_LIP_BIG);
+  auto edge = [&](uint32_t iv, float& dc, float& m, float& v1y, float& v2y) {
+    const f4ptr er = (f4ptr)(code + q0 + 8u * iv);
+    const v4f r0 = er[0], r1 = er[1];
+    const float v1x = r0.x, ex = r0.z, ey = r0.w, n2e = r1.x;
+    v1y = r0.y; v2y = r1.y;
+    const float wx = cx - v1x, wy = cy - v1y;
+    const float num = wx * ex + wy * ey;
+    const float t = __builtin_amdgcn_fmed3f(approx ? num * r1.z : num / n2e, 0.f, 1.f);
+    const float bx = wx - t * ex, by = wy - t * ey;
+    const float dc2 = bx * bx + by * by;
+    dc = approx ? __builtin_amdgcn_sqrtf(dc2) : sqrtf_(dc2);
+    m = 1.0e-5f * (absf(wx) + absf(wy) + absf(ex) + absf(ey) + rb + absf(cx) + absf(cy)) + pad;
+  };
+  float U = __builtin_inff();
+  float lo[16];
+  uint32_t keepd = 0u, keeps = 0u;
+#pragma unroll
+  for (uint32_t iv = 0; iv < 16u; iv++) {
+    lo[iv] = 0.0f;
+    if (iv < nv) {
+      float dc, m, v1y, v2y;
+      edge(iv, dc, m, v1y, v2y);
+      bad = bad || nonfinite(dc) || nonfinite(m);
+      U = minf(U, (dc + rb) + m);
+      lo[iv] = (dc - rb) - m;
+      const float y0 = (cy - rb) - m, y1 = (cy + rb) + m;
+      const bool above = y0 >= v1y && y0 >= v2y, below = y1 < v1y && y1 < v2y;
+      if (!(above || below)) keeps |= 1u << iv;
+    }
+  }
+#pragma unroll
+  for (uint32_t iv = 0; iv < 16u; iv++)
+    if (iv < nv && !(lo[iv] > U)) keepd |= 1u << iv;
+  return bad ? GSDF_EDGE_UNDECIDED : (keepd | (keeps << 16));
 }
 
 template <int K, typename F>
@@ -423,6 +474,18 @@
     if (LIP) { Rv[LIP_LO] = L[LIP_LO]; Rv[LIP_HI] = GSDF_SKIP_BIG; }          \
     else { KLOOP Rv[kp] = L[kp]; }                                            \
   }
+#ifdef GSDF_SPECIALIZED
+#define GSDF_EDGE_WORD(pc) ((pc) == kSpecEdgePc ? emask_w : GSDF_EDGE_UNDECIDED)
+#define GSDF_EDGE_LIP(pc) \
+  { if ((pc) == kSpecEdgePc && emask_out != nullptr) *emask_out = EdgeBall{pv[0].x, pv[0].y, edge_seam ? -1.0f : lipR, edge_pad}; }
+#define GSDF_EDGE_NOTE_SEAM() { edge_seam = true; }
+#define GSDF_EDGE_NOTE_MAG(S) { edge_pad = maxf(edge_pad, 2.0e-6f * (S)); }
+#else
+#define GSDF_EDGE_WORD(pc) GSDF_EDGE_UNDECIDED
+#define GSDF_EDGE_LIP(pc) {}
+#define GSDF_EDGE_NOTE_SEAM() {}
+#define GSDF_EDGE_NOTE_MAG(S) {}
+#endif
 #ifndef GSDF_SPECIALIZED
 template <int K, int SHARE = 0, bool LIP = false>
 __device__ __forceinline__ void sdf_eval(code_ptr code, P3 (&pv)[K], float (&Rv)[K],
@@ -431,8 +494,10 @@
                                          const float lip_h = 0.0f, const uint32_t lip_base = 0u,
                                          const uint32_t bmask_w = 0u ,
                                          uint32_t* lip_fired = nullptr ,
-                                         XYCache* xyc = nullptr ) {
+                                         XYCache* xyc = nullptr ,
+                                         const uint32_t emask_w = GSDF_EDGE_UNDECIDED, EdgeBall* emask_out = nullptr ) {
   using namespace dm;
+  (void)emask_w; (void)emask_out;
   static_assert(!LIP || (K == 2 && SHARE == 0), "interval mode: two points per lane, lower and upper bound");
   [[maybe_unused]] float lipR = lip_h;
   const dm::uniform_word bmask{bmask_w};
@@ -836,12 +901,15 @@
           if (!done1) poly_edges<1, false>(code, q0, nv, v0x, v0y, p1, d1, neg1);
           const float sd = sqrtf_(d1[0]);
           KLOOP Rv[kp] = neg1[0] ? -sd : sd;
+          GSDF_EDGE_LIP(pc)
         } else {
           float d[K];
           bool neg[K];
           bool done = false;
           uint64_t keepd = ~0ull, keeps = ~0ull;
-          if (brick && nv >= 6u && nv <= 64u) poly_cull<K>(code, q0, nv, pv, keepd, keeps, (hdr >> 31) != 0u);
+          const uint32_t ew = GSDF_EDGE_WORD(pc);
+          if (ew != GSDF_EDGE_UNDECIDED) { keepd = (uint64_t)(ew & 0xffffu); keeps = (uint64_t)(ew >> 16); }
+          else if (brick && nv >= 6u && nv <= 64u) poly_cull<K>(code, q0, nv, pv, keepd, keeps, (hdr >> 31) != 0u);
           if (hdr >> 31) done = poly_edges<K, true>(code, q0, nv, v0x, v0y, pv, d, neg, keepd, keeps);
           if (!done) poly_edges<K, false>(code, q0, nv, v0x, v0y, pv, d, neg, keepd, keeps);
           float sd[K];
@@ -1009,6 +1077,7 @@
           if (LIP) {
             LIP_WIDEN(lds[((slot) * K + LIP_LO) * nthreads], lds[((slot) * K + LIP_HI) * nthreads]);
             lipR = minf(lipR * lip_screw(hxy[0], lipR, absf(lead), tanTaper), GSDF_LIP_BIG);
+            GSDF_EDGE_NOTE_MAG(absf(xs[0]) + absf(n1[0]) + absf(pv[0].y))
           }
         }
         pc += 7;
@@ -1354,13 +1423,14 @@
         if (LIP) {
           lds[((lip_base + slot) * K) * nthreads] = lipR;
           lds[((lip_base + slot) * K + LIP_HI) * nthreads] = absf(pv[0].x) + absf(pv[0].y) + absf(pv[0].z);
+          GSDF_EDGE_NOTE_MAG(absf(pv[0].x) + absf(pv[0].y) + absf(pv[0].z))
         }
         pc += 1;
         break;
       }
       case D_LIP_POP: { if (LIP) lipR = lds[((lip_base + slot) * K) * nthreads]; pc += 1; break; }
       case D_LIP_MUL: { if (LIP) lipR = minf(lipR * PF(0), GSDF_LIP_BIG); pc += 2; break; }
-      case D_LIP_WRAP: { if (LIP) { if (absf(pv[0].x) + lipR >= PF(0)) lipR = lipR + PF(1); } pc += 3; break; }
+      case D_LIP_WRAP: { if (LIP) { if (absf(pv[0].x) + lipR >= PF(0)) { lipR = lipR + PF(1); GSDF_EDGE_NOTE_SEAM() } } pc += 3; break; }
       default:
         if (op == D_SKIP) {
         const uint32_t sw = PU(2);
@@ -1407,5 +1477,9 @@
 #undef GSDF_GATE_TAKEN
 #undef GSDF_LIP_DOM_BODY
 #undef GSDF_LIP_SEAM_BODY
-
-}
+#undef GSDF_EDGE_WORD
+#undef GSDF_EDGE_LIP
+#undef GSDF_EDGE_NOTE_SEAM
+#undef GSDF_EDGE_NOTE_MAG
+
+}
diff --git a/gsdf_amd/csrc/kernels_octree.h b/gsdf_amd/csrc/kernels_octree.h
--- a/gsdf_amd/csrc/kernels_octree.h
+++ b/gsdf_amd/csrc/kernels_octree.h
@@ -2,13 +2,31 @@
 #include "kernels_common.h"
 
 #define PRUNE_STAGE 1024
+#define PRUNE_STAGE_E 680
+__device__ __forceinline__ uint32_t edge_word_of(code_ptr code, bool keep, uint32_t fired, const gsdf_dev::EdgeBall& ball) {
+#ifdef GSDF_SPECIALIZED
+  if (gsdf_dev::kSpecEdgePc != GSDF_EDGE_NONE) {
+    constexpr uint32_t pc = gsdf_dev::kSpecEdgePc != GSDF_EDGE_NONE ? gsdf_dev::kSpecEdgePc : 0u;
+    constexpr uint32_t hdr = gsdf_dev::kSpecCode[pc + 1u], nv = hdr & 0x7fffffffu, q0 = (pc + 4u + 7u) & ~7u;
+    const dm::lane_pred want = dm::pred(keep) & dm::pred(ball.rb >= 0.0f) & dm::pred((fired & gsdf_dev::kSpecEdgeSkipMask) == 0u);
+    if (want.wave != 0ull) {
+      const uint32_t w = gsdf_dev::poly_edge_word(code, q0, nv, ball.cx, ball.cy, ball.rb, ball.pad, false, (hdr >> 31) != 0u);
+      return want.lane ? w : GSDF_EDGE_UNDECIDED;
+    }
+  }
+#endif
+  (void)code; (void)keep; (void)fired; (void)ball;
+  return GSDF_EDGE_UNDECIDED;
+}
+static_assert(PRUNE_STAGE_E * (sizeof(uint16_t) * 4 + sizeof(uint32_t)) <= PRUNE_STAGE * sizeof(uint16_t) * 4 && PRUNE_STAGE_E >= 256, "the cubes and their edge masks share the stage's block");
 __global__ void __launch_bounds__(BLOCK) prune_kernel(const uint32_t* __restrict__ code_g, const Cube* __restrict__ in,
                                                       unsigned long long in_cap, int expand, int level, int ncols, int lip_base, float ox,
                                                       float oy, float oz, float res,
                                                       int do_test, Cube* __restrict__ out, unsigned long long out_cap,
                                                       int shard_here, unsigned shard_rank, unsigned shard_count,
                                                       MeshCounters* __restrict__ ctr, const unsigned* __restrict__ spec_part,
-                                                      unsigned spec_rows, int spec_top_S, unsigned spec_mask) {
+                                                      unsigned spec_rows, int spec_top_S, unsigned spec_mask,
+                                                      uint32_t* __restrict__ eout ) {
   code_ptr code = as_code(code_g);
   float* lds = g_smem + threadIdx.x;
   if (spec_part != nullptr && blockIdx.x == 0) {
@@ -29,6 +47,8 @@
   }
   Cube* s_q = (Cube*)(g_smem + (size_t)(ncols > 0 ? ncols : 1) * 2 * BLOCK);
   unsigned* s_w = (unsigned*)(s_q + PRUNE_STAGE);
+  uint32_t* s_e = (uint32_t*)(s_q + PRUNE_STAGE_E);
+  const unsigned stage_cap = eout != nullptr ? PRUNE_STAGE_E : PRUNE_STAGE;
   unsigned long long* s_base = (unsigned long long*)(s_w + 8);
   unsigned long long n_in = expand ? uniform_u64(ctr->n_level[level + 1]) : 0ull;
   if (n_in > in_cap) n_in = in_cap;
@@ -46,6 +66,7 @@
     const unsigned long long fb = *s_base;
     if (fb + cur <= out_cap) {
       for (unsigned k = threadIdx.x; k < cur; k += BLOCK) out[fb + k] = s_q[k];
+      if (eout != nullptr) for (unsigned k = threadIdx.x; k < cur; k += BLOCK) eout[fb + k] = s_e[k];
     } else if (threadIdx.x == 0) {
       ctr->q_overflow = 1ull;
     }
@@ -56,6 +77,8 @@
     const uint64_t i = base + threadIdx.x;
     const bool valid = i < n_items;
     Cube c = {0, 0, 0, 0};
+    gsdf_dev::EdgeBall ball = {0.0f, 0.0f, -1.0f, 0.0f};
+    uint32_t fired = 0u;
     if (valid && expand) {
       const Cube pc = in[i >> 3];
       const unsigned k = (unsigned)(i & 7);
@@ -77,8 +100,7 @@
         gsdf_dev::sdf_eval<2>(code, pv, dv, lds, BLOCK);
         pkeep = pvalid & ~nb::abs_ge_p(dv[0], maxDist);
       } else {
-        uint32_t fired = 0u;
-        gsdf_dev::sdf_eval<2, 0, true>(code, pv, dv, lds, BLOCK, false, maxDist, (uint32_t)lip_base, 0u, &fired);
+        gsdf_dev::sdf_eval<2, 0, true>(code, pv, dv, lds, BLOCK, false, maxDist, (uint32_t)lip_base, 0u, &fired, nullptr, GSDF_EDGE_UNDECIDED, &ball);
         pkeep = pvalid & ~(dm::pred(nb::ge0(dv[0])) | dm::pred(nb::le0(dv[1])));
         c.w = (uint16_t)fired;
       }
@@ -94,8 +116,12 @@
     const unsigned w0 = s_w[0], w1 = s_w[1], w2 = s_w[2], w3 = s_w[3];
     const unsigned total = w0 + w1 + w2 + w3;
     const unsigned wpre = (wave > 0 ? w0 : 0u) + (wave > 1 ? w1 : 0u) + (wave > 2 ? w2 : 0u);
-    if (cur + total > PRUNE_STAGE) flush();
+    if (cur + total > stage_cap) flush();
     if (keep) s_q[cur + wpre + lane_prefix] = c;
+    if (eout != nullptr) {
+      const uint32_t eword = edge_word_of(code, keep, fired, ball);
+      if (keep) s_e[cur + wpre + lane_prefix] = eword;
+    }
     cur += total;
     __syncthreads();
   }
@@ -116,6 +142,14 @@
   k = i - off;
   return j;
 }
+__device__ __forceinline__ unsigned spec_number(unsigned j, unsigned x, unsigned y, unsigned z) {
+  unsigned k = 0;
+  for (unsigned d = 0; d < j; d++) {
+    const unsigned b = j - 1u - d, xb = (x >> b) & 1u, yb = (y >> b) & 1u, zb = (z >> b) & 1u;
+    k = (k << 3) | (zb << 2) | (yb << 1) | (xb ^ yb);
+  }
+  return k;
+}
 __device__ __forceinline__ Cube spec_cube(unsigned j, unsigned k) {
   unsigned x = 0, y = 0, z = 0;
   for (unsigned d = 0; d < j; d++) {
@@ -132,7 +166,8 @@
                                                            int ptest, int shard_level, unsigned shard_rank, unsigned shard_count,
                                                            uint8_t* __restrict__ pass, unsigned* __restrict__ clear_p, unsigned clear_words,
                                                            uint16_t* __restrict__ mask16 ,
-                                                           unsigned mask_off ) {
+                                                           unsigned mask_off ,
+                                                           uint32_t* __restrict__ emask32 ) {
   code_ptr code = as_code(code_g);
   float* lds = g_smem + threadIdx.x;
   (void)ncols;
@@ -156,14 +191,20 @@
     P3 pv[2] = {p, p};
     float dv[2];
     bool keep;
+    gsdf_dev::EdgeBall ball = {0.0f, 0.0f, -1.0f, 0.0f};
+    uint32_t fired = 0u;
     if (ptest == 2) {
       gsdf_dev::sdf_eval<2>(code, pv, dv, lds, BLOCK);
       keep = !nb::abs_ge(dv[0], maxDist);
     } else {
-      uint32_t fired = 0u;
-      gsdf_dev::sdf_eval<2, 0, true>(code, pv, dv, lds, BLOCK, false, maxDist, (uint32_t)lip_base, 0u, &fired);
+      gsdf_dev::sdf_eval<2, 0, true>(code, pv, dv, lds, BLOCK, false, maxDist, (uint32_t)lip_base, 0u, &fired, nullptr, GSDF_EDGE_UNDECIDED, &ball);
       keep = !(nb::ge0(dv[0]) || nb::le0(dv[1]));
       if (mask16 != nullptr && valid && tested && i >= mask_off) mask16[i - mask_off] = (uint16_t)fired;
+    }
+    if (emask32 != nullptr) {
+      const bool last = valid && i >= mask_off;
+      const uint32_t eword = edge_word_of(code, last && keep && tested, fired, ball);
+      if (last) emask32[i - mask_off] = eword;
     }
     if (!tested) keep = true;
     const bool own = level != shard_level || brick_owner(c.x, c.y, c.z, shard_count) == shard_rank;
@@ -175,7 +216,9 @@
 __global__ void __launch_bounds__(BLOCK) prune_resolve_kernel(const uint8_t* __restrict__ pass, int top, int S, unsigned n_spec,
                                                               unsigned test_mask, Cube* __restrict__ out, unsigned long long out_cap,
                                                               MeshCounters* __restrict__ ctr, unsigned* __restrict__ part,
-                                                              const uint16_t* __restrict__ mask16 ) {
+                                                              const uint16_t* __restrict__ mask16 ,
+                                                              const uint32_t* __restrict__ emask32 ,
+                                                              uint32_t* __restrict__ eout ) {
   __shared__ Cube s_q[SPEC_STAGE];
   __shared__ unsigned s_n, s_items[8], s_pass[8];
   __shared__ unsigned long long s_base;
@@ -230,6 +273,9 @@
   const unsigned long long fb = s_base;
   if (fb + n <= out_cap) {
     for (unsigned q = threadIdx.x; q < n && q < SPEC_STAGE; q += BLOCK) out[fb + q] = s_q[q];
+    if (emask32 != nullptr) {
+      for (unsigned q = threadIdx.x; q < n && q < SPEC_STAGE; q += BLOCK) eout[fb + q] = emask32[spec_number((unsigned)(S - 1), s_q[q].x, s_q[q].y, s_q[q].z)];
+    }
   } else if (threadIdx.x == 0) {
     ctr->q_overflow = 1ull;
   }
@@ -279,7 +325,7 @@
       hdr[blk] = nrec | (ntri << 8);
 #ifndef GSDF_EXP_NO_PSUM
       if (ROWS) atomicAdd(&psum[blk / MARCH_GROUP], PSUM_PACK(nrec, ntri, nact, zrows));
-      else if (nact) atomicAdd(&psum[blk / MARCH_GROUP], PSUM_PACK(nrec, ntri, nact, 0u));
+      else if (nact) atomicAdd(&psum[blk / MARCH_GROUP], PSUM_PACK(nrec, ntri, nact, zrows));
 #endif
     }
     if (cut) {
@@ -299,7 +345,8 @@
                                                           float res, uint32_t* __restrict__ hdr, uint32_t* __restrict__ rec,
                                                           unsigned long long* __restrict__ psum, unsigned long long n_blocks_cap,
                                                           MeshCounters* __restrict__ ctr,
-                                                          unsigned mask_valid ) {
+                                                          unsigned mask_valid ,
+                                                          const uint32_t* __restrict__ emask ) {
   code_ptr code = as_code(code_g);
   float* lds = g_smem + threadIdx.x;
   uint8_t* s_nt = (uint8_t*)(g_smem + (size_t)(nslots * K > 8 ? nslots * K : 8) * BLOCK);
@@ -308,10 +355,12 @@
   const unsigned wave_off = __builtin_amdgcn_readfirstlane(threadIdx.x & ~63u);
   const uint8_t nt0 = NTLDS ? GSDF_MC_NTRI[threadIdx.x] : (uint8_t)0;
   unsigned long long cw_first = 0ull;
+  uint32_t ew_first = GSDF_EDGE_UNDECIDED;
   if (UCUBE) {
     uint64_t ci = ((uint64_t)blockIdx.x * BLOCK + wave_off) >> (3 * sh);
     if (ci >= cube_cap) ci = cube_cap - 1;
     cw_first = *(const unsigned long long*)(cubes + ci);
+    if (emask != nullptr) ew_first = emask[ci];
   }
   unsigned long long n_cubes = ctr->n_level[lq];
   cw_first = uniform_u64(cw_first);
@@ -329,7 +378,12 @@
     if (b >= n_leaves) return 0ull;
     return *(const unsigned long long*)(cubes + (b >> (3 * sh)));
   };
+  auto edge_word = [&](uint64_t b) -> uint32_t {
+    if (emask == nullptr || b >= n_leaves) return GSDF_EDGE_UNDECIDED;
+    return emask[b >> (3 * sh)];
+  };
   unsigned long long cw_next = cw_first;
+  uint32_t ew_next = ew_first;
   for (uint64_t base = (uint64_t)blockIdx.x * BLOCK + (UCUBE ? wave_off : 0u); base < n_leaves; base += step) {
     const uint64_t i = base + (UCUBE ? lane : threadIdx.x);
     const bool valid = UCUBE ? true : i < n_leaves;
@@ -338,7 +392,8 @@
     unsigned nact = 0;
     unsigned zrows = 8u;
     const unsigned long long cw = cw_next;
-    if (UCUBE) cw_next = cube_word(base + step);
+    const uint32_t ew = (uint32_t)__builtin_amdgcn_readfirstlane((int)ew_next);
+    if (UCUBE) { cw_next = cube_word(base + step); ew_next = edge_word(base + step); }
     if (!UCUBE && valid) {
       const Cube pc = cubes[i >> (3 * sh)];
       const unsigned l = (unsigned)(i & ((1u << (3 * sh)) - 1u));
@@ -372,7 +427,7 @@
       pk[kp].y = py;                                                         \
       pk[kp].z = (r & 1u) ? za + res : za;                                   \
     }                                                                        \
-    gsdf_dev::sdf_eval<K, 2>(code, pk, dk, lds, BLOCK, true, 0.0f, 0u, bmask, nullptr, &xyc); \
+    gsdf_dev::sdf_eval<K, 2>(code, pk, dk, lds, BLOCK, true, 0.0f, 0u, bmask, nullptr, &xyc, ew); \
     _Pragma("unroll") for (int j = 0; j < 8 - K; j++) dall[j] = dall[j + K]; \
     _Pragma("unroll") for (int kp = 0; kp < K; kp++) dall[8 - K + kp] = dk[kp]; \
   }
@@ -409,7 +464,7 @@
       pk[kp].y = py;                                                                         \
       pk[kp].z = (r & 1u) ? za + res : za;                                                   \
     }                                                                                        \
-    gsdf_dev::sdf_eval<KK, 2>(code, pk, dk, lds, BLOCK, true, 0.0f, 0u, bmask, nullptr, &xyc); \
+    gsdf_dev::sdf_eval<KK, 2>(code, pk, dk, lds, BLOCK, true, 0.0f, 0u, bmask, nullptr, &xyc, ew); \
     _Pragma("unroll") for (int kp = 0; kp < KK; kp++) dall[(D0) + kp] = dk[kp];              \
   }
         if (BOTH) {
@@ -501,7 +556,8 @@
       dc[0] = dall[0]; dc[1] = dall[2]; dc[2] = dall[6]; dc[3] = dall[4]; dc[4] = dall[1]; dc[5] = dall[3]; dc[6] = dall[7]; dc[7] = dall[5];
     }
     const uint64_t blk = UCUBE ? base >> 6 : uniform_u64((base + (uint64_t)(threadIdx.x & ~63u)) >> 6);
-    leaf_block_tail<NTLDS, DZ && UCUBE && K == 4>(dc, index, pass, nact, zrows, lxy, lz, blk, n_blocks_cap, s_nt, hdr, rec, psum);
+    leaf_block_tail<NTLDS, DZ && UCUBE && K == 4>(dc, index, pass, nact, (DZ && UCUBE && K == 4) ? zrows : (UCUBE && ew != GSDF_EDGE_UNDECIDED ? 1u : 0u), lxy, lz, blk, n_blocks_cap, s_nt,
+                                                  hdr, rec, psum);
   }
   if (!UCUBE) {
     unsigned* s_stat = (unsigned*)g_smem;
diff --git a/gsdf_amd/csrc/specialize.cpp b/gsdf_amd/csrc/specialize.cpp
--- a/gsdf_amd/csrc/specialize.cpp
+++ b/gsdf_amd/csrc/specialize.cpp
@@ -72,14 +72,26 @@
   }
   if (p.code.empty()) s += "0u";
   s += "};\n";
+  snprintf(buf, sizeof buf, "static constexpr uint32_t kSpecEdgePc = 0x%xu;\n", p.edge_pc);
+  s += buf;
+  {
+    uint32_t inside = 0;
+    for (const Ins& in : decode(p))
+      if (in.op == D_SKIP && in.pc < p.edge_pc && p.edge_pc < in.pc + GSDF_GATE_SKIP(p.code[in.pc + 3])) inside |= 1u << (p.code[in.pc + 1] & 31u);
+    snprintf(buf, sizeof buf, "static constexpr uint32_t kSpecEdgeSkipMask = 0x%xu;\n", p.edge_pc == GSDF_EDGE_NONE ? 0u : inside);
+    s += buf;
+  }
   s += "template <int K, int SHARE = 0, bool LIP = false>\n"
        "__device__ __forceinline__ void sdf_eval(code_ptr code, P3 (&pv)[K], float (&Rv)[K], float* __restrict__ lds,\n"
        "                                         const uint32_t nthreads, const bool brick = false,\n"
        "                                         const float lip_h = 0.0f, const uint32_t lip_base = 0u,\n"
-       "                                         const uint32_t bmask_w = 0u, uint32_t* lip_fired = nullptr, XYCache* xyc = nullptr) {\n"
+       "                                         const uint32_t bmask_w = 0u, uint32_t* lip_fired = nullptr, XYCache* xyc = nullptr,\n"
+       "                                         const uint32_t emask_w = GSDF_EDGE_UNDECIDED, EdgeBall* emask_out = nullptr) {\n"
        "  using namespace dm;\n"
        "  static_assert(!LIP || (K == 2 && SHARE == 0), \"interval mode: two points per lane\");\n"
-       "  (void)code; (void)lds; (void)nthreads; (void)brick; (void)lip_base; (void)bmask_w; (void)lip_fired; (void)xyc;\n"
+       "  (void)code; (void)lds; (void)nthreads; (void)brick; (void)lip_base; (void)bmask_w; (void)lip_fired; (void)xyc; (void)emask_w; (void)emask_out;\n"
+       "  [[maybe_unused]] bool edge_seam = false;  // (interval mode, edge masks: interp.h, GSDF_EDGE_*)\n"
+       "  [[maybe_unused]] float edge_pad = 0.0f;\n"
        "  [[maybe_unused]] float lipR = lip_h;\n"
        "  [[maybe_unused]] const dm::uniform_word bmask{bmask_w};  // (its bit tests stay scalar: dev_math.h)\n"
        "  KLOOP Rv[kp] = 0.0f;\n"
diff --git a/gsdf_amd/hip.py b/gsdf_amd/hip.py
--- a/gsdf_amd/hip.py
+++ b/gsdf_amd/hip.py
@@ -16,7 +16,7 @@
            "gsdf_hip_eval3", "gsdf_hip_eval2", "gsdf_hip_eval3_dev", "gsdf_hip_eval2_dev", "gsdf_hip_normals3", "gsdf_hip_image2", "gsdf_hip_image2_color", "gsdf_hip_picture_size", "gsdf_hip_color_iq", "gsdf_hip_color_gradient", "gsdf_hip_view_orbit", "gsdf_hip_render3",
            "gsdf_hip_mesh_octree", "gsdf_hip_mesh_dualcontour", "gsdf_hip_mesh_flat", "gsdf_hip_mesh_stats_get", "gsdf_hip_mesh_read", "gsdf_hip_mesh_dev_tris",
            "gsdf_hip_mesh_stl", "gsdf_hip_mesh_host_tris", "gsdf_hip_mesh_host_stl", "gsdf_hip_mesh_destroy", "gsdf_hip_brick_owner", "gsdf_hip_slab_range",
-           "gsdf_hip_mesh_payload", "gsdf_hip_mesh_march", "gsdf_hip_mesh_stage_ms", "gsdf_hip_mesh_octree_start", "gsdf_hip_mesh_octree_wait", "gsdf_hip_comm_transport", "gsdf_hip_gather_plan",
+           "gsdf_hip_mesh_payload", "gsdf_hip_mesh_edge_bricks", "gsdf_hip_mesh_march", "gsdf_hip_mesh_stage_ms", "gsdf_hip_mesh_octree_start", "gsdf_hip_mesh_octree_wait", "gsdf_hip_comm_transport", "gsdf_hip_gather_plan",
            "gsdf_hip_mesh_read_records", "gsdf_hip_mesh_weld", "gsdf_hip_indexed_counts", "gsdf_hip_indexed_stats_get", "gsdf_hip_indexed_read",
            "gsdf_hip_indexed_normals", "gsdf_hip_indexed_read_normals", "gsdf_hip_indexed_ply", "gsdf_hip_indexed_host_ply", "gsdf_hip_indexed_destroy",
            "gsdf_hip_indexed_create", "gsdf_hip_indexed_report", "gsdf_hip_indexed_shells", "gsdf_hip_indexed_read_shell_of", "gsdf_hip_indexed_extract",
@@ -254,6 +254,8 @@
                                            C.POINTER(C.c_size_t), C.POINTER(C.c_uint64)]
         L.gsdf_hip_mesh_payload.argtypes = [C.c_void_p, C.POINTER(C.c_uint64), C.POINTER(C.c_uint64)]
         L.gsdf_hip_mesh_march.argtypes = [C.c_void_p]
+        L.gsdf_hip_mesh_edge_bricks.restype = C.c_uint64
+        L.gsdf_hip_mesh_edge_bricks.argtypes = [C.c_void_p]
         L.gsdf_hip_mesh_stage_ms.argtypes = [C.c_void_p, C.POINTER(C.c_double), C.POINTER(C.c_char_p), C.c_int, C.POINTER(C.c_int)]
         L.gsdf_hip_eval3_submit.argtypes = [C.c_void_p, C.c_void_p, C.c_size_t, C.c_size_t, C.c_void_p, C.c_size_t, C.POINTER(C.c_int)]
         L.gsdf_hip_eval_wait.argtypes = [C.c_void_p, C.c_int]
@@ -677,6 +679,9 @@
     def TotalPruned(self):
         return int(self.stats.pruned_leaves)
 
+    def edge_bricks(self):
+        return int(lib().gsdf_hip_mesh_edge_bricks(self._mesh))
+
     def payload(self):
         n, b = C.c_uint64(), C.c_uint64()
         k = lib().gsdf_hip_mesh_payload(self._mesh, C.byref(n), C.byref(b))
diff --git a/include/gsdf_hip.h b/include/gsdf_hip.h
--- a/include/gsdf_hip.h
+++ b/include/gsdf_hip.h
@@ -174,6 +174,7 @@
 int gsdf_hip_mesh_stats_get(const gsdf_mesh* m, gsdf_mesh_stats* st);
 int gsdf_hip_mesh_stage_ms(const gsdf_mesh* m, double* ms, const char** names, int cap, int* n);
 int gsdf_hip_mesh_payload(const gsdf_mesh* m, uint64_t* n_records, uint64_t* payload_bytes);
+uint64_t gsdf_hip_mesh_edge_bricks(const gsdf_mesh* m);
 int gsdf_hip_mesh_read_records(const gsdf_mesh* m, uint32_t* dst, uint64_t dst_records, uint64_t* n_records);
 int gsdf_hip_mesh_march(gsdf_mesh* m);
 int gsdf_hip_mesh_read(const gsdf_mesh* m, uint64_t first, uint64_t count, float* dst);
```

Result: faster. 499.4 billion, median of 6 (+1.2%).
